# xUhEngwAng/I2V-Adapter-Unofficial

Measured on AMD Instinct MI355X. Metric: denoising steps/sec @ 16fx512x512 SD1.5+I2V-Adapter, higher is better.
Workload: dtype f16

## Files before the change

i2v-adapter-unofficial_amd/_lib.py:

```python
import ctypes as C
import os

_HERE = os.path.dirname(os.path.abspath(__file__))
LIB_PATH = os.environ.get("I2V_LIB_PATH") or os.path.join(_HERE, "libi2v_hip.so")
ABI_VERSION = 27

I2V_EPI_NONE, I2V_EPI_GELU, I2V_EPI_GEGLU = 0, 1, 2
I2V_STORE_ROWMAJOR, I2V_STORE_ROWPERM, I2V_STORE_VT, I2V_STORE_VT_T = 0, 1, 2, 3
I2V_A_PLAIN, I2V_A_CONV3X3 = 0, 1
I2V_LORA_MAX_ADAPTERS, I2V_LORA_MAX_RANK = 8, 256
I2V_ROUTE_GENERIC, I2V_ROUTE_CONV_THIN, I2V_ROUTE_BIG_TILE, I2V_ROUTE_BIG_DEEP, I2V_ROUTE_BIG_SPLITK = 0, 1, 2, 3, 4
I2V_EXTRA_NONE, I2V_EXTRA_LNF, I2V_EXTRA_HILO, I2V_EXTRA_GNS, I2V_EXTRA_UPF = 0, 1, 2, 4, 8
I2V_TATTN_LDS_FORM, I2V_TATTN_REG_FORM = 0, 1
I2V_ADD_RES_MAX = 16
I2V_TAESD_PREP_IDENTITY, I2V_TAESD_PREP_UNIT, I2V_TAESD_PREP_CLAMP = 0, 1, 2


class HipLibraryError(RuntimeError):
    pass


class GemmParams(C.Structure):
    _fields_ = [
        ("a", C.c_void_p), ("lda", C.c_int64),
        ("a2", C.c_void_p), ("lda2", C.c_int64),
        ("k_split", C.c_int32), ("a_mode", C.c_int32),
        ("w", C.c_void_p), ("ldw", C.c_int64),
        ("bias", C.c_void_p),
        ("residual", C.c_void_p), ("ldr", C.c_int64),
        ("rowvec", C.c_void_p), ("ld_rowvec", C.c_int64), ("rows_per_vec", C.c_int32), ("rowvec_period", C.c_int32),
        ("ln_wsum", C.c_void_p), ("ln_eps", C.c_float),
        ("c", C.c_void_p), ("ldc", C.c_int64),
        ("M", C.c_int32), ("N", C.c_int32), ("K", C.c_int32),
        ("epilogue", C.c_int32), ("store_mode", C.c_int32),
        ("frames", C.c_int32), ("hw", C.c_int32),
        ("vt_len", C.c_int32), ("vt_ld", C.c_int32),
        ("out_scale", C.c_float),
        ("n_img", C.c_int32), ("in_h", C.c_int32), ("in_w", C.c_int32), ("cin", C.c_int32),
        ("out_h", C.c_int32), ("out_w", C.c_int32), ("stride", C.c_int32), ("upsample", C.c_int32),
        ("asym_pad", C.c_int32), ("conv_kblock", C.c_int32),
        ("w_batch_stride", C.c_int64), ("rows_per_w", C.c_int32),
        ("a_perm_frames", C.c_int32), ("a_perm_hw", C.c_int32),
        ("workspace", C.c_void_p), ("workspace_bytes", C.c_int64),
        ("c_is_f32", C.c_int32),
        ("gn_partial", C.c_void_p), ("gn_groups", C.c_int32),
        ("residual_lo", C.c_void_p), ("c_lo", C.c_void_p),
    ]


class GemmRoute(C.Structure):
    _fields_ = [
        ("family", C.c_int32), ("a_mode", C.c_int32),
        ("rows", C.c_int32), ("cols", C.c_int32), ("stages", C.c_int32),
        ("splits", C.c_int32), ("kps", C.c_int32),
        ("extra", C.c_int32), ("persistent", C.c_int32),
        ("generic_tile", C.c_int32), ("vec4", C.c_int32),
        ("epilogue", C.c_int32), ("store_mode", C.c_int32),
    ]

    def as_dict(self):
        return {name: int(getattr(self, name)) for name, _ in self._fields_}


class AttnParams(C.Structure):
    _fields_ = [
        ("q", C.c_void_p), ("q_row_stride", C.c_int64), ("q_batch_stride", C.c_int64),
        ("k", C.c_void_p), ("k_row_stride", C.c_int64), ("k_batch_stride", C.c_int64),
        ("vt", C.c_void_p), ("vt_row_stride", C.c_int64), ("vt_batch_stride", C.c_int64),
        ("o", C.c_void_p), ("o_row_stride", C.c_int64), ("o_batch_stride", C.c_int64),
        ("batch_q", C.c_int32), ("kv_group", C.c_int32), ("heads", C.c_int32), ("head_dim", C.c_int32),
        ("lq", C.c_int32), ("lk", C.c_int32),
        ("scale", C.c_float), ("accumulate", C.c_int32), ("acc_scale", C.c_float),
        ("lse", C.c_void_p),
    ]


class AttnBwdParams(C.Structure):
    _fields_ = [
        ("q", C.c_void_p), ("q_row_stride", C.c_int64), ("q_batch_stride", C.c_int64),
        ("qt", C.c_void_p), ("qt_row_stride", C.c_int64), ("qt_batch_stride", C.c_int64),
        ("k", C.c_void_p), ("k_row_stride", C.c_int64), ("k_batch_stride", C.c_int64),
        ("kt", C.c_void_p), ("kt_row_stride", C.c_int64), ("kt_batch_stride", C.c_int64),
        ("v", C.c_void_p), ("v_row_stride", C.c_int64), ("v_batch_stride", C.c_int64),
        ("dout", C.c_void_p), ("do_row_stride", C.c_int64), ("do_batch_stride", C.c_int64),
        ("doutt", C.c_void_p), ("dot_row_stride", C.c_int64), ("dot_batch_stride", C.c_int64),
        ("lse", C.c_void_p), ("delta", C.c_void_p),
        ("dq", C.c_void_p), ("dq_row_stride", C.c_int64), ("dq_batch_stride", C.c_int64),
        ("dk", C.c_void_p), ("dk_row_stride", C.c_int64), ("dk_batch_stride", C.c_int64),
        ("dv", C.c_void_p), ("dv_row_stride", C.c_int64), ("dv_batch_stride", C.c_int64),
        ("batch_q", C.c_int32), ("kv_group", C.c_int32), ("heads", C.c_int32), ("head_dim", C.c_int32),
        ("lq", C.c_int32), ("lk", C.c_int32),
        ("scale", C.c_float), ("kv_partitions", C.c_int32), ("dkv_partial", C.c_void_p),
    ]


class TAttnParams(C.Structure):
    _fields_ = [
        ("q", C.c_void_p), ("q_row_stride", C.c_int64),
        ("k", C.c_void_p), ("k_row_stride", C.c_int64),
        ("vt", C.c_void_p), ("vt_ld", C.c_int32),
        ("o", C.c_void_p), ("o_row_stride", C.c_int64),
        ("n_pixels", C.c_int32), ("frames", C.c_int32), ("heads", C.c_int32), ("head_dim", C.c_int32),
        ("scale", C.c_float),
    ]


class TAttnRoute(C.Structure):
    _fields_ = [
        ("form", C.c_int32), ("dqk", C.c_int32), ("dpv", C.c_int32),
        ("pf", C.c_int32), ("nqt", C.c_int32), ("blocks", C.c_int32),
    ]

    def as_dict(self):
        return {name: int(getattr(self, name)) for name, _ in self._fields_}


class MotionAttnParams(C.Structure):
    _fields_ = [
        ("x", C.c_void_p), ("ldx", C.c_int64),
        ("gamma", C.c_void_p),
        ("shift", C.c_void_p), ("ld_shift", C.c_int64),
        ("w_qkv", C.c_void_p),
        ("out", C.c_void_p), ("ldo", C.c_int64),
        ("rows", C.c_int64),
        ("channels", C.c_int32), ("heads", C.c_int32), ("head_dim", C.c_int32), ("frames", C.c_int32),
        ("eps", C.c_float), ("scale", C.c_float),
        ("w_o", C.c_void_p), ("b_o", C.c_void_p),
    ]


class CrossAttnFusedParams(C.Structure):
    _fields_ = [
        ("x", C.c_void_p), ("ldx", C.c_int64),
        ("gamma", C.c_void_p), ("beta", C.c_void_p),
        ("w_q", C.c_void_p),
        ("ctx_frag", C.c_void_p),
        ("out", C.c_void_p), ("ldo", C.c_int64),
        ("rows", C.c_int64), ("rows_per_ctx", C.c_int64),
        ("channels", C.c_int32), ("heads", C.c_int32), ("head_dim", C.c_int32), ("ctx_len", C.c_int32),
        ("eps", C.c_float), ("scale", C.c_float),
        ("ip_frag", C.c_void_p), ("ip_len", C.c_int32), ("ip_scale", C.c_float),
        ("w_o", C.c_void_p), ("b_o", C.c_void_p),
    ]


class FfFusedParams(C.Structure):
    _fields_ = [
        ("x", C.c_void_p), ("ldx", C.c_int64),
        ("gamma", C.c_void_p), ("beta", C.c_void_p),
        ("w1", C.c_void_p), ("b1", C.c_void_p),
        ("w2", C.c_void_p), ("b2", C.c_void_p),
        ("out", C.c_void_p), ("ldo", C.c_int64),
        ("rows", C.c_int64),
        ("channels", C.c_int32), ("inner", C.c_int32),
        ("eps", C.c_float),
        ("w3", C.c_void_p), ("b3", C.c_void_p),
        ("res2", C.c_void_p), ("ld_res2", C.c_int64),
        ("perm_frames", C.c_int32), ("perm_hw", C.c_int32),
        ("res2_lo", C.c_void_p), ("out_lo", C.c_void_p),
    ]


class LnQkvParams(C.Structure):
    _fields_ = [
        ("x", C.c_void_p), ("ldx", C.c_int64),
        ("gamma", C.c_void_p), ("beta", C.c_void_p),
        ("w", C.c_void_p),
        ("qk", C.c_void_p), ("ld_qk", C.c_int64),
        ("vt", C.c_void_p), ("vt_batch_stride", C.c_int64), ("vt_row_stride", C.c_int64),
        ("rows", C.c_int64), ("rows_per_image", C.c_int64),
        ("channels", C.c_int32), ("n_qk", C.c_int32),
        ("eps", C.c_float),
        ("x_image_stride", C.c_int64),
    ]


class UnetConfig(C.Structure):
    _fields_ = [
        ("in_channels", C.c_int32), ("out_channels", C.c_int32),
        ("block_out_channels", C.c_int32 * 4),
        ("layers_per_block", C.c_int32), ("num_attention_heads", C.c_int32),
        ("cross_attention_dim", C.c_int32), ("norm_num_groups", C.c_int32),
        ("motion_max_seq_length", C.c_int32), ("motion_num_attention_heads", C.c_int32),
        ("use_motion_mid_block", C.c_int32), ("ip_num_tokens", C.c_int32),
    ]


class UnetPlan(C.Structure):
    _fields_ = [
        ("batch", C.c_int32), ("frames", C.c_int32), ("height", C.c_int32), ("width", C.c_int32),
        ("ctx_len", C.c_int32), ("has_ip", C.c_int32),
    ]


class GnParams(C.Structure):
    _fields_ = [
        ("x", C.c_void_p), ("c1", C.c_int32),
        ("x2", C.c_void_p), ("c2", C.c_int32),
        ("gamma", C.c_void_p), ("beta", C.c_void_p),
        ("y", C.c_void_p),
        ("n_img", C.c_int32), ("hw", C.c_int32), ("groups", C.c_int32), ("frames_per_stat", C.c_int32),
        ("eps", C.c_float), ("silu", C.c_int32),
        ("out_perm", C.c_int32), ("frames", C.c_int32),
        ("workspace", C.c_void_p),
        ("gpartial_in", C.c_void_p), ("gpartial_rows", C.c_int32),
    ]


class LoraAdapter(C.Structure):
    _fields_ = [("down", C.c_void_p), ("up", C.c_void_p), ("rank", C.c_int32), ("scale", C.c_float)]


class LnParams(C.Structure):
    _fields_ = [
        ("x", C.c_void_p), ("ldx", C.c_int64),
        ("gamma", C.c_void_p), ("beta", C.c_void_p),
        ("pe", C.c_void_p), ("ld_pe", C.c_int64), ("pe_period", C.c_int32),
        ("y", C.c_void_p), ("ldy", C.c_int64),
        ("rows", C.c_int32), ("C", C.c_int32),
        ("eps", C.c_float),
        ("x_rows_per_batch", C.c_int32), ("x_batch_stride", C.c_int64),
    ]


class AddResidualsEntry(C.Structure):
    _fields_ = [("dst", C.c_void_p), ("dst_lo", C.c_void_p), ("skip", C.c_void_p), ("skip_lo", C.c_void_p), ("res", C.c_void_p),
                ("numel", C.c_int64)]


class AddResidualsParams(C.Structure):
    _fields_ = [("t", AddResidualsEntry * I2V_ADD_RES_MAX), ("n", C.c_int32), ("scale_rows", C.c_int32), ("scale_table", C.c_void_p),
                ("step_idx", C.c_void_p)]


class ConvC64Params(C.Structure):
    _fields_ = [
        ("x", C.c_void_p), ("ldx", C.c_int64),
        ("w", C.c_void_p), ("bias", C.c_void_p),
        ("residual", C.c_void_p), ("ldr", C.c_int64),
        ("out", C.c_void_p), ("ldo", C.c_int64),
        ("n_img", C.c_int32), ("height", C.c_int32), ("width", C.c_int32),
        ("cin", C.c_int32), ("cout", C.c_int32),
        ("relu_mid", C.c_int32), ("relu_out", C.c_int32),
        ("max_workgroups", C.c_int32),
    ]


_P = C.c_void_p
SIGNATURES = {
    "i2v_abi_version": (C.c_int, []),
    "i2v_last_error": (C.c_char_p, []),
    "i2v_gemm_f16": (C.c_int, [C.POINTER(GemmParams), _P]),
    "i2v_gemm_ln_supported": (C.c_int, [C.POINTER(GemmParams)]),
    "i2v_gemm_batch_supported": (C.c_int, [C.POINTER(GemmParams)]),
    "i2v_gemm_upconv_fold_supported": (C.c_int, [C.POINTER(GemmParams)]),
    "i2v_gemm_workspace_bytes": (C.c_int64, [C.POINTER(GemmParams)]),
    "i2v_gemm_gn_partial_rows": (C.c_int32, [C.POINTER(GemmParams)]),
    "i2v_gemm_route": (C.c_int, [C.POINTER(GemmParams), C.POINTER(GemmRoute)]),
    "i2v_gemm_last_route": (C.c_int, [C.POINTER(GemmRoute)]),
    "i2v_gemm_kernel_exists": (C.c_int, [C.POINTER(GemmRoute)]),
    "i2v_attention_f16": (C.c_int, [C.POINTER(AttnParams), _P]),
    "i2v_temporal_attention_f16": (C.c_int, [C.POINTER(TAttnParams), _P]),
    "i2v_temporal_attention_route": (C.c_int, [C.POINTER(TAttnParams), C.POINTER(TAttnRoute)]),
    "i2v_temporal_attention_last_route": (C.c_int, [C.POINTER(TAttnRoute)]),
    "i2v_tattn_kernel_exists": (C.c_int, [C.POINTER(TAttnRoute)]),
    "i2v_motion_attn_supported": (C.c_int32, [C.c_int64, C.c_int32, C.c_int32, C.c_int32, C.c_int32]),
    "i2v_motion_attn_pack_rows": (C.c_int32, [C.c_int32, C.c_int32]),
    "i2v_motion_attn_f16": (C.c_int, [C.POINTER(MotionAttnParams), _P]),
    "i2v_cross_attn_fused_supported": (C.c_int32, [C.c_int64, C.c_int32, C.c_int32, C.c_int32, C.c_int32, C.c_int64]),
    "i2v_cross_attn_fused_pack_rows": (C.c_int32, [C.c_int32, C.c_int32]),
    "i2v_cross_attn_fused_ctx_elems": (C.c_int64, [C.c_int32, C.c_int32, C.c_int32]),
    "i2v_cross_attn_fused_f16": (C.c_int, [C.POINTER(CrossAttnFusedParams), _P]),
    "i2v_ln_qkv_supported": (C.c_int32, [C.c_int64, C.c_int32, C.c_int32, C.c_int64]),
    "i2v_ln_qkv_f16": (C.c_int, [C.POINTER(LnQkvParams), _P]),
    "i2v_ff_fused_supported": (C.c_int32, [C.c_int64, C.c_int32, C.c_int32]),
    "i2v_ff_fused_tail_supported": (C.c_int32, [C.c_int64, C.c_int32, C.c_int32, C.c_int32, C.c_int32]),
    "i2v_ff_fused_f16": (C.c_int, [C.POINTER(FfFusedParams), _P]),
    "i2v_groupnorm_workspace_bytes": (C.c_int64, [C.c_int32, C.c_int32, C.c_int32]),
    "i2v_groupnorm_f16": (C.c_int, [C.POINTER(GnParams), _P]),
    "i2v_groupnorm_fold_f16": (C.c_int, [C.POINTER(GnParams), _P, C.c_int64, _P, C.c_int32, _P, _P, _P]),
    "i2v_layernorm_f16": (C.c_int, [C.POINTER(LnParams), _P]),
    "i2v_softmax_rows_f16": (C.c_int, [_P, C.c_int64, _P, C.c_int64, C.c_int32, C.c_int32, C.c_float, _P]),
    "i2v_nchw_to_tokens": (C.c_int, [_P, C.c_int32, _P, C.c_int32, C.c_int32, C.c_int32, C.c_int32, _P]),
    "i2v_tokens_to_nchw": (C.c_int, [_P, C.c_int32, C.c_int64, _P, C.c_int32, C.c_int32, C.c_int32, C.c_int32, _P]),
    "i2v_timestep_embedding": (C.c_int, [_P, _P, C.c_int32, _P, C.c_int32, C.c_int32, _P]),
    "i2v_silu_f16": (C.c_int, [_P, _P, C.c_int64, _P]),
    "i2v_repeat_rows_f16": (C.c_int, [_P, _P, C.c_int64, C.c_int64, C.c_int32, _P]),
    "i2v_copy3d_f16": (C.c_int, [_P, C.c_int64, C.c_int64, _P, C.c_int64, C.c_int64, C.c_int64, C.c_int64,
                                 C.c_int64, _P]),
    "i2v_pack_ctx_fragments_elems": (C.c_int64, [C.c_int32, C.c_int32, C.c_int32]),
    "i2v_pack_ctx_fragments_f16": (C.c_int, [_P, C.c_int64, _P, C.c_int64, C.c_int64, _P, C.c_int32, C.c_int32, C.c_int32, C.c_int32, _P]),
    "i2v_ddim_prep": (C.c_int, [_P, _P, _P, C.c_int32, C.c_int32, C.c_int32, C.c_int32, C.c_int32, C.c_int32, _P]),
    "i2v_gaussian_sample_f32": (C.c_int, [_P, _P, _P, C.c_int32, C.c_int32, C.c_int32, _P]),
    "i2v_first_frame_prior_f32": (C.c_int, [_P, _P, _P, _P, C.c_int32, C.c_int32, C.c_int32, C.c_int32, C.c_int32,
                                            C.c_float, C.c_float, C.c_float, C.c_float, C.c_float, _P]),
    "i2v_attention_lse_f32": (C.c_int, [C.POINTER(AttnParams), _P, _P]),
    "i2v_attention_bwd_f16": (C.c_int, [C.POINTER(AttnBwdParams), _P]),
    "i2v_transpose_f16": (C.c_int, [_P, C.c_int64, C.c_int64, _P, C.c_int64, C.c_int64, C.c_int32, C.c_int32, C.c_int32, _P]),
    "i2v_rowdot_heads_f32": (C.c_int, [_P, C.c_int64, _P, C.c_int64, _P, C.c_int64, C.c_int32, C.c_int32, C.c_int32, _P]),
    "i2v_layernorm_bwd_f16": (C.c_int, [_P, C.c_int64, _P, C.c_int64, _P, _P, C.c_int64, _P, C.c_int64, C.c_int32, C.c_int32,
                                        C.c_float, _P]),
    "i2v_geglu_bwd_f16": (C.c_int, [_P, C.c_int64, _P, C.c_int64, _P, C.c_int64, C.c_int64, C.c_int32, _P]),
    "i2v_geglu_f16": (C.c_int, [_P, C.c_int64, _P, C.c_int64, C.c_int64, C.c_int32, _P]),
    "i2v_colsum_f32": (C.c_int, [_P, C.c_int64, _P, C.c_int64, C.c_int32, _P]),
    "i2v_colsum_prod_f32": (C.c_int, [_P, C.c_int64, _P, C.c_int64, _P, C.c_int64, C.c_int32, _P]),
    "i2v_colsum_workspace_bytes": (C.c_int64, [C.c_int64, C.c_int32]),
    "i2v_colsum_det_f32": (C.c_int, [_P, C.c_int64, _P, C.c_int64, _P, C.c_int64, C.c_int32, _P, _P]),
    "i2v_masked_mse_grad_f16": (C.c_int, [_P, _P, _P, C.c_int64, C.c_int32, C.c_int32, C.c_int32, C.c_float, _P]),
    "i2v_masked_mse_grad_f32": (C.c_int, [_P, _P, _P, _P, C.c_int64, C.c_int32, C.c_int32, C.c_int32, C.c_float, _P]),
    "i2v_groupnorm_bwd_workspace_bytes": (C.c_int64, [C.c_int32, C.c_int32, C.c_int32]),
    "i2v_groupnorm_bwd_f16": (C.c_int, [C.POINTER(GnParams), _P, _P, _P, _P]),
    "i2v_add_f16": (C.c_int, [_P, _P, _P, C.c_int64, _P]),
    "i2v_permute_rows_f16": (C.c_int, [_P, _P, C.c_int64, C.c_int32, C.c_int32, C.c_int32, C.c_int32, _P]),
    "i2v_zero_insert2x_f16": (C.c_int, [_P, _P, C.c_int64, C.c_int32, C.c_int32, C.c_int32, _P]),
    "i2v_sum_pool2x_f16": (C.c_int, [_P, _P, C.c_int64, C.c_int32, C.c_int32, C.c_int32, _P]),
    "i2v_sumsq_f32": (C.c_int, [_P, C.c_int64, _P, _P]),
    "i2v_adamw_f32": (C.c_int, [_P, _P, _P, _P, C.c_int64, C.c_float, C.c_float, C.c_float, C.c_float, C.c_float, C.c_int32,
                                C.c_float, _P, C.c_float, _P]),
    "i2v_adamw_guarded_f32": (C.c_int, [_P, _P, _P, _P, C.c_int64, C.c_float, C.c_float, C.c_float, C.c_float, C.c_float,
                                        C.c_float, C.c_float, _P, C.c_int32, _P, _P, _P, _P]),
    "i2v_axpby_f32": (C.c_int, [_P, _P, C.c_float, C.c_float, C.c_int64, _P]),
    "i2v_select_row_f16": (C.c_int, [_P, C.c_int64, C.c_int32, _P, _P, C.c_int32, _P]),
    "i2v_ddim_cfg_step": (C.c_int, [_P, _P, C.c_int32, C.c_int64, _P, C.c_int32, _P, C.c_float, C.c_int32, C.c_int32,
                                    C.c_int32, C.c_int32, C.c_int32, _P]),
    "i2v_dpm_cfg_step": (C.c_int, [_P, _P, _P, C.c_int32, C.c_int64, _P, C.c_int32, _P, C.c_float, C.c_int32, C.c_int32,
                                   C.c_int32, C.c_int32, C.c_int32, _P]),
    "i2v_lcm_cfg_step": (C.c_int, [_P, _P, C.c_int32, _P, C.c_int32, C.c_int64, _P, C.c_int32, _P, C.c_float, C.c_int32, C.c_int32,
                                   C.c_int32, C.c_int32, C.c_int32, _P]),
    "i2v_freeu_f16": (C.c_int, [_P, _P, _P, _P, _P, _P, C.c_int32, C.c_int32, C.c_int32, C.c_int32, C.c_int32, C.c_float, C.c_float, _P]),
    "i2v_vae_tile_blend": (C.c_int, [_P, _P, _P, _P, C.c_int32, C.c_int32, C.c_int32, C.c_int32, C.c_int64, C.c_int32, C.c_int32, C.c_int32,
                                     C.c_int32, C.c_int32, _P, C.c_int32, C.c_int32, C.c_int32, C.c_int32, _P]),
    "i2v_lora_merge": (C.c_int, [_P, _P, C.c_int32, C.c_int32, C.c_int32, C.POINTER(LoraAdapter), C.c_int32, _P]),
    "i2v_freeinit_workspace_bytes": (C.c_int64, [C.c_int32, C.c_int32, C.c_int32, C.c_int32, C.c_int32]),
    "i2v_freeinit_mix": (C.c_int, [_P, _P, _P, _P, _P, _P, C.c_int64, C.c_int32, C.c_int32, C.c_int32, C.c_int32, C.c_int32, C.c_float,
                                   C.c_float, _P]),
    "i2v_freenoise_gather_f16": (C.c_int, [_P, C.c_int64, _P, C.c_int64, _P, C.c_int64, C.c_int32, C.c_int32, C.c_int32, C.c_int32, _P]),
    "i2v_freenoise_blend_f16": (C.c_int, [_P, C.c_int64, _P, C.c_int64, _P, _P, C.c_int64, C.c_int32, C.c_int32, C.c_int32, C.c_int32,
                                          C.c_int32, _P]),
    "i2v_clip_embed_f16": (C.c_int, [_P, _P, _P, _P, _P, C.c_int32, C.c_int32, C.c_int32, C.c_int32, C.c_int32, _P]),
    "i2v_clip_attention_f16": (C.c_int, [_P, C.c_int64, C.c_int32, C.c_int32, C.c_int32, _P, C.c_int64, C.c_int32, C.c_int32, C.c_int32,
                                         C.c_int32, C.c_float, _P]),
    "i2v_quick_gelu_f16": (C.c_int, [_P, _P, C.c_int64, _P]),
    "i2v_clip_patchify_f16": (C.c_int, [_P, _P, C.c_int64, C.c_int32, C.c_int32, C.c_int32, C.c_int32, _P]),
    "i2v_clip_vision_embed_f16": (C.c_int, [_P, _P, C.c_int64, _P, _P, C.c_int32, C.c_int32, C.c_int32, _P]),
    "i2v_clip_vision_attention_f16": (C.c_int, [_P, C.c_int64, C.c_int32, C.c_int32, C.c_int32, _P, C.c_int64, C.c_int32, C.c_int32,
                                                C.c_int32, C.c_int32, C.c_float, _P]),
    "i2v_perceiver_attention_f16": (C.c_int, [_P, C.c_int64, C.c_int32, _P, C.c_int64, C.c_int32, C.c_int32, C.c_int32, _P, C.c_int64,
                                              C.c_int32, C.c_int32, C.c_int32, _P, C.c_int64, C.c_int32, C.c_int32, C.c_int32, C.c_int32,
                                              C.c_float, _P]),
    "i2v_add_residuals_f16": (C.c_int, [C.POINTER(AddResidualsParams), _P]),
    "i2v_conv3x3_c64_f16": (C.c_int, [C.POINTER(ConvC64Params), _P]),
    "i2v_taesd_prep_f16": (C.c_int, [_P, C.c_int32, _P, C.c_int64, C.c_int32, C.c_int32, C.c_int32, C.c_int32, _P]),
    "i2v_pixel_unshuffle8_f16": (C.c_int, [_P, C.c_int32, _P, C.c_int32, C.c_int32, C.c_int32, C.c_int32, _P]),
    "i2v_avgpool2x_f16": (C.c_int, [_P, _P, C.c_int32, C.c_int32, C.c_int32, C.c_int32, _P]),
    "i2v_relu_f16": (C.c_int, [_P, _P, C.c_int64, _P]),
    "i2v_add_broadcast_residual_f16": (C.c_int, [_P, _P, _P, _P, _P, C.c_int64, C.c_int64, _P, C.c_int32, _P, _P]),
    "i2v_interp_rows_f16": (C.c_int, [_P, C.c_int64, C.c_int32, _P, _P, _P, _P, C.c_int64, C.c_int32, C.c_int32, _P]),
    "i2v_masked_renoise_f32": (C.c_int, [_P, _P, _P, _P, _P, C.c_int32, _P, C.c_int64, C.c_int32, C.c_int32, _P]),
    "i2v_weight_embeds_f16": (C.c_int, [_P, _P, _P, _P, C.c_int32, C.c_int32, C.c_int32, C.c_int64, C.c_int64, C.c_int32, _P]),
# ... 56 lines not shown
```

i2v-adapter-unofficial_amd/blocks.py:

```python
import math
import os
from typing import Optional

import torch
from torch import nn

from . import kernels as K
from . import streams
from ._lib import (I2V_EPI_GEGLU, I2V_EPI_GELU, I2V_EPI_NONE, I2V_STORE_ROWPERM, HipLibraryError)
from .checkpoint import PretrainedMixin

f16 = torch.float16


class HipModule(nn.Module):

    def __init__(self):
        super().__init__()
        self._packed = None
        self._packed_key = None

    def _pack(self):
        return {}

# ... 81 lines not shown
                    for ky in rows[py][ty]:
                        for kx in rows[px][tx]:
                            acc = w[:, :, ky, kx] if acc is None else acc + w[:, :, ky, kx]
                    taps.append(acc)
            phases.append(torch.stack(taps, dim=1))
    f = torch.stack(phases, dim=0)
    if K.conv_k_block(ci):
        f = f.reshape(4, co, 4, ci // 64, 64).permute(0, 1, 3, 2, 4)
    return f.reshape(4, co, 4 * ci).to(dtype).contiguous()


UPCONV_FOLD = os.environ.get("I2V_UPCONV_FOLD", "1") != "0"


def pack_geglu(weight, bias):
    inner = weight.shape[0] // 2
    w = torch.stack([weight[:inner], weight[inner:]], dim=1).reshape(2 * inner, weight.shape[1])
    b = torch.stack([bias[:inner], bias[inner:]], dim=1).reshape(2 * inner)
    return w16(w), w16(b)


LN_FOLD = os.environ.get("I2V_LN_FOLD", "1") != "0"


def fold_layernorm(weight, bias, gamma, beta):
    wf = (weight.detach().float() * gamma.detach().float()[None, :]).to(f16).contiguous()
    wsum = wf.float().sum(dim=1).contiguous()
    b = weight.detach().float() @ beta.detach().float()
    if bias is not None:
        b = b + bias.detach().float()
    return wf, wsum, b.to(f16).contiguous()


def fold_layernorm_geglu(proj_weight, proj_bias, gamma, beta):
    wf, wsum, b = fold_layernorm(proj_weight, proj_bias, gamma, beta)
    inner = wf.shape[0] // 2
    il = lambda t: torch.stack([t[:inner], t[inner:]], dim=1).reshape((2 * inner,) + tuple(t.shape[1:])).contiguous()
    return il(wf), il(wsum), il(b)


class LnFoldPlan:

    def __init__(self):
        self._cache = {}

    def get(self, key, probe):
        if not LN_FOLD:
            return False
        if key not in self._cache:
            self._cache[key] = bool(probe())
        return self._cache[key]


class ProjectedContext:

    def __init__(self, text, ip):
        self.text, self.ip = text, ip
        self.kv = {}
        self.frag = {}

    @property
    def shape(self):
        return self.text.shape


class ProjectedTemb:

    def __init__(self, all_proj, slices):
        self.all_proj, self.slices = all_proj, slices

    def view_for(self, resnet):
        off, n = self.slices[resnet]
        return self.all_proj[:, off: off + n]

    def first_half(self):
        r = self.all_proj.shape[0]
        return self if r == 1 else ProjectedTemb(self.all_proj[: r // 2], self.slices)


GN_FOLD = os.environ.get("I2V_GN_FOLD", "1") != "0"
GN_FOLD_RATIO = float(os.environ.get("I2V_GN_FOLD_RATIO", "4"))


def gn_proj_in(x, gamma, beta, groups, eps, w, bias, frames=0):
    n, hh, ww, c = x.shape
    hw = hh * ww
    fps = frames if frames > 0 else 1
    s_groups, n_out = n // fps, w.shape[0]
    if GN_FOLD and GN_FOLD_RATIO * s_groups * n_out <= n * hw:
        kw = dict(rows_per_vec=fps * hw, w_rows=fps * hw, a_perm=(frames, hw) if frames > 0 else None)
        if _fold_supported(x, s_groups, n_out, kw):
            w_s, b_s = K.groupnorm_fold(x, gamma, beta, groups, eps, w, bias, frames_per_stat=fps)
            return K.gemm(x.view(-1, c), w_s, None, rowvec=b_s, **kw)
    if frames > 0:
        h = K.groupnorm(x, gamma, beta, groups, eps, frames_per_stat=frames, out_perm=True, frames=frames)
    else:
        h = K.groupnorm(x, gamma, beta, groups, eps).view(-1, c)
    return K.gemm(h, w, bias)


_FOLD_OK = {}


def _fold_supported(x, s_groups, n_out, kw):
    key = (tuple(x.shape), s_groups, n_out, kw["w_rows"], kw["a_perm"])
    ok = _FOLD_OK.get(key)
    if ok is None:
        c = x.shape[3]
        w_s = torch.empty((s_groups, n_out, c), dtype=f16, device=x.device)
        b_s = torch.empty((s_groups, n_out), dtype=f16, device=x.device)
        ok = _FOLD_OK[key] = K.gemm(x.view(-1, c), w_s, None, rowvec=b_s, query_batch_support=True, **kw)
    return ok


def to_tokens(x: torch.Tensor, c_pad: Optional[int] = None) -> torch.Tensor:
    return K.nchw_to_tokens(x, c_pad)


def from_tokens(x: torch.Tensor, dtype) -> torch.Tensor:
    return K.tokens_to_nchw(x, dtype=dtype if dtype in (torch.float32, f16) else f16)


def _as_f16_matrix(t: torch.Tensor) -> torch.Tensor:
    if not t.is_cuda:
        raise HipLibraryError(f"tensor on {t.device}: the HIP path has no CPU fallback")
    return t.to(f16).contiguous()


class Timesteps(nn.Module):

    def __init__(self, num_channels: int, flip_sin_to_cos: bool = True, downscale_freq_shift: float = 0):
        super().__init__()
        if not flip_sin_to_cos or downscale_freq_shift != 0:
            raise NotImplementedError("hot path uses Timesteps(C, flip_sin_to_cos=True, freq_shift=0)")
        self.num_channels = num_channels

    def forward(self, timesteps: torch.Tensor) -> torch.Tensor:
        return K.timestep_embedding(timesteps.to(torch.float32).contiguous(), self.num_channels)


class TimestepEmbedding(HipModule):

    def __init__(self, in_channels: int, time_embed_dim: int, act_fn: str = "silu"):
        super().__init__()
        self.linear_1 = nn.Linear(in_channels, time_embed_dim)
        self.act = nn.SiLU()
        self.linear_2 = nn.Linear(time_embed_dim, time_embed_dim)

    def _pack(self):
        return dict(w1=w16(self.linear_1.weight), b1=w16(self.linear_1.bias), w2=w16(self.linear_2.weight),
                    b2=w16(self.linear_2.bias))

    def forward(self, sample, condition=None):
        p = self.packed()
        h = K.silu(K.gemm(_as_f16_matrix(sample), p["w1"], p["b1"]))
        return K.gemm(h, p["w2"], p["b2"])


_PRECISE_STREAM = os.environ.get("I2V_STREAM_PRECISE", "0") != "0"


def precise_stream() -> bool:
    return _PRECISE_STREAM


def set_precise_stream(on: bool) -> bool:
    global _PRECISE_STREAM
    prev, _PRECISE_STREAM = _PRECISE_STREAM, bool(on)
    return prev


GN_FROM_CONV = os.environ.get("I2V_GN_FROM_CONV", "1") != "0"


class ResnetBlock2D(HipModule):
# ... 194 lines not shown
        return o

    def forward(self, hidden_states, encoder_hidden_states=None, attention_mask=None):
        if attention_mask is not None:
            raise NotImplementedError("attention masks are never passed on the hot path (SURVEY 8b)")
        p = self.packed()
        x = _as_f16_matrix(hidden_states)
        b, l, c = x.shape
        q = K.gemm(x.view(-1, c), p["wq"])
        ctx = x if encoder_hidden_states is None else _as_f16_matrix(encoder_hidden_states)
        ctx_ip = None
        if self.ip_num_tokens and encoder_hidden_states is not None:
            end = ctx.shape[1] - self.ip_num_tokens
            ctx_text = torch.empty((ctx.shape[0], end, ctx.shape[2]), dtype=f16, device=x.device)
            ctx_ip = torch.empty((ctx.shape[0], self.ip_num_tokens, ctx.shape[2]), dtype=f16, device=x.device)
            K.copy3d(ctx[:, :end], ctx_text)
            K.copy3d(ctx[:, end:], ctx_ip)
            ctx = ctx_text
        if b % ctx.shape[0] != 0:
            raise ValueError(f"context batch {ctx.shape[0]} does not divide query batch {b}")
        o = self._cross(q, ctx, ctx_ip, b, l, b // ctx.shape[0])
        out = K.gemm(o, p["wo"], p["bo"])
        return out.view(b, l, -1).to(hidden_states.dtype)


class GEGLU(nn.Module):
    def __init__(self, dim_in, dim_out, bias=True):
        super().__init__()
        self.proj = nn.Linear(dim_in, dim_out * 2, bias=bias)


class GELU(nn.Module):
    def __init__(self, dim_in, dim_out, approximate="none", bias=True):
        super().__init__()
        if approximate != "none":
            raise NotImplementedError("only erf GELU is implemented")
        self.proj = nn.Linear(dim_in, dim_out, bias=bias)


def ff_tail_operands(weight, bias, c_in, c_out):
    if c_in != c_out or not K.ff_fused_tail_supported(128, c_in, 4 * c_in):
        return None
    return K.pack_ff_tail(weight.detach().reshape(c_out, c_in), bias)


class FeedForward(HipModule):

    def __init__(self, dim, dim_out=None, mult=4, dropout=0.0, activation_fn="geglu", inner_dim=None, bias=True):
        super().__init__()
        if not bias:
            raise NotImplementedError("ff_bias=False is not on the hot path")
        inner_dim = int(dim * mult) if inner_dim is None else inner_dim
        dim_out = dim if dim_out is None else dim_out
        self.activation_fn = activation_fn
        if activation_fn == "geglu":
            act = GEGLU(dim, inner_dim, bias=bias)
        elif activation_fn == "gelu":
            act = GELU(dim, inner_dim, bias=bias)
        else:
            raise ValueError(f"unsupported activation_fn {activation_fn}")
        self.net = nn.ModuleList([act, nn.Dropout(dropout), nn.Linear(inner_dim, dim_out, bias=bias)])

    def _pack(self):
        proj = self.net[0].proj
        if self.activation_fn == "geglu":
            w1, b1 = pack_geglu(proj.weight.detach(), proj.bias.detach())
        else:
            w1, b1 = w16(proj.weight), w16(proj.bias)
        out = LazyPack(w1=w1, b1=b1, w2=w16(self.net[2].weight), b2=w16(self.net[2].bias))
        if self.activation_fn == "geglu" and K.ff_fused_supported(128, self.net[2].weight.shape[0], self.net[2].weight.shape[1]):
            out.lazy("fused", lambda proj=proj, lin=self.net[2]: K.pack_ff_fused(proj.weight, proj.bias, lin.weight, lin.bias))
        return out

    def _fwd(self, n2d, residual2d, **store):
        p = self.packed()
        epi = I2V_EPI_GEGLU if self.activation_fn == "geglu" else I2V_EPI_GELU
        h = K.gemm(n2d, p["w1"], p["b1"], epilogue=epi)
        return K.gemm(h, p["w2"], p["b2"], residual=residual2d, **store)

    def fused_supported(self, x2d):
        p = self.packed()
        return FUSED_FF and "fused" in p and K.ff_fused_supported(x2d.shape[0], x2d.shape[1], p["b1"].numel() // 2)

    def _fwd_fused(self, x2d, gamma32, beta32, eps, tail=None):
        return K.ff_fused(x2d, gamma32, beta32, self.packed()["fused"], eps=eps, tail=tail, precise=precise_stream())

    def tail_supported(self, x2d, tail):
        p = self.packed()
        return (FUSED_FF and FUSED_FF_TAIL and tail is not None and tail[0] is not None and "fused" in p and
                K.ff_fused_tail_supported(x2d.shape[0], x2d.shape[1], p["b1"].numel() // 2, tail[2], tail[3]))

    def fold_norm(self, norm):
        if self.activation_fn != "geglu":
            return None
        proj = self.net[0].proj
        return fold_layernorm_geglu(proj.weight, proj.bias, norm.weight, norm.bias)

    def _fwd_folded(self, x2d, eps, folded, **store):
        p = self.packed()
        wf, wsum, bf = folded
        h = K.gemm(x2d, wf, bf, epilogue=I2V_EPI_GEGLU, ln=(wsum, eps))
        return K.gemm(h, p["w2"], p["b2"], residual=x2d, **store)

    def folded_supported(self, x2d, eps, folded):
        wf, wsum, bf = folded
        return K.gemm(x2d, wf, bf, epilogue=I2V_EPI_GEGLU, ln=(wsum, eps), query_ln_support=True)

    def forward(self, hidden_states, scale: float = 1.0):
        x = _as_f16_matrix(hidden_states)
        shp = x.shape
        return self._fwd(x.view(-1, shp[-1]), None).view(*shp[:-1], -1).to(hidden_states.dtype)


class SinusoidalPositionalEmbedding(nn.Module):

    def __init__(self, embed_dim: int, max_seq_length: int = 32):
        super().__init__()
        self.embed_dim, self.max_seq_length = embed_dim, max_seq_length
        self.register_buffer("pe", self._table(embed_dim, max_seq_length))

    @staticmethod
    def _table(embed_dim, max_seq_length):
        position = torch.arange(max_seq_length, device="cpu").unsqueeze(1)
        div_term = torch.exp(torch.arange(0, embed_dim, 2, device="cpu") * (-math.log(10000.0) / embed_dim))
        pe = torch.zeros(1, max_seq_length, embed_dim, device="cpu")
        pe[0, :, 0::2] = torch.sin(position * div_term)
        pe[0, :, 1::2] = torch.cos(position * div_term)
        return pe

    def reset_table_(self):
        with torch.no_grad():
            self.pe.copy_(self._table(self.embed_dim, self.max_seq_length).to(self.pe.dtype))


FUSED_MOTION_ATTN = os.environ.get("I2V_MOTION_FUSED", "1") != "0"
FUSED_FF = os.environ.get("I2V_FF_FUSED", "1") != "0"
FUSED_FF_TAIL = os.environ.get("I2V_FF_TAIL", "1") != "0"
FUSED_ATTN_OUT = os.environ.get("I2V_ATTN_OUTP", "1") != "0"


class TemporalTransformerBlock(HipModule):

    def __init__(self, dim, num_attention_heads, attention_head_dim, dropout=0.0, cross_attention_dim=None,
                 activation_fn="geglu", attention_bias=False, double_self_attention=True,
                 norm_elementwise_affine=True, norm_eps=1e-5, positional_embeddings="sinusoidal",
                 num_positional_embeddings=32, **_unused):
        super().__init__()
        if cross_attention_dim is not None or not double_self_attention or positional_embeddings != "sinusoidal":
            raise NotImplementedError("motion modules use double self-attention with sinusoidal positions (A9)")
        self.dim, self.heads, self.dim_head = dim, num_attention_heads, attention_head_dim
        self.eps = norm_eps
        self.max_len = num_positional_embeddings
        self.pos_embed = SinusoidalPositionalEmbedding(dim, max_seq_length=num_positional_embeddings)
        self.norm1 = nn.LayerNorm(dim, elementwise_affine=norm_elementwise_affine, eps=norm_eps)
        self.attn1 = Attention(query_dim=dim, heads=num_attention_heads, dim_head=attention_head_dim,
                               dropout=dropout, bias=attention_bias)
        self.norm2 = nn.LayerNorm(dim, elementwise_affine=norm_elementwise_affine, eps=norm_eps)
        self.attn2 = Attention(query_dim=dim, heads=num_attention_heads, dim_head=attention_head_dim,
                               dropout=dropout, bias=attention_bias)
        self.norm3 = nn.LayerNorm(dim, elementwise_affine=norm_elementwise_affine, eps=norm_eps)
        self.ff = FeedForward(dim, dropout=dropout, activation_fn=activation_fn)
        self._plan = LnFoldPlan()
        self.free_noise = None

    def _pack(self):
        p = LazyPack(pe=w16(self.pos_embed.pe[0]))
        for i, (norm, attn) in enumerate(((self.norm1, self.attn1), (self.norm2, self.attn2)), 1):
# ... 68 lines not shown
                if FUSED_ATTN_OUT:
                    t = K.motion_attn(t, tab[0], tab[1], p[f"wqkv{i}"], heads=self.heads, head_dim=self.dim_head, frames=frames,
                                      eps=self.eps, out_proj=p[f"wo_frag{i}"])
                    continue
                o = K.motion_attn(t, tab[0], tab[1], p[f"wqkv{i}"], heads=self.heads, head_dim=self.dim_head, frames=frames,
                                  eps=self.eps)
                t = K.gemm(o, p[f"wo{i}"], p[f"bo{i}"], residual=t)
                continue
            n = None if fold_attn else K.layernorm(t, p[f"g{i}"], p[f"b{i}"], self.eps, pe=p["pe"], pe_period=frames)
            with streams.fork(overlap, t.device) as fk:
                with fk.side():
                    if fold_attn:
                        vt = K.project_vt(t, p[f"f_wv{i}"], frames, bias=p[f"f_cv{i}"], ln=(p[f"f_sv{i}"], self.eps),
                                          pe_t=p[f"f_pev{i}"], pe_period=frames)
                    else:
                        vt = K.project_vt(n, p[f"wv{i}"], frames)
                if fold_attn:
                    qk = K.gemm(t, p[f"f_wqk{i}"], p[f"f_cqk{i}"], ln=(p[f"f_sqk{i}"], self.eps),
                                rowvec=p[f"f_peqk{i}"], rowvec_period=frames)
                else:
                    qk = K.gemm(n, p[f"wqk{i}"])
            o = K.temporal_attention(qk[:, :c], qk[:, c:], vt, n_pixels=n_pixels, frames=frames, heads=self.heads,
                                     head_dim=self.dim_head, scale=self.dim_head ** -0.5)
            t = K.gemm(o, p[f"wo{i}"], p[f"bo{i}"], residual=t)
        return t

    def _fwd_ff(self, t, fold_ff, tail):
        p = self.packed()

        def ret(v, applied=False):
            return v if tail is None else (v, applied)
        if self.ff.fused_supported(t):
            if self.ff.tail_supported(t, tail):
                return ret(self.ff._fwd_fused(t, p["g3_f32"], p["b3_f32"], self.eps, tail=tail), True)
            return ret(self.ff._fwd_fused(t, p["g3_f32"], p["b3_f32"], self.eps))
        if fold_ff:
            return ret(self.ff._fwd_folded(t, self.eps, p["f_ff"]))
        n = K.layernorm(t, p["g3"], p["b3"], self.eps)
        return ret(self.ff._fwd(n, t))


class TransformerTemporalModel(HipModule):

    def __init__(self, num_attention_heads=16, attention_head_dim=88, in_channels=None, out_channels=None,
                 num_layers=1, dropout=0.0, norm_num_groups=32, cross_attention_dim=None, attention_bias=False,
                 activation_fn="geglu", norm_elementwise_affine=True, double_self_attention=True,
                 positional_embeddings=None, num_positional_embeddings=None):
        super().__init__()
        inner_dim = num_attention_heads * attention_head_dim
        self.in_channels, self.inner_dim = in_channels, inner_dim
        self.groups = norm_num_groups
        self.norm = nn.GroupNorm(norm_num_groups, in_channels, eps=1e-6, affine=True)
        self.proj_in = nn.Linear(in_channels, inner_dim)
        self.transformer_blocks = nn.ModuleList([
            TemporalTransformerBlock(inner_dim, num_attention_heads, attention_head_dim, dropout=dropout,
                                     cross_attention_dim=cross_attention_dim, activation_fn=activation_fn,
                                     attention_bias=attention_bias, double_self_attention=double_self_attention,
                                     norm_elementwise_affine=norm_elementwise_affine,
                                     positional_embeddings=positional_embeddings,
                                     num_positional_embeddings=num_positional_embeddings)
            for _ in range(num_layers)])
        self.proj_out = nn.Linear(inner_dim, in_channels)

    def _pack(self):
        p = LazyPack(g=w16(self.norm.weight), b=w16(self.norm.bias), wi=w16(self.proj_in.weight),
                     bi=w16(self.proj_in.bias), wo=w16(self.proj_out.weight), bo=w16(self.proj_out.bias))
        p.lazy("tail", lambda po=self.proj_out, ci=self.inner_dim, co=self.in_channels: ff_tail_operands(po.weight, po.bias, ci, co))
        return p

    def set_free_noise(self, settings):
        for blk in self.transformer_blocks:
            if settings is not None and settings.context_length > blk.max_len:
                raise ValueError(f"`context_length` {settings.context_length} exceeds the motion module's num_positional_embeddings "
                                 f"({blk.max_len})")
        for blk in self.transformer_blocks:
            blk.free_noise = settings

    def _fwd(self, x, num_frames):
        p = self.packed()
        n, hh, ww, c = x.shape
        if n % num_frames != 0:
            raise ValueError(f"batch {n} is not a multiple of num_frames {num_frames}")
        n_pixels = (n // num_frames) * hh * ww
        t = gn_proj_in(x, p["g"], p["b"], self.groups, 1e-6, p["wi"], p["bi"], frames=num_frames)
        applied = False
        for j, blk in enumerate(self.transformer_blocks):
            if j + 1 == len(self.transformer_blocks):
                t, applied = blk._fwd(t, n_pixels, num_frames, tail=(p["tail"], K.sview(x, -1, c), num_frames, hh * ww))
            else:
                t = blk._fwd(t, n_pixels, num_frames)
        if applied:
            return K.sview(t, n, hh, ww, c)
        out = K.gemm(t, p["wo"], p["bo"], residual=K.sview(x, -1, c), store=I2V_STORE_ROWPERM, frames=num_frames,
                     hw=hh * ww, precise=precise_stream())
        return K.sview(out, n, hh, ww, c)

    def forward(self, hidden_states, encoder_hidden_states=None, num_frames: int = 1, return_dict=False, **_unused):
        return (from_tokens(self._fwd(to_tokens(hidden_states), num_frames), hidden_states.dtype),)


class ImageProjection(HipModule):

    def __init__(self, image_embed_dim=768, cross_attention_dim=768, num_image_text_embeds=4):
        super().__init__()
        self.num_image_text_embeds = num_image_text_embeds
        self.cross_attention_dim = cross_attention_dim
        self.image_embeds = nn.Linear(image_embed_dim, num_image_text_embeds * cross_attention_dim)
        self.norm = nn.LayerNorm(cross_attention_dim)

    def _pack(self):
        return dict(w=w16(self.image_embeds.weight), b=w16(self.image_embeds.bias), g=w16(self.norm.weight),
                    be=w16(self.norm.bias))

    def forward(self, image_embeds):
        p = self.packed()
        x = _as_f16_matrix(image_embeds)
        y = K.gemm(x, p["w"], p["b"]).view(-1, self.cross_attention_dim)
        y = K.layernorm(y, p["g"], p["be"], self.norm.eps)
        return y.view(x.shape[0], self.num_image_text_embeds, self.cross_attention_dim)


class _ResamplerAttention(nn.Module):

    def __init__(self, dim, inner):
        super().__init__()
        self.to_q, self.to_k, self.to_v = (nn.Linear(dim, inner, bias=False) for _ in range(3))
        self.to_out = nn.ModuleList([nn.Linear(inner, dim, bias=False), nn.Dropout(0.0)])


class _ResamplerFeedForward(nn.Module):

    def __init__(self, dim, inner):
        super().__init__()
        self.net = nn.ModuleList([GELU(dim, inner, bias=False), nn.Dropout(0.0), nn.Linear(inner, dim, bias=False)])


class Resampler(HipModule):

    DIM_HEAD, MAX_QUERIES, MAX_KEYS = 64, 64, 288

    def __init__(self, embed_dims=768, output_dims=1024, hidden_dims=1280, depth=4, dim_head=64, heads=16, num_queries=8, ffn_ratio=4):
        super().__init__()
        if dim_head != self.DIM_HEAD:
            raise NotImplementedError(f"dim_head {dim_head}: the attention kernel (i2v_perceiver_attention_f16) implements head_dim "
                                      f"{self.DIM_HEAD} only")
        if not 1 <= num_queries <= self.MAX_QUERIES:
            raise NotImplementedError(f"num_queries {num_queries}: the attention kernel (i2v_perceiver_attention_f16) takes 1 to "
                                      f"{self.MAX_QUERIES} queries")
        inner_ff = int(hidden_dims * ffn_ratio)
        if embed_dims % 8 or output_dims % 8 or hidden_dims % 8 or inner_ff % 8 or inner_ff != hidden_dims * ffn_ratio:
            raise NotImplementedError(f"embed_dims {embed_dims}, output_dims {output_dims}, hidden_dims {hidden_dims} and hidden_dims * "
                                      f"ffn_ratio {hidden_dims * ffn_ratio} must be multiples of 8 (i2v_gemm_f16)")
        self.embed_dims, self.output_dims, self.hidden_dims = embed_dims, output_dims, hidden_dims
        self.depth, self.dim_head, self.heads, self.num_queries, self.ffn_ratio = depth, dim_head, heads, num_queries, ffn_ratio
        self.latents = nn.Parameter(torch.randn(1, num_queries, hidden_dims) / hidden_dims ** 0.5)
        self.proj_in = nn.Linear(embed_dims, hidden_dims)
        self.proj_out = nn.Linear(hidden_dims, output_dims)
        self.norm_out = nn.LayerNorm(output_dims)
        self.layers = nn.ModuleList([
            nn.ModuleList([nn.LayerNorm(hidden_dims), nn.LayerNorm(hidden_dims), _ResamplerAttention(hidden_dims, dim_head * heads),
                           nn.Sequential(nn.LayerNorm(hidden_dims), _ResamplerFeedForward(hidden_dims, inner_ff))])
            for _ in range(depth)])

    def check_tokens(self, tokens: int):
        if tokens < 1 or tokens + self.num_queries > self.MAX_KEYS:
            raise NotImplementedError(f"{tokens} image tokens + {self.num_queries} queries: the attention kernel "
                                      f"(i2v_perceiver_attention_f16) takes at most {self.MAX_KEYS} keys")
# ... 500 lines not shown
```

i2v-adapter-unofficial_amd/csrc/ff_fused.hip:

```cpp
#include <stdlib.h>

#include <type_traits>

#include "common.h"

namespace {

__device__ __forceinline__ void ff_dma16(__amdgpu_buffer_rsrc_t rsrc, f16* lds_wave_base, unsigned voff, unsigned soff = 0) {
  __builtin_amdgcn_raw_ptr_buffer_load_lds(rsrc, (__attribute__((address_space(3))) void*)lds_wave_base, 16, voff, soff, 0, 0);
}
__device__ __forceinline__ int opaque(int v) {
  asm volatile("" : "+v"(v));
  return v;
}

constexpr int FF_PIX = 8;
constexpr int FF_CH = 128;
constexpr int FF_U = 2;
constexpr int FF_PD = 3;
constexpr int FF_AD = 4;

template <int C, int INNER, int H, bool PROJ, bool HILO = false>
__global__ __launch_bounds__(64 * H) void ff_fused_kernel(const i2v_ff_fused_params p, const int ntiles, long long* __restrict__ stamps) {
  constexpr int KS = C / 32, NJ = C / 64, NCH = INNER / FF_CH, DN = C / H, DT = (DN + 15) / 16;
  static_assert(C % 64 == 0 && H == 8 && INNER % FF_CH == 0 && DT == 3 && DN == 40, "SD-1.5 64^2 level: C = 320, inner = 1280");
  static_assert(PROJ || !HILO, "the precise stream enters and leaves through the tail");
  extern __shared__ __attribute__((aligned(16))) f16 lds[];
  f16* panel = lds;
  f16* hbuf = lds + FF_PIX * 16 * C;
  f16* raw = lds + FF_PIX * 16 * C;
  static_assert(2 * FF_PIX * 16 * FF_CH <= FF_PIX * 16 * C, "the raw rows of a tile cover the chunk buffers (160 KB of LDS in all)");
  const int tid = threadIdx.x, lane = tid & 63, wave = __builtin_amdgcn_readfirstlane(tid >> 6);
  const int g = lane >> 4, l15 = lane & 15, sub = lane & 7, sw = l15 & 7;
  const int swz[2] = {(g ^ sw) * 8, ((4 + g) ^ sw) * 8};
  const f16* __restrict__ X = reinterpret_cast<const f16*>(p.x);

  auto fetch_rows = [&](const int tile) {
    const f16* base = X + ((int64_t)tile * (FF_PIX * 16) + 16 * wave) * p.ldx;
    const auto rs = __builtin_amdgcn_make_buffer_rsrc(const_cast<f16*>(base), 0, (int)((15 * p.ldx + C) * 2), 0x00020000);
    const int ln = opaque(lane);
    const unsigned voff = (unsigned)(((ln >> 3) * p.ldx + (ln & 7) * 8) * 2);
#pragma unroll
    for (int half = 0; half < 2; ++half)
#pragma unroll
      for (int j = 0; j < NJ; ++j)
        ff_dma16(rs, raw + 16 * wave * C + (half * NJ + j) * 512, voff, (unsigned)((8 * half * p.ldx + 8 * j * 8) * 2));
  };
  auto fetch_residual = [&](const int tile) {
    const f16* base = X + ((int64_t)tile * (FF_PIX * 16) + 16 * wave) * p.ldx;
    const auto rs = __builtin_amdgcn_make_buffer_rsrc(const_cast<f16*>(base), 0, (int)((15 * p.ldx + C) * 2), 0x00020000);
    constexpr int CPR = C / 8;
    static_assert((16 * CPR) % 64 == 0 && CPR % 8 == 0, "whole DMA instructions per wave, swizzle inside groups of 8 chunks");
    const int ln = opaque(lane);
#pragma unroll
    for (int i = 0; i < 16 * CPR / 64; ++i) {
      const int q = i * 64 + ln, r = q / CPR, cp = q - r * CPR;
      ff_dma16(rs, panel + 16 * wave * C + i * 512, (unsigned)((r * p.ldx + (cp ^ (r & 7)) * 8) * 2));
    }
  };
  auto normalise_rows = [&]() {
    f16x8 xv[2][NJ];
#pragma unroll
    for (int half = 0; half < 2; ++half)
#pragma unroll
      for (int j = 0; j < NJ; ++j) xv[half][j] = *reinterpret_cast<const f16x8*>(raw + 16 * wave * C + ((half * NJ + j) * 64 + lane) * 8);
    const float* gp = reinterpret_cast<const float*>(p.gamma);
    const float* bp = reinterpret_cast<const float*>(p.beta);
    asm volatile("" : "+s"(gp), "+s"(bp));
    f32x4 ga[NJ][2], be[NJ][2];
#pragma unroll
    for (int j = 0; j < NJ; ++j) {
      ga[j][0] = *reinterpret_cast<const f32x4*>(gp + (sub + 8 * j) * 8);
      ga[j][1] = *reinterpret_cast<const f32x4*>(gp + (sub + 8 * j) * 8 + 4);
      be[j][0] = *reinterpret_cast<const f32x4*>(bp + (sub + 8 * j) * 8);
      be[j][1] = *reinterpret_cast<const f32x4*>(bp + (sub + 8 * j) * 8 + 4);
    }
#pragma unroll
    for (int half = 0; half < 2; ++half) {
      const int row = 16 * wave + 8 * half + (lane >> 3);
      float v[NJ][8];
      float s = 0.f;
#pragma unroll
      for (int j = 0; j < NJ; ++j)
#pragma unroll
        for (int e = 0; e < 8; ++e) {
          v[j][e] = (float)xv[half][j][e];
          s += v[j][e];
        }
      s = sum_lanes8(s);
      const float mean = s / (float)C;
      float q = 0.f;
#pragma unroll
      for (int j = 0; j < NJ; ++j)
#pragma unroll
        for (int e = 0; e < 8; ++e) {
          v[j][e] -= mean;
          q = fmaf(v[j][e], v[j][e], q);
        }
      q = sum_lanes8(q);
      const float rstd = rsqrtf(q / (float)C + p.eps);
#pragma unroll
      for (int j = 0; j < NJ; ++j) {
        const int ch = sub + 8 * j;
        f16x8 o;
#pragma unroll
        for (int e = 0; e < 8; ++e) o[e] = (f16)fmaf(v[j][e] * rstd, ga[j][e >> 2][e & 3], be[j][e >> 2][e & 3]);
        *reinterpret_cast<f16x8*>(panel + row * C + ((ch ^ (row & 7)) * 8)) = o;
      }
    }
// ... 197 lines not shown
      auto load_res2 = [&](const int h) {
#pragma unroll
        for (int q = 0; q < HP; ++q) {
          const f16* rrow = R2 + (int64_t)orow[h * HP + q] * p.ld_res2;
          r01[h][q] = *reinterpret_cast<const u32x4*>(rrow + c01);
          r2[h][q] = (eg == 0) ? *reinterpret_cast<const u32x4*>(rrow + 32) : u32x4{0u, 0u, 0u, 0u};
        }
      };
      const f16* __restrict__ R2L = reinterpret_cast<const f16*>(HILO ? p.res2_lo : p.res2) + wave * DN;
      f16* __restrict__ OL = reinterpret_cast<f16*>(HILO ? p.out_lo : p.out) + wave * DN;
      u32x4 l01[HP], l2[HP];
      auto load_res2_lo = [&](const int h) {
        if constexpr (HILO) {
#pragma unroll
          for (int q = 0; q < HP; ++q) {
            const f16* rrow = R2L + (int64_t)orow[h * HP + q] * p.ld_res2;
            l01[q] = *reinterpret_cast<const u32x4*>(rrow + c01);
            l2[q] = (eg == 0) ? *reinterpret_cast<const u32x4*>(rrow + 32) : u32x4{0u, 0u, 0u, 0u};
          }
        }
      };
      out_rows(tile, el15, orow);
#pragma unroll
      for (int pix = 0; pix < FF_PIX; ++pix)
#pragma unroll
        for (int t = 0; t < DT; ++t) {
          if (16 * t + 4 * eg < DN) {
            f16x4* slot = reinterpret_cast<f16x4*>(panel + 16 * pix * C + res_off[t]);
            const f16x4 xres = *slot;
            f32x4 o = acc2[pix][t];
#pragma unroll
            for (int r = 0; r < 4; ++r) o[r] += (float)xres[r];
            *slot = to_half(o);
          }
        }
      lds_barrier();
      f32x4 acc3[FF_PIX][DT];
      {
        const float* b3 = reinterpret_cast<const float*>(p.b3) + wave * DN;
#pragma unroll
        for (int t = 0; t < DT; ++t) {
          const f32x4 bias3 = (16 * t + 4 * eg < DN) ? *reinterpret_cast<const f32x4*>(b3 + 16 * t + 4 * eg) : f32x4{0.f, 0.f, 0.f, 0.f};
#pragma unroll
          for (int pix = 0; pix < FF_PIX; ++pix) acc3[pix][t] = bias3;
        }
      }
      {
        const int w3o = wave * (KS * DT * 1024);
        auto ldw3 = [&](const int s, const int t) {
          return __builtin_bit_cast(f16x8, __builtin_amdgcn_raw_buffer_load_b128(rs_w3, w_lane, w3o + (s * DT + t) * 1024, 0));
        };
        f16x8 wf[FF_PD][DT];
#pragma unroll
        for (int s = 0; s < FF_PD - 1; ++s)
#pragma unroll
          for (int t = 0; t < DT; ++t) wf[s][t] = ldw3(s, t);
        constexpr int NI = KS * FF_PIX;
        auto lda = [&](const int i) {
          return *reinterpret_cast<const f16x8*>(alane + 16 * (i % FF_PIX) * C + 64 * ((i / FF_PIX) >> 1) + swz[(i / FF_PIX) & 1]);
        };
        f16x8 af[FF_AD + 1];
#pragma unroll
        for (int i = 0; i < FF_AD; ++i) af[i] = lda(i);
#pragma unroll
        for (int i = 0; i < NI; ++i) {
          const int s = i / FF_PIX, pix = i % FF_PIX;
          if (pix == 0 && s + FF_PD - 1 < KS) {
#pragma unroll
            for (int t = 0; t < DT; ++t) wf[(s + FF_PD - 1) % FF_PD][t] = ldw3(s + FF_PD - 1, t);
          }
          if (pix == 0 && s + FF_PD - 1 == KS - 1) {
            if (next < ntiles) fetch_rows(next);
            load_res2(0);
          }
          if (i + FF_AD < NI) af[(i + FF_AD) % (FF_AD + 1)] = lda(i + FF_AD);
#pragma unroll
          for (int t = 0; t < DT; ++t) acc3[pix][t] = mfma16x16x32(wf[s % FF_PD][t], af[i % (FF_AD + 1)], acc3[pix][t]);
          __builtin_amdgcn_sched_barrier(0);
        }
      }
      FF_T(t_p);
      load_res2(1);
      load_res2_lo(0);
#pragma unroll
      for (int pix = 0; pix < FF_PIX; ++pix) {
        if (pix == HP) {
          __builtin_amdgcn_sched_barrier(0);
          load_res2_lo(1);
        }
        const u32x4 q01 = r01[pix / HP][pix % HP], q2 = r2[pix / HP][pix % HP];
        u32x2 xa = {q01[0], q01[1]}, xb = {q01[2], q01[3]}, xc = {q2[0], q2[1]}, xd = {q2[2], q2[3]};
        asm volatile("s_nop 1\n\tv_permlane16_swap_b32 %0, %1\n\tv_permlane16_swap_b32 %2, %3\n\t"
                     "v_permlane16_swap_b32 %4, %5\n\tv_permlane16_swap_b32 %6, %7"
                     : "+v"(xa[0]), "+v"(xb[0]), "+v"(xa[1]), "+v"(xb[1]), "+v"(xc[0]), "+v"(xd[0]), "+v"(xc[1]), "+v"(xd[1]));
        const f16x4 xres[DT] = {__builtin_bit_cast(f16x4, xa), __builtin_bit_cast(f16x4, xb), __builtin_bit_cast(f16x4, xc)};
        f16x4 xlo[DT] = {};
        if constexpr (HILO) {
          const u32x4 p01 = l01[pix % HP], p2 = l2[pix % HP];
          u32x2 la = {p01[0], p01[1]}, lb = {p01[2], p01[3]}, lc = {p2[0], p2[1]}, ld = {p2[2], p2[3]};
          asm volatile("s_nop 1\n\tv_permlane16_swap_b32 %0, %1\n\tv_permlane16_swap_b32 %2, %3\n\t"
                       "v_permlane16_swap_b32 %4, %5\n\tv_permlane16_swap_b32 %6, %7"
                       : "+v"(la[0]), "+v"(lb[0]), "+v"(la[1]), "+v"(lb[1]), "+v"(lc[0]), "+v"(ld[0]), "+v"(lc[1]), "+v"(ld[1]));
          xlo[0] = __builtin_bit_cast(f16x4, la);
          xlo[1] = __builtin_bit_cast(f16x4, lb);
          xlo[2] = __builtin_bit_cast(f16x4, lc);
        }
        u32x2 oh[DT], ol[DT];
#pragma unroll
        for (int t = 0; t < DT; ++t) {
          f32x4 o = acc3[pix][t];
#pragma unroll
          for (int r = 0; r < 4; ++r) o[r] += (float)xres[t][r];
          if constexpr (HILO) {
#pragma unroll
            for (int r = 0; r < 4; ++r) o[r] += (float)xlo[t][r];
          }
          const f16x4 o16 = to_half(o);
          oh[t] = __builtin_bit_cast(u32x2, o16);
          if constexpr (HILO) {
            f32x4 d;
#pragma unroll
            for (int r = 0; r < 4; ++r) d[r] = o[r] - (float)o16[r];
            ol[t] = __builtin_bit_cast(u32x2, to_half(d));
          }
        }
        store_row(O + (int64_t)orow[pix] * p.ldo, oh);
        if constexpr (HILO) store_row(OL + (int64_t)orow[pix] * p.ldo, ol);
      }
    }
    lds_barrier();
    FF_T(t_epi);
  }
#ifdef I2V_FF_STAMPS
  if (stamps != nullptr && lane == 0) {
    long long* st = stamps + ((int64_t)blockIdx.x * H + wave) * 8;
    st[0] = t_ln; st[1] = t_ff1; st[2] = t_glu; st[3] = t_bar; st[4] = t_ff2; st[5] = t_epi; st[6] = t_w; st[7] = t_p;
  }
#endif
}

constexpr size_t FF_LDS = 2 * (size_t)FF_PIX * 16 * 320 * sizeof(f16);

template <bool PROJ, bool HILO = false>
int ff_cus() { return i2v_big_lds_kernel_cus(reinterpret_cast<const void*>(ff_fused_kernel<320, 1280, 8, PROJ, HILO>), FF_LDS); }

}

extern "C" int32_t i2v_ff_fused_supported(int64_t rows, int32_t channels, int32_t inner) {
  return rows > 0 && rows % (FF_PIX * 16) == 0 && rows / (FF_PIX * 16) < (1 << 24) && channels == 320 && inner == 1280 &&
         ff_cus<false>() > 0;
}

extern "C" int32_t i2v_ff_fused_tail_supported(int64_t rows, int32_t channels, int32_t inner, int32_t perm_frames, int32_t perm_hw) {
  if (!(rows > 0 && rows % (FF_PIX * 16) == 0 && rows / (FF_PIX * 16) < (1 << 24) && channels == 320 && inner == 1280)) return 0;
  if (perm_frames != 0 || perm_hw != 0) {
    if (perm_frames <= 0 || (perm_frames & (perm_frames - 1)) || perm_hw <= 0 || rows % ((int64_t)perm_frames * perm_hw) != 0) return 0;
  }
  return ff_cus<true>() > 0;
}

extern "C" int i2v_ff_fused_f16(const i2v_ff_fused_params* pp, i2v_stream_t stream) {
  I2V_CHECK_ARG(pp != nullptr, "i2v_ff_fused_f16: null params");
  const i2v_ff_fused_params& p = *pp;
  I2V_CHECK_ARG(p.x && p.gamma && p.beta && p.w1 && p.b1 && p.w2 && p.b2 && p.out, "i2v_ff_fused_f16: null pointer");
  const bool tail = p.w3 != nullptr;
  I2V_CHECK_ARG(p.rows > 0 && p.rows % (FF_PIX * 16) == 0 && p.rows / (FF_PIX * 16) < (1 << 24) && p.channels == 320 && p.inner == 1280,
                "i2v_ff_fused_f16: rows %lld channels %d inner %d is not a fused shape (i2v_ff_fused_supported)", (long long)p.rows,
                p.channels, p.inner);
  I2V_CHECK_ARG(p.ldx >= p.channels && p.ldx % 8 == 0 && p.ldo >= p.channels && p.ldo % 8 == 0, "i2v_ff_fused_f16: row strides");
  I2V_CHECK_ARG(i2v_al16(p.x) && i2v_al16(p.gamma) && i2v_al16(p.beta) && i2v_al16(p.w1) && i2v_al16(p.b1) && i2v_al16(p.w2) && i2v_al16(p.b2) && i2v_al16(p.out),
                "i2v_ff_fused_f16: pointers must be 16-byte aligned");
  I2V_CHECK_ARG(p.ldx < (1 << 24), "i2v_ff_fused_f16: ldx");
  if (tail) {
    I2V_CHECK_ARG(p.b3 && p.res2, "i2v_ff_fused_f16: the tail needs w3, b3 and res2");
    I2V_CHECK_ARG(i2v_al16(p.w3) && i2v_al16(p.b3) && i2v_al16(p.res2) && p.ld_res2 >= p.channels && p.ld_res2 % 8 == 0,
                  "i2v_ff_fused_f16: tail operands must be 16-byte aligned, ld_res2 a multiple of 8");
    I2V_CHECK_ARG(i2v_ff_fused_tail_supported(p.rows, p.channels, p.inner, p.perm_frames, p.perm_hw) ||
                      ff_cus<true>() == 0,
                  "i2v_ff_fused_f16: perm_frames %d / perm_hw %d do not describe rows %lld (i2v_ff_fused_tail_supported)", p.perm_frames,
                  p.perm_hw, (long long)p.rows);
    I2V_CHECK_ARG(!(p.perm_frames > 0 && p.out == p.x), "i2v_ff_fused_f16: out must not alias x when the tail permutes the rows");
    I2V_CHECK_ARG((p.res2_lo == nullptr) == (p.out_lo == nullptr) && i2v_al16(p.res2_lo) && i2v_al16(p.out_lo) && (p.out_lo == nullptr || p.out_lo != p.out),
                  "i2v_ff_fused_f16: res2_lo and out_lo come together, 16-byte aligned");
  } else {
    I2V_CHECK_ARG(p.b3 == nullptr && p.res2 == nullptr && p.perm_frames == 0 && p.perm_hw == 0 && p.res2_lo == nullptr && p.out_lo == nullptr,
                  "i2v_ff_fused_f16: tail fields set without w3");
  }
  const bool hilo = tail && p.out_lo != nullptr;
  const int cus = hilo ? ff_cus<true, true>() : tail ? ff_cus<true>() : ff_cus<false>();
  if (cus <= 0) I2V_FAIL(I2V_ERR_UNSUPPORTED, "i2v_ff_fused_f16: %zu bytes of LDS refused by this device", FF_LDS);
  const int ntiles = (int)(p.rows / (FF_PIX * 16));
  const int grid = i2v_persistent_grid(ntiles, cus);
  long long* stamps = nullptr;
#ifdef I2V_FF_STAMPS
  stamps = getenv("I2V_FF_STAMP_PTR") ? reinterpret_cast<long long*>(strtoull(getenv("I2V_FF_STAMP_PTR"), nullptr, 0)) : nullptr;
#endif
  hipStream_t s = reinterpret_cast<hipStream_t>(stream);
  if (hilo)
    hipLaunchKernelGGL((ff_fused_kernel<320, 1280, 8, true, true>), dim3((unsigned)grid), dim3(512), FF_LDS, s, p, ntiles, stamps);
  else if (tail)
    hipLaunchKernelGGL((ff_fused_kernel<320, 1280, 8, true>), dim3((unsigned)grid), dim3(512), FF_LDS, s, p, ntiles, stamps);
  else
    hipLaunchKernelGGL((ff_fused_kernel<320, 1280, 8, false>), dim3((unsigned)grid), dim3(512), FF_LDS, s, p, ntiles, stamps);
  return i2v_check_launch("i2v_ff_fused_f16");
}
```

i2v-adapter-unofficial_amd/csrc/norm.hip:

```cpp
#include <cstdlib>

#include "common.h"

namespace {

static inline int gn_rows_per_chunk(int n_img, int hw) {
  const int want_chunks = (int)i2v_cdiv(1024, n_img);
  int rpc = (int)i2v_cdiv(hw, want_chunks);
  rpc = (rpc + 7) / 8 * 8;
  if (rpc < 16) rpc = 16;
  if (rpc > 256) rpc = 256;
  return rpc;
}

__device__ __forceinline__ float wave_sum(float v) {
#pragma unroll
  for (int o = 32; o >= 1; o >>= 1) v += __shfl_xor(v, o, 64);
  return v;
}

constexpr int GN_MAXC = 2560, GN_MAXG = 64;
__global__ __launch_bounds__(256) void gn_stats_kernel(const f16* __restrict__ x1, int c1, const f16* __restrict__ x2,
                                                       int c2, int hw, int rpc, float* __restrict__ partial,
                                                       float* __restrict__ gpartial = nullptr, int groups = 0) {
// ... 645 lines not shown
        if (row < p.rows) {
          f16x8 pv = zero8();
          if (p.pe) pv = ld_global_16B(reinterpret_cast<const f16*>(p.pe) + (int64_t)(row % p.pe_period) * p.ld_pe + vi * 8);
          f16x8 o;
#pragma unroll
          for (int e = 0; e < 8; ++e) {
            float t = (v[r][i][e] - mean[r]) * rstd[r] * (float)ga[e] + (float)be[e];
            if (p.pe) t += (float)pv[e];
            o[e] = (f16)t;
          }
          *reinterpret_cast<f16x8*>(reinterpret_cast<f16*>(p.y) + (int64_t)row * p.ldy + vi * 8) = o;
        }
      }
    }
  }
}

__global__ __launch_bounds__(256) void softmax_rows_kernel(const f16* __restrict__ x, int64_t ldx, f16* __restrict__ y,
                                                           int64_t ldy, int rows, int cols, float scale_log2) {
  const int lane = threadIdx.x & 63;
  const int row = blockIdx.x * 4 + (threadIdx.x >> 6);
  if (row >= rows) return;
  const f16* xr = x + (int64_t)row * ldx;
  f16* yr = y + (int64_t)row * ldy;
  const int nvec = cols / 8;
  float mx = -INFINITY;
  for (int v = lane; v < nvec; v += 64) {
    const f16x8 t = ld_global_16B(xr + v * 8);
#pragma unroll
    for (int e = 0; e < 8; ++e) mx = fmaxf(mx, (float)t[e]);
  }
  for (int c = nvec * 8 + lane; c < cols; c += 64) mx = fmaxf(mx, (float)xr[c]);
#pragma unroll
  for (int o = 32; o >= 1; o >>= 1) mx = fmaxf(mx, __shfl_xor(mx, o, 64));
  const float mb = mx * scale_log2;
  float sum = 0.f;
  for (int v = lane; v < nvec; v += 64) {
    const f16x8 t = ld_global_16B(xr + v * 8);
#pragma unroll
    for (int e = 0; e < 8; ++e) sum += __builtin_amdgcn_exp2f((float)t[e] * scale_log2 - mb);
  }
  for (int c = nvec * 8 + lane; c < cols; c += 64) sum += __builtin_amdgcn_exp2f((float)xr[c] * scale_log2 - mb);
  sum = wave_sum(sum);
  const float inv = 1.0f / sum;
  for (int v = lane; v < nvec; v += 64) {
    const f16x8 t = ld_global_16B(xr + v * 8);
    f16x8 o;
#pragma unroll
    for (int e = 0; e < 8; ++e) o[e] = (f16)(__builtin_amdgcn_exp2f((float)t[e] * scale_log2 - mb) * inv);
    *reinterpret_cast<f16x8*>(yr + v * 8) = o;
  }
  for (int c = nvec * 8 + lane; c < cols; c += 64) yr[c] = (f16)(__builtin_amdgcn_exp2f((float)xr[c] * scale_log2 - mb) * inv);
}

}

extern "C" int64_t i2v_groupnorm_workspace_bytes(int32_t n_img, int32_t hw, int32_t channels) {
  const int64_t nchunk = i2v_cdiv(hw, gn_rows_per_chunk(n_img, hw));
  return ((int64_t)n_img * nchunk * channels * 2 + (int64_t)n_img * channels * 2 + (int64_t)n_img * nchunk * GN_MAXG * 2) *
         (int64_t)sizeof(float);
}

extern "C" int i2v_groupnorm_fold_f16(const i2v_gn_params* pp, const void* w, int64_t ldw, const void* bias, int32_t n_out,
                                      void* w_out, void* bias_out, i2v_stream_t stream) {
  I2V_CHECK_ARG(pp != nullptr, "i2v_groupnorm_fold_f16: null params");
  const i2v_gn_params& p = *pp;
  const int C = p.c1 + p.c2;
  I2V_CHECK_ARG(p.x && p.gamma && p.beta && p.workspace && w && w_out && bias_out, "i2v_groupnorm_fold_f16: null pointer");
  I2V_CHECK_ARG(p.n_img > 0 && p.hw > 0 && p.c1 > 0 && p.c2 >= 0 && n_out > 0 && ldw >= C,
                "i2v_groupnorm_fold_f16: bad sizes");
  I2V_CHECK_ARG((p.c2 == 0) == (p.x2 == nullptr), "i2v_groupnorm_fold_f16: x2 / c2 mismatch");
  I2V_CHECK_ARG(p.c1 % 8 == 0 && p.c2 % 8 == 0, "i2v_groupnorm_fold_f16: channel counts must be multiples of 8");
  I2V_CHECK_ARG(p.groups > 0 && C % p.groups == 0, "i2v_groupnorm_fold_f16: channels %d not divisible by groups %d", C,
                p.groups);
  I2V_CHECK_ARG(p.frames_per_stat > 0 && p.n_img % p.frames_per_stat == 0,
                "i2v_groupnorm_fold_f16: n_img %d not divisible by frames_per_stat %d", p.n_img, p.frames_per_stat);
  I2V_CHECK_ARG(i2v_al16(p.x) && (!p.x2 || i2v_al16(p.x2)) && i2v_al16(p.workspace) && i2v_al16(p.gamma) && i2v_al16(p.beta),
                "i2v_groupnorm_fold_f16: pointers must be 16-byte aligned");
  hipStream_t s = reinterpret_cast<hipStream_t>(stream);
  const int rpc = gn_rows_per_chunk(p.n_img, p.hw);
  const int nchunk = (int)i2v_cdiv(p.hw, rpc);
  float* partial = reinterpret_cast<float*>(p.workspace);
  float* coef = partial + (int64_t)p.n_img * nchunk * C * 2;
  if (p.groups <= GN_MAXG && C <= GN_MAXC) {
    float* gpartial = coef + (int64_t)p.n_img * C * 2;
    hipLaunchKernelGGL(gn_stats_kernel, dim3(nchunk, p.n_img), dim3(256), (size_t)C * 2 * sizeof(float), s,
                       reinterpret_cast<const f16*>(p.x), p.c1, reinterpret_cast<const f16*>(p.x2), p.c2, p.hw, rpc, partial, gpartial,
                       p.groups);
    hipLaunchKernelGGL(gn_finalize_g_kernel, dim3(p.n_img / p.frames_per_stat, p.groups), dim3(256), 0, s, gpartial, nchunk, C,
                       p.groups, p.frames_per_stat, p.hw, rpc, p.eps, reinterpret_cast<const f16*>(p.gamma),
                       reinterpret_cast<const f16*>(p.beta), coef);
  } else {
    hipLaunchKernelGGL(gn_stats_kernel, dim3(nchunk, p.n_img), dim3(256), 0, s, reinterpret_cast<const f16*>(p.x), p.c1,
                       reinterpret_cast<const f16*>(p.x2), p.c2, p.hw, rpc, partial);
    hipLaunchKernelGGL(gn_finalize_kernel, dim3(p.n_img / p.frames_per_stat, p.groups), dim3(256), 0, s, partial, nchunk, C,
                       p.groups, p.frames_per_stat, p.hw, rpc, p.eps, reinterpret_cast<const f16*>(p.gamma),
                       reinterpret_cast<const f16*>(p.beta), coef);
  }
  hipLaunchKernelGGL(gn_fold_kernel, dim3(n_out, p.n_img / p.frames_per_stat), dim3(256), 0, s, coef, p.frames_per_stat, C,
                     reinterpret_cast<const f16*>(w), ldw, reinterpret_cast<const f16*>(bias), n_out,
                     reinterpret_cast<f16*>(w_out), reinterpret_cast<f16*>(bias_out));
  return i2v_check_launch("i2v_groupnorm_fold_f16");
}

extern "C" int i2v_groupnorm_f16(const i2v_gn_params* pp, i2v_stream_t stream) {
  I2V_CHECK_ARG(pp != nullptr, "i2v_groupnorm_f16: null params");
  const i2v_gn_params& p = *pp;
  const int C = p.c1 + p.c2;
  I2V_CHECK_ARG(p.x && p.gamma && p.beta && p.y && p.workspace, "i2v_groupnorm_f16: null pointer");
  I2V_CHECK_ARG(p.n_img > 0 && p.hw > 0 && p.c1 > 0 && p.c2 >= 0, "i2v_groupnorm_f16: bad sizes");
  I2V_CHECK_ARG((p.c2 == 0) == (p.x2 == nullptr), "i2v_groupnorm_f16: x2 / c2 mismatch");
  I2V_CHECK_ARG(p.c1 % 8 == 0 && p.c2 % 8 == 0, "i2v_groupnorm_f16: channel counts must be multiples of 8 (%d, %d)",
                p.c1, p.c2);
  I2V_CHECK_ARG(p.groups > 0 && C % p.groups == 0, "i2v_groupnorm_f16: channels %d not divisible by groups %d", C,
                p.groups);
  I2V_CHECK_ARG(p.frames_per_stat > 0 && p.n_img % p.frames_per_stat == 0,
                "i2v_groupnorm_f16: n_img %d not divisible by frames_per_stat %d", p.n_img, p.frames_per_stat);
  if (p.out_perm) I2V_CHECK_ARG(p.frames > 0 && p.n_img % p.frames == 0, "i2v_groupnorm_f16: bad frames for out_perm");
  I2V_CHECK_ARG(i2v_al16(p.x) && i2v_al16(p.y) && (!p.x2 || i2v_al16(p.x2)) && i2v_al16(p.workspace) && i2v_al16(p.gamma) && i2v_al16(p.beta),
                "i2v_groupnorm_f16: pointers must be 16-byte aligned");
  hipStream_t s = reinterpret_cast<hipStream_t>(stream);
  if (p.gpartial_in != nullptr) {
    I2V_CHECK_ARG(p.frames_per_stat == 1 && !p.out_perm && p.x2 == nullptr && p.groups <= GN_MAXG && C <= GN_MAXC,
                  "i2v_groupnorm_f16: gpartial_in is for per-image statistics of one source without a row permutation");
    I2V_CHECK_ARG(p.gpartial_rows > 0 && p.hw % p.gpartial_rows == 0 && (reinterpret_cast<uintptr_t>(p.gpartial_in) & 7) == 0,
                  "i2v_groupnorm_f16: gpartial_rows (%d) must divide hw (%d)", p.gpartial_rows, p.hw);
    const int pchunks = p.hw / p.gpartial_rows;
    const size_t lds = ((size_t)pchunks * p.groups * 2 + (size_t)p.groups * 2) * sizeof(float);
    I2V_CHECK_ARG(lds <= 48 * 1024, "i2v_groupnorm_f16: %d partial blocks per image do not fit the finalise step", pchunks);
    const int rpc = gn_rows_per_chunk(p.n_img, p.hw);
    hipLaunchKernelGGL(gn_apply_fused_kernel, dim3((unsigned)i2v_cdiv(p.hw, rpc), p.n_img), dim3(256), lds, s,
                       reinterpret_cast<const f16*>(p.x), p.c1, static_cast<const f16*>(nullptr), 0,
                       reinterpret_cast<const float*>(p.gpartial_in), p.groups, reinterpret_cast<const f16*>(p.gamma),
                       reinterpret_cast<const f16*>(p.beta), p.eps, reinterpret_cast<f16*>(p.y), p.hw, rpc, p.silu, pchunks,
                       p.gpartial_rows);
    return i2v_check_launch("i2v_groupnorm_f16(partials from the producer)");
  }
  {
    size_t lds = 0;
    const int gb = gn_slab_plan(p.n_img, p.hw, C, p.groups, p.frames_per_stat, &lds);
    if (gb > 0) {
      static const bool attr_ok = hipFuncSetAttribute(reinterpret_cast<const void*>(gn_slab_kernel),
                                                      hipFuncAttributeMaxDynamicSharedMemorySize, 97 * 1024) == hipSuccess;
      if (attr_ok) {
        hipLaunchKernelGGL(gn_slab_kernel, dim3(p.groups / gb, p.n_img / p.frames_per_stat), dim3(256), lds, s,
                           reinterpret_cast<const f16*>(p.x), p.c1, reinterpret_cast<const f16*>(p.x2), p.c2,
                           reinterpret_cast<const f16*>(p.gamma), reinterpret_cast<const f16*>(p.beta),
                           reinterpret_cast<f16*>(p.y), p.hw, p.frames_per_stat, p.groups, gb, p.eps, p.silu, p.out_perm,
                           p.frames);
        return i2v_check_launch("i2v_groupnorm_f16(slab)");
      }
    }
  }
  const int rpc = gn_rows_per_chunk(p.n_img, p.hw);
  const int nchunk = (int)i2v_cdiv(p.hw, rpc);
  float* partial = reinterpret_cast<float*>(p.workspace);
  float* coef = partial + (int64_t)p.n_img * nchunk * C * 2;
  const f16* x1 = reinterpret_cast<const f16*>(p.x);
  const f16* x2 = reinterpret_cast<const f16*>(p.x2);
  static const int fused_off = getenv("I2V_GN_FUSED") ? (atoi(getenv("I2V_GN_FUSED")) == 0) : 0;
  const size_t fused_lds = ((size_t)nchunk * p.groups * 2 + (size_t)p.groups * 2) * sizeof(float);
  if (!fused_off && p.frames_per_stat == 1 && !p.out_perm && p.groups <= GN_MAXG && C <= GN_MAXC && fused_lds <= 48 * 1024) {
    float* gpartial = coef + (int64_t)p.n_img * C * 2;
    hipLaunchKernelGGL(gn_stats_kernel, dim3(nchunk, p.n_img), dim3(256), (size_t)C * 2 * sizeof(float), s, x1, p.c1, x2, p.c2, p.hw,
                       rpc, partial, gpartial, p.groups);
    hipLaunchKernelGGL(gn_apply_fused_kernel, dim3(nchunk, p.n_img), dim3(256), fused_lds, s, x1, p.c1, x2, p.c2, gpartial, p.groups,
                       reinterpret_cast<const f16*>(p.gamma), reinterpret_cast<const f16*>(p.beta), p.eps,
                       reinterpret_cast<f16*>(p.y), p.hw, rpc, p.silu, nchunk, rpc);
    return i2v_check_launch("i2v_groupnorm_f16(fused finalize)");
  }
  if (!fused_off && p.groups <= GN_MAXG && C <= GN_MAXC) {
    float* gpartial = coef + (int64_t)p.n_img * C * 2;
    hipLaunchKernelGGL(gn_stats_kernel, dim3(nchunk, p.n_img), dim3(256), (size_t)C * 2 * sizeof(float), s, x1, p.c1, x2, p.c2, p.hw,
                       rpc, partial, gpartial, p.groups);
    hipLaunchKernelGGL(gn_finalize_g_kernel, dim3(p.n_img / p.frames_per_stat, p.groups), dim3(256), 0, s, gpartial, nchunk, C,
                       p.groups, p.frames_per_stat, p.hw, rpc, p.eps, reinterpret_cast<const f16*>(p.gamma),
                       reinterpret_cast<const f16*>(p.beta), coef);
  } else {
    hipLaunchKernelGGL(gn_stats_kernel, dim3(nchunk, p.n_img), dim3(256), 0, s, x1, p.c1, x2, p.c2, p.hw, rpc, partial);
    hipLaunchKernelGGL(gn_finalize_kernel, dim3(p.n_img / p.frames_per_stat, p.groups), dim3(256), 0, s, partial, nchunk, C,
                       p.groups, p.frames_per_stat, p.hw, rpc, p.eps, reinterpret_cast<const f16*>(p.gamma),
                       reinterpret_cast<const f16*>(p.beta), coef);
  }
  const int64_t total = (int64_t)p.n_img * p.hw * (C / 8);
  const int blocks = (int)(i2v_cdiv(total, 256) < 4096 ? i2v_cdiv(total, 256) : 4096);
  hipLaunchKernelGGL(gn_apply_kernel, dim3(blocks), dim3(256), 0, s, x1, p.c1, x2, p.c2, coef,
                     reinterpret_cast<f16*>(p.y), p.n_img, p.hw, p.silu, p.out_perm, p.frames);
  return i2v_check_launch("i2v_groupnorm_f16");
}


extern "C" int64_t i2v_groupnorm_bwd_workspace_bytes(int32_t n_img, int32_t hw, int32_t channels) {
  const int64_t nchunk = i2v_cdiv(hw, gn_rows_per_chunk(n_img, hw));
  return ((int64_t)n_img * nchunk * channels * 5 + (int64_t)n_img * channels * 5) * (int64_t)sizeof(float);
}

extern "C" int i2v_groupnorm_bwd_f16(const i2v_gn_params* pp, const void* dy, void* dx, void* dx2, i2v_stream_t stream) {
  I2V_CHECK_ARG(pp != nullptr, "i2v_groupnorm_bwd_f16: null params");
  const i2v_gn_params& p = *pp;
  const int C = p.c1 + p.c2;
  I2V_CHECK_ARG(p.x && p.gamma && p.beta && p.workspace && dy && dx, "i2v_groupnorm_bwd_f16: null pointer");
  I2V_CHECK_ARG(p.n_img > 0 && p.hw > 0 && p.c1 > 0 && p.c2 >= 0, "i2v_groupnorm_bwd_f16: bad sizes");
  I2V_CHECK_ARG((p.c2 == 0) == (p.x2 == nullptr) && (p.c2 == 0) == (dx2 == nullptr), "i2v_groupnorm_bwd_f16: x2 / dx2 / c2 mismatch");
  I2V_CHECK_ARG(p.c1 % 8 == 0 && p.c2 % 8 == 0 && p.groups > 0 && C % p.groups == 0, "i2v_groupnorm_bwd_f16: channel counts");
  I2V_CHECK_ARG(p.frames_per_stat > 0 && p.n_img % p.frames_per_stat == 0 && !p.out_perm,
                "i2v_groupnorm_bwd_f16: frames_per_stat must divide n_img; out_perm is not supported");
  I2V_CHECK_ARG(i2v_al16(p.x) && (!p.x2 || i2v_al16(p.x2)) && i2v_al16(dy) && i2v_al16(dx) && (!dx2 || i2v_al16(dx2)) && i2v_al16(p.workspace) &&
                    i2v_al16(p.gamma) && i2v_al16(p.beta), "i2v_groupnorm_bwd_f16: pointers must be 16-byte aligned");
  hipStream_t s = reinterpret_cast<hipStream_t>(stream);
// ... 61 lines not shown
```

i2v-adapter-unofficial_amd/i2v_adapter.py:

```python
import os
from typing import Optional

import torch
from torch import nn

from . import kernels as K
from . import streams
from .blocks import (gn_proj_in, ff_tail_operands, precise_stream, Attention, FeedForward, HipModule, LazyPack, LnFoldPlan, _as_f16_matrix,
                     fold_layernorm, from_tokens, to_tokens, w16)
from ._lib import HipLibraryError
from .checkpoint import PretrainedMixin

f16 = torch.float16


def get_block(out_channel, block_depth, num_attention_heads, transformer_layers_per_block):
    block = nn.Module()
    attn_blocks = []
    for _ in range(block_depth):
        attn_block = nn.Module()
        tbs = []
        for _ in range(transformer_layers_per_block):
            tb = nn.Module()
            tb.i2v_adapter = Attention(query_dim=out_channel, heads=num_attention_heads,
# ... 47 lines not shown
                 ff_bias: bool = True, attention_out_bias: bool = True, with_adapter: bool = True, **_unused):
        super().__init__()
        if norm_type != "layer_norm" or only_cross_attention or double_self_attention or positional_embeddings:
            raise NotImplementedError("only the layer-norm spatial block of the hot path is implemented "
                                      "(SURVEY 8b: ada-norm / GLIGEN / only_cross_attention branches are dropped)")
        self.dim, self.heads, self.dim_head = dim, num_attention_heads, attention_head_dim
        self.eps = norm_eps
        self.only_cross_attention = only_cross_attention
        self.norm1 = nn.LayerNorm(dim, elementwise_affine=norm_elementwise_affine, eps=norm_eps)
        self.attn1 = Attention(query_dim=dim, heads=num_attention_heads, dim_head=attention_head_dim,
                               dropout=dropout, bias=attention_bias, out_bias=attention_out_bias)
        if cross_attention_dim is not None:
            self.norm2 = nn.LayerNorm(dim, elementwise_affine=norm_elementwise_affine, eps=norm_eps)
            self.attn2 = Attention(query_dim=dim, cross_attention_dim=cross_attention_dim,
                                   heads=num_attention_heads, dim_head=attention_head_dim, dropout=dropout,
                                   bias=attention_bias, out_bias=attention_out_bias)
        else:
            self.norm2 = None
            self.attn2 = None
        self.norm3 = nn.LayerNorm(dim, elementwise_affine=norm_elementwise_affine, eps=norm_eps)
        self.ff = FeedForward(dim, dropout=dropout, activation_fn=activation_fn, inner_dim=ff_inner_dim,
                              bias=ff_bias)
        self.i2v_adapter = Attention(query_dim=dim, heads=num_attention_heads, dim_head=attention_head_dim,
                                     dropout=dropout, bias=attention_bias, cross_attention_dim=dim,
                                     out_bias=attention_out_bias) if with_adapter else None
        self._plan = LnFoldPlan()

    def _pack(self):
        a1, ad = self.attn1, self.i2v_adapter
        p = LazyPack(g1=w16(self.norm1.weight), b1=w16(self.norm1.bias), g3=w16(self.norm3.weight),
                     b3=w16(self.norm3.bias))
        qkq = [a1.to_q.weight, a1.to_k.weight] + ([ad.to_q.weight] if ad is not None else [])
        p["w_qkq"] = w16(torch.cat(qkq, dim=0))
        p["w_v1"] = w16(a1.to_v.weight)
        p["w_o1"], p["b_o1"] = w16(a1.to_out[0].weight), w16(a1.to_out[0].bias)
        if ad is not None:
            p["w_k_ad"], p["w_v_ad"] = w16(ad.to_k.weight), w16(ad.to_v.weight)
            p["w_o_dual"] = w16(torch.cat([a1.to_out[0].weight, ad.to_out[0].weight], dim=1))
            p["b_o_dual"] = w16(a1.to_out[0].bias.float() + ad.to_out[0].bias.float())
        if self.attn2 is not None:
            p["g2"], p["b2"] = w16(self.norm2.weight), w16(self.norm2.bias)
            p["w_q2"] = w16(self.attn2.to_q.weight)
            p["w_o2"], p["b_o2"] = w16(self.attn2.to_out[0].weight), w16(self.attn2.to_out[0].bias)
            p["f_q2"] = fold_layernorm(self.attn2.to_q.weight, None, self.norm2.weight, self.norm2.bias)
            p.lazy("wq2_frag", lambda a2=self.attn2, heads=self.heads: K.pack_cross_q(a2.to_q.weight, heads))
            p.lazy("wo2_frag", lambda a2=self.attn2, heads=self.heads: K.pack_attn_out(a2.to_out[0].weight, a2.to_out[0].bias, heads))
            p.lazy("g2_f32", lambda n2=self.norm2: n2.weight.detach().float().contiguous())
            p.lazy("b2_f32", lambda n2=self.norm2: n2.bias.detach().float().contiguous())
        p["f_qkq"] = fold_layernorm(torch.cat(qkq, dim=0), None, self.norm1.weight, self.norm1.bias)
        p["f_v1"] = fold_layernorm(a1.to_v.weight, None, self.norm1.weight, self.norm1.bias)
        p["f_ff"] = self.ff.fold_norm(self.norm3)
        p.lazy("g3_f32", lambda n3=self.norm3: n3.weight.detach().float().contiguous())
        p.lazy("b3_f32", lambda n3=self.norm3: n3.bias.detach().float().contiguous())
        if K.ln_qkv_supported(128, self.dim, 3 * self.dim, 128):
            p.lazy("g1_f32", lambda n1=self.norm1: n1.weight.detach().float().contiguous())
            p.lazy("b1_f32", lambda n1=self.norm1: n1.bias.detach().float().contiguous())
            p.lazy("w_lnqkv2", lambda a1=a1: K.pack_ln_qkv(torch.cat([a1.to_q.weight, a1.to_k.weight], dim=0), a1.to_v.weight))
            if ad is not None:
                p.lazy("w_lnqkv3", lambda a1=a1, ad=ad: K.pack_ln_qkv(torch.cat([a1.to_q.weight, a1.to_k.weight, ad.to_q.weight], dim=0), a1.to_v.weight))
                p.lazy("w_lnkv_ad", lambda ad=ad: K.pack_ln_qkv(ad.to_k.weight, ad.to_v.weight))
        return p

    def _fold_ok(self, x, L, rows_qkq):
        M = x.shape[0]

        def probe1():
            p = self.packed()
            wf, ws, cb = p["f_qkq"]
            wv, sv, cv = p["f_v1"]
            return (K.gemm(x, wf[:rows_qkq], cb[:rows_qkq], ln=(ws[:rows_qkq], self.eps), query_ln_support=True) and
                    K.project_vt(x, wv, L, bias=cv, ln=(sv, self.eps), query_ln_support=True))

        def probe2():
            wf, ws, cb = self.packed()["f_q2"]
            return K.gemm(x, wf, cb, ln=(ws, self.eps), query_ln_support=True)

        def probe3():
            p = self.packed()
            return p["f_ff"] is not None and self.ff.folded_supported(x, self.eps, p["f_ff"])

        return (self._plan.get((1, M, L, rows_qkq), probe1),
                self.attn2 is not None and self._plan.get((2, M), probe2), self._plan.get((3, M), probe3))

    def _fwd(self, x, n_img, L, enable_cross_frame_attn, num_frames, ctx_text, ctx_ip, cfg_expand=False, tail=None):
        p = self.packed()
        c = self.dim
        if self.i2v_adapter is None:
            enable_cross_frame_attn = False
        if enable_cross_frame_attn:
            if num_frames is None:
                raise ValueError('`num_frames` must be provided when `enable_cross_frame_attn` is True.')
            if n_img % num_frames != 0:
                raise ValueError(f'Batch size {n_img} must be divisible by the number of frames {num_frames}.')
        rows_qkq = 3 * c if enable_cross_frame_attn else 2 * c
        fold1, fold2, fold3 = self._fold_ok(x, L, rows_qkq)
        overlap = x.shape[0] <= streams.MAX_ROWS
        fused_qkv = FUSED_LN_QKV and "w_lnqkv2" in p and K.ln_qkv_supported(x.shape[0], c, rows_qkq, L)
        n = None if (fold1 or fused_qkv) else K.layernorm(x, p["g1"], p["b1"], self.eps)
        k0 = v0t = None
        if fused_qkv:
            proj, vt1 = K.ln_qkv(x, p["g1_f32"], p["b1_f32"], p["w_lnqkv3" if enable_cross_frame_attn else "w_lnqkv2"],
                                 n_qk=rows_qkq, rows_per_image=L, eps=self.eps)
        with streams.fork(overlap, x.device) as fk:
            with fk.side():
                if fused_qkv:
                    pass
                elif fold1:
                    wv, sv, cv = p["f_v1"]
                    vt1 = K.project_vt(x, wv, L, bias=cv, ln=(sv, self.eps))
                else:
                    vt1 = K.project_vt(n, p["w_v1"], L)
                if enable_cross_frame_attn and fused_qkv and K.ln_qkv_supported(n_img // num_frames * L, c, c, L):
                    clips = n_img // num_frames
                    k0, v0t = K.ln_qkv(x, p["g1_f32"], p["b1_f32"], p["w_lnkv_ad"], n_qk=c, rows_per_image=L, eps=self.eps,
                                       images=clips, x_image_stride=num_frames * L * x.stride(0))
                elif enable_cross_frame_attn:
                    clips = n_img // num_frames
                    if n is None:
                        first = K.layernorm(x.view(clips, num_frames * L, c)[:, :L], p["g1"], p["b1"], self.eps)
                    elif clips == 1:
                        first = n[:L]
                    else:
                        first = torch.empty((clips, L, c), dtype=f16, device=x.device)
                        K.copy3d(n.view(clips, num_frames * L, c)[:, :L], first)
                    f2d = first.reshape(-1, c)
                    k0 = K.gemm(f2d, p["w_k_ad"])
                    v0t = K.project_vt(f2d, p["w_v_ad"], L)
            if fused_qkv:
                pass
            elif fold1:
                wf, ws, cb = p["f_qkq"]
                proj = K.gemm(x, wf[:rows_qkq], cb[:rows_qkq], ln=(ws[:rows_qkq], self.eps))
            else:
                proj = K.gemm(n, p["w_qkq"][:rows_qkq])
        with streams.fork(overlap and enable_cross_frame_attn, x.device) as fk:
            if enable_cross_frame_attn:
                with fk.side():
                    o2 = K.attention(proj[:, 2 * c:], k0, v0t, batch_q=n_img, lq=L, lk=L, heads=self.heads,
                                     head_dim=self.dim_head, kv_group=num_frames, scale=self.dim_head ** -0.5)
            o1 = K.attention(proj[:, :c], proj[:, c:2 * c], vt1, batch_q=n_img, lq=L, lk=L, heads=self.heads,
                             head_dim=self.dim_head, scale=self.dim_head ** -0.5)
        if enable_cross_frame_attn:
            x = K.gemm(o1, p["w_o_dual"], p["b_o_dual"], a2=o2, residual=x)
        else:
            x = K.gemm(o1, p["w_o1"], p["b_o1"], residual=x)
        if cfg_expand:
            x, n_img = K.duplicate_batch(x), 2 * n_img
        if self.attn2 is not None:
            if ctx_text is None:
                raise ValueError("encoder_hidden_states is required by the cross-attention layer")
            if n_img % ctx_text.shape[0] != 0:
                raise ValueError(f"context batch {ctx_text.shape[0]} does not divide batch {n_img}")
            kv_group = n_img // ctx_text.shape[0]
            kv = self.attn2.context_kv(ctx_text, ctx_ip)
            _k, _vt, kip, _vtip, lt, li = kv
            use_ip = kip is not None and bool(self.attn2.ip_num_tokens)
            fused_out2 = False
            if FUSED_TEXT_ATTN and (not use_ip or li <= 16) and \
                    K.cross_attn_fused_supported(x.shape[0], c, self.heads, self.dim_head, lt, kv_group * L):
                frag, frag_ip = self.attn2.context_fragments(ctx_text, kv)
                o = K.cross_attn_fused(x, p["g2_f32"], p["b2_f32"], p["wq2_frag"], frag, heads=self.heads, head_dim=self.dim_head,
                                       ctx_len=lt, rows_per_ctx=kv_group * L, eps=self.eps, scale=self.attn2.scale,
                                       ip_frag=frag_ip, ip_len=li if use_ip else 0, ip_scale=float(self.attn2.ip_scale),
                                       out_proj=p["wo2_frag"] if FUSED_ATTN_OUT else None)
                fused_out2 = FUSED_ATTN_OUT
            else:
                if fold2:
                    wf, ws, cb = p["f_q2"]
                    q = K.gemm(x, wf, cb, ln=(ws, self.eps))
                else:
                    n = K.layernorm(x, p["g2"], p["b2"], self.eps)
                    q = K.gemm(n, p["w_q2"])
                o = self.attn2._cross(q, ctx_text, ctx_ip, n_img, L, kv_group, kv=kv)
            if fused_out2:
                x = o
            else:
                x = K.gemm(o, p["w_o2"], p["b_o2"], residual=x)
        def ret(v, applied=False):
            return v if tail is None else (v, applied)
        if self.ff.fused_supported(x):
            if self.ff.tail_supported(x, tail):
                return ret(self.ff._fwd_fused(x, p["g3_f32"], p["b3_f32"], self.eps, tail=tail), True)
            return ret(self.ff._fwd_fused(x, p["g3_f32"], p["b3_f32"], self.eps))
        if fold3:
            return ret(self.ff._fwd_folded(x, self.eps, p["f_ff"]))
        n = K.layernorm(x, p["g3"], p["b3"], self.eps)
        return ret(self.ff._fwd(n, x))

    def _split_ctx(self, encoder_hidden_states):
        if encoder_hidden_states is None:
            return None, None
        ctx = _as_f16_matrix(encoder_hidden_states)
        nip = self.attn2.ip_num_tokens if self.attn2 is not None else 0
        if not nip:
            return ctx, None
        end = ctx.shape[1] - nip
        ct = torch.empty((ctx.shape[0], end, ctx.shape[2]), dtype=f16, device=ctx.device)
        ci = torch.empty((ctx.shape[0], nip, ctx.shape[2]), dtype=f16, device=ctx.device)
        K.copy3d(ctx[:, :end], ct)
        K.copy3d(ctx[:, end:], ci)
        return ct, ci

    def forward(self, hidden_states, enable_cross_frame_attn: bool = False, num_frames: Optional[int] = None,
                attention_mask=None, encoder_hidden_states=None, encoder_attention_mask=None, timestep=None,
                cross_attention_kwargs=None, class_labels=None, added_cond_kwargs=None):
        if attention_mask is not None or encoder_attention_mask is not None:
            raise NotImplementedError("attention masks are never passed on the hot path (SURVEY 8b)")
        x = _as_f16_matrix(hidden_states)
        b, l, c = x.shape
        ct, ci = self._split_ctx(encoder_hidden_states)
        out = self._fwd(x.view(-1, c), b, l, enable_cross_frame_attn, num_frames, ct, ci)
        return out.view(b, l, c).to(hidden_states.dtype)


class _Out:
    def __init__(self, sample):
        self.sample = sample

    def __getitem__(self, i):
        return (self.sample,)[i]


class I2VAdapterTransformer2DModel(HipModule):

    def __init__(self, num_attention_heads: int = 16, attention_head_dim: int = 88,
                 in_channels: Optional[int] = None, out_channels: Optional[int] = None, num_layers: int = 1,
                 dropout: float = 0.0, norm_num_groups: int = 32, cross_attention_dim: Optional[int] = None,
                 attention_bias: bool = False, sample_size: Optional[int] = None,
                 num_vector_embeds: Optional[int] = None, patch_size: Optional[int] = None,
                 activation_fn: str = "geglu", num_embeds_ada_norm: Optional[int] = None,
                 use_linear_projection: bool = False, only_cross_attention: bool = False,
                 double_self_attention: bool = False, upcast_attention: bool = False,
                 norm_type: str = "layer_norm", norm_elementwise_affine: bool = True, norm_eps: float = 1e-5,
                 attention_type: str = "default", caption_channels: int = None, with_adapter: bool = True):
        super().__init__()
        if in_channels is None or num_vector_embeds is not None or patch_size is not None:
            raise NotImplementedError("only the continuous-input branch is on the hot path (SURVEY 8b)")
        inner_dim = num_attention_heads * attention_head_dim
        self.in_channels, self.inner_dim = in_channels, inner_dim
        self.groups = norm_num_groups
        self.use_linear_projection = use_linear_projection
        self.norm = nn.GroupNorm(norm_num_groups, in_channels, eps=1e-6, affine=True)
        if use_linear_projection:
            self.proj_in = nn.Linear(in_channels, inner_dim)
        else:
            self.proj_in = nn.Conv2d(in_channels, inner_dim, kernel_size=1, stride=1, padding=0)
        self.transformer_blocks = nn.ModuleList([
            I2VAdapterTransformerBlock(inner_dim, num_attention_heads, attention_head_dim, dropout=dropout,
                                       cross_attention_dim=cross_attention_dim, activation_fn=activation_fn,
                                       attention_bias=attention_bias, only_cross_attention=only_cross_attention,
                                       double_self_attention=double_self_attention, norm_type=norm_type,
                                       norm_elementwise_affine=norm_elementwise_affine, norm_eps=norm_eps,
                                       with_adapter=with_adapter)
            for _ in range(num_layers)])
        if use_linear_projection:
            self.proj_out = nn.Linear(inner_dim, in_channels)
        else:
            self.proj_out = nn.Conv2d(inner_dim, in_channels, kernel_size=1, stride=1, padding=0)

    def from_transformer2d_model(self, transformer2d_model):
        self.load_state_dict(transformer2d_model.state_dict(), strict=False)
        for mine, theirs in zip(self.transformer_blocks, transformer2d_model.transformer_blocks):
            mine.i2v_adapter.load_state_dict(theirs.attn1.state_dict())
            mine.i2v_adapter.to_out[0].weight.data.zero_()
            mine.i2v_adapter.to_out[0].bias.data.zero_()

    def _pack(self):
        p = LazyPack(g=w16(self.norm.weight), b=w16(self.norm.bias),
                     wi=w16(self.proj_in.weight.reshape(self.inner_dim, self.in_channels)), bi=w16(self.proj_in.bias),
                     wo=w16(self.proj_out.weight.reshape(self.in_channels, self.inner_dim)), bo=w16(self.proj_out.bias))
        p.lazy("tail", lambda po=self.proj_out, ci=self.inner_dim, co=self.in_channels: ff_tail_operands(po.weight, po.bias, ci, co))
        return p

    def packed(self):
        leaves = [self.norm.weight, self.norm.bias, self.proj_in.weight, self.proj_in.bias, self.proj_out.weight,
                  self.proj_out.bias]
        key = tuple((p.data_ptr(), p._version, p.dtype) for p in leaves)
        if self._packed is None or key != self._packed_key:
            for p in leaves:
                if not p.is_cuda:
                    raise HipLibraryError(
                        f"{type(self).__name__} has parameters on {p.device}: the HIP path has no CPU fallback")
            with torch.no_grad():
                self._packed = self._pack()
            self._packed_key = key
        return self._packed

    def _fwd(self, x, enable_cross_frame_attn, num_frames, ctx_text, ctx_ip, cfg_expand=False):
        p = self.packed()
        n_img, hh, ww, c = x.shape
        t = gn_proj_in(x, p["g"], p["b"], self.groups, 1e-6, p["wi"], p["bi"])
        applied = False
        for j, blk in enumerate(self.transformer_blocks):
            expand = cfg_expand and j == 0
            n_in = n_img
            if expand:
                n_img, x = 2 * n_img, K.duplicate_batch(x)
            if j + 1 == len(self.transformer_blocks):
                t, applied = blk._fwd(t, n_in, hh * ww, enable_cross_frame_attn, num_frames, ctx_text, ctx_ip,
                                      cfg_expand=expand, tail=(p["tail"], K.sview(x, -1, c), 0, 0))
            else:
                t = blk._fwd(t, n_in, hh * ww, enable_cross_frame_attn, num_frames, ctx_text, ctx_ip, cfg_expand=expand)
        if applied:
            return K.sview(t, n_img, hh, ww, c)
        out = K.gemm(t, p["wo"], p["bo"], residual=K.sview(x, -1, c), precise=precise_stream())
        return K.sview(out, n_img, hh, ww, c)

    def forward(self, hidden_states, enable_cross_frame_attn: bool = False, encoder_hidden_states=None,
                num_frames: Optional[int] = None, timestep=None, added_cond_kwargs=None, class_labels=None,
                cross_attention_kwargs=None, attention_mask=None, encoder_attention_mask=None,
                return_dict: bool = True):
        if attention_mask is not None or encoder_attention_mask is not None:
            raise NotImplementedError("attention masks are never passed on the hot path (SURVEY 8b)")
        ct, ci = self.transformer_blocks[0]._split_ctx(encoder_hidden_states)
        out = from_tokens(self._fwd(to_tokens(hidden_states), enable_cross_frame_attn, num_frames, ct, ci),
                          hidden_states.dtype)
        if not return_dict:
            return (out,)
        return _Out(out)
```

i2v-adapter-unofficial_amd/kernels.py:

```python
import ctypes as C
import functools
import os
from typing import Optional

import torch

from . import _lib
from ._lib import (I2V_A_CONV3X3, I2V_A_PLAIN, I2V_EPI_GEGLU, I2V_EPI_GELU, I2V_EPI_NONE, I2V_STORE_ROWMAJOR,
                   I2V_STORE_ROWPERM, I2V_STORE_VT, I2V_STORE_VT_T, AttnBwdParams, AttnParams, GemmParams, GnParams,
                   HipLibraryError, LnParams, TAttnParams)

f16 = torch.float16


def _stream():
    return C.c_void_p(torch.cuda.current_stream().cuda_stream)


def _req(t: torch.Tensor, name: str, dtype=f16):
    if not isinstance(t, torch.Tensor):
        raise TypeError(f"{name} must be a tensor")
    if not t.is_cuda:
        raise HipLibraryError(f"{name} is on {t.device}: the I2V-Adapter HIP path has no CPU fallback "
                              "(move tensors to a ROCm device)")
    if dtype is not None and t.dtype != dtype:
        raise TypeError(f"{name} must be {dtype}, got {t.dtype}")
    return t


def _mat(t: torch.Tensor, name: str):
    _req(t, name)
    if t.dim() != 2:
        raise ValueError(f"{name} must be 2-D, got {tuple(t.shape)}")
    if t.shape[1] > 1 and t.stride(1) != 1:
        raise ValueError(f"{name} must have unit stride along its last dim")
    ld = t.stride(0) if t.shape[0] > 1 else max(t.stride(0), t.shape[1])
    return t, ld


def _p(t: Optional[torch.Tensor]):
    return None if t is None else C.c_void_p(t.data_ptr())


def pad8(n: int) -> int:
    return (n + 7) // 8 * 8


def lo_of(t):
    return None if t is None else getattr(t, "_i2v_lo", None)


def sview(t, *shape):
    v, lo = t.view(*shape), lo_of(t)
    if lo is not None:
        v._i2v_lo = lo.view(*shape)
    return v


def _attach_lo(p_res_lo_setter, residual, out):
    rl = lo_of(residual)
    if rl is not None and (rl.shape != residual.shape or rl.stride() != residual.stride() or rl.dtype != f16):
        raise ValueError("the low half of a stream tensor must be laid out like the tensor")
    cl = torch.empty_like(out)
    if cl.stride() != out.stride():
        raise ValueError("precise stream: `out` must be dense")
    p_res_lo_setter(rl, cl)
    out._i2v_lo = cl
    return rl, cl


def gemm(a, w, bias=None, *, a2=None, residual=None, rowvec=None, rows_per_vec=0, epilogue=I2V_EPI_NONE,
         out=None, store=I2V_STORE_ROWMAJOR, frames=0, hw=0, vt_len=0, vt_ld=0, out_scale=1.0, ln=None,
         rowvec_period=0, query_ln_support=False, w_rows=0, a_perm=None, query_batch_support=False, precise=False):
    lib = _lib.load()
    a, lda = _mat(a, "a")
    w_stack = None
    if w.dim() == 3:
        _req(w, "w")
        if w_rows <= 0 or not w.is_contiguous() or a.shape[0] != w.shape[0] * w_rows:
            raise ValueError(f"stacked w {tuple(w.shape)} needs contiguous storage and w_rows with S * w_rows == M")
        w_stack, w = w, w[0]
    w, ldw = _mat(w, "w")
    M, K1 = a.shape
    N, K = w.shape
    p = GemmParams()
    if w_stack is not None:
        p.w_batch_stride, p.rows_per_w = w_stack.stride(0), w_rows
    if a_perm is not None:
        p.a_perm_frames, p.a_perm_hw = int(a_perm[0]), int(a_perm[1])
    p.a, p.lda = _p(a), lda
    if a2 is not None:
        a2, lda2 = _mat(a2, "a2")
        if a2.shape[0] != M or K1 + a2.shape[1] != K:
            raise ValueError(f"dual-source A shapes {tuple(a.shape)} + {tuple(a2.shape)} do not match W {tuple(w.shape)}")
        p.a2, p.lda2, p.k_split = _p(a2), lda2, K1
    elif K1 != K:
        raise ValueError(f"A is {tuple(a.shape)} but W is {tuple(w.shape)}")
    p.a_mode = I2V_A_PLAIN
    p.w, p.ldw = _p(w), ldw
    if bias is not None:
        _req(bias, "bias")
        if bias.numel() != N or not bias.is_contiguous():
            raise ValueError("bias must be a contiguous vector of N elements")
        p.bias = _p(bias)
    n_out = N // 2 if epilogue == I2V_EPI_GEGLU else N
    if store in (I2V_STORE_VT, I2V_STORE_VT_T):
        tokens, chans = (N, M) if store == I2V_STORE_VT else (M, N)
        if out is None or vt_len <= 0 or vt_ld < vt_len or tokens % vt_len != 0:
            raise ValueError("VT store needs an `out` buffer, vt_len > 0, vt_ld >= vt_len and tokens % vt_len == 0")
        _req(out, "out")
        if not out.is_contiguous() or out.numel() < (tokens // vt_len) * chans * vt_ld:
            raise ValueError("VT `out` must be contiguous with at least (tokens / vt_len) * channels * vt_ld elements")
        p.c, p.ldc = _p(out), vt_ld
        p.vt_len, p.vt_ld = vt_len, vt_ld
    else:
        if out is None:
            out = torch.empty((M, n_out), dtype=f16, device=a.device)
        out, ldc = _mat(out, "out")
        if out.shape != (M, n_out):
            raise ValueError(f"out must be {(M, n_out)}, got {tuple(out.shape)}")
        p.c, p.ldc = _p(out), ldc
    if residual is not None:
        residual, ldr = _mat(residual, "residual")
        if residual.shape != (M, n_out) or epilogue == I2V_EPI_GEGLU:
            raise ValueError(f"residual must be {(M, n_out)} (and is not supported with GEGLU)")
        p.residual, p.ldr = _p(residual), ldr
    if rowvec is not None:
        rowvec, ldv = _mat(rowvec, "rowvec")
        if rowvec_period > 0:
            want = (N, rowvec_period) if store == I2V_STORE_VT_T else (rowvec_period, N)
            if rowvec.shape[0] < want[0] or rowvec.shape[1] < want[1] or (store != I2V_STORE_VT_T and rowvec.shape[1] != N):
                raise ValueError(f"periodic rowvec must cover {want}, got {tuple(rowvec.shape)}")
            p.rowvec, p.ld_rowvec, p.rowvec_period = _p(rowvec), ldv, rowvec_period
        else:
            if rows_per_vec <= 0 or M % rows_per_vec != 0 or rowvec.shape != (M // rows_per_vec, N):
                raise ValueError(f"rowvec must be [M / rows_per_vec, N], got {tuple(rowvec.shape)}")
            p.rowvec, p.ld_rowvec, p.rows_per_vec = _p(rowvec), ldv, rows_per_vec
    if ln is not None:
        wsum, eps = ln
# ... 451 lines not shown
            raise ValueError(f"cross_attn_fused: ip_frag is {tuple(ip_frag.shape)} (pack_ctx_fragments of the image tokens)")
        p.ip_frag, p.ip_len, p.ip_scale = _p(ip_frag), int(ip_len), float(ip_scale)
    if out_proj is not None:
        p.w_o, p.b_o = _attn_out_operands(out_proj, c, heads, head_dim, "cross_attn_fused")
    _lib.check(lib.i2v_cross_attn_fused_f16(C.byref(p), _stream()), "i2v_cross_attn_fused_f16")
    return out


def ln_qkv_supported(rows, channels, n_qk, rows_per_image):
    return bool(_lib.load().i2v_ln_qkv_supported(rows, channels, n_qk, rows_per_image))


def pack_ln_qkv(w_qk, w_v):
    w = torch.cat([w_qk.detach().to(f16), w_v.detach().to(f16)], dim=0)
    n, c = w.shape
    if n % 160 or c % 32:
        raise ValueError(f"pack_ln_qkv: {n} rows x {c} columns is not whole waves of 160 rows / K steps of 32")
    return w.view(n // 16, 16, c // 32, 4, 8).permute(0, 2, 3, 1, 4).contiguous().view(n, c)


def ln_qkv(x, gamma32, beta32, w_packed, *, n_qk, rows_per_image, eps, qk=None, vt=None, images=None, x_image_stride=0):
    lib = _lib.load()
    x, ldx = _mat(x, "x")
    rows, c = x.shape
    if images is not None:
        if x_image_stride % ldx or (images - 1) * (x_image_stride // ldx) + rows_per_image > rows:
            raise ValueError(f"ln_qkv: {images} images of {rows_per_image} rows at stride {x_image_stride} do not fit x {tuple(x.shape)}")
        rows = images * rows_per_image
    _req(w_packed, "w")
    for name, t in (("gamma32", gamma32), ("beta32", beta32)):
        _req(t, name, dtype=torch.float32)
    if tuple(gamma32.shape) != (c,) or tuple(beta32.shape) != (c,) or tuple(w_packed.shape) != (n_qk + c, c) or \
            not w_packed.is_contiguous():
        raise ValueError(f"ln_qkv: gamma {tuple(gamma32.shape)}, beta {tuple(beta32.shape)}, w {tuple(w_packed.shape)} for C {c}, "
                         f"n_qk {n_qk} (pack_ln_qkv)")
    if rows % rows_per_image:
        raise ValueError(f"ln_qkv: {rows} rows are not whole images of {rows_per_image}")
    n_img, ld = rows // rows_per_image, pad8(rows_per_image)
    if qk is None:
        qk = torch.empty((rows, n_qk), dtype=f16, device=x.device)
    if vt is None:
        vt = torch.empty((n_img, c, ld), dtype=f16, device=x.device)
    qk, ld_qk = _mat(qk, "qk")
    _req(vt, "vt")
    if tuple(qk.shape) != (rows, n_qk) or tuple(vt.shape) != (n_img, c, ld) or not vt.is_contiguous():
        raise ValueError(f"ln_qkv: qk {tuple(qk.shape)}, vt {tuple(vt.shape)}")
    p = _lib.LnQkvParams()
    p.x, p.ldx = _p(x), ldx
    p.gamma, p.beta, p.w = _p(gamma32), _p(beta32), _p(w_packed)
    p.qk, p.ld_qk = _p(qk), ld_qk
    p.vt, p.vt_batch_stride, p.vt_row_stride = _p(vt), c * ld, ld
    p.rows, p.rows_per_image, p.channels, p.n_qk, p.eps = rows, rows_per_image, c, n_qk, float(eps)
    p.x_image_stride = int(x_image_stride) if images is not None else 0
    _lib.check(lib.i2v_ln_qkv_f16(C.byref(p), _stream()), "i2v_ln_qkv_f16")
    return qk, vt


def ff_fused_supported(rows, channels, inner):
    return bool(_lib.load().i2v_ff_fused_supported(rows, channels, inner))


def pack_ff_fused(w1, b1, w2, b2):
    inner, c = w2.shape[1], w2.shape[0]
    nch, heads, dn = inner // 128, 8, c // 8
    dt = (dn + 15) // 16
    dev = w1.device
    m = torch.arange(16, device=dev)
    idx = ((m & 1) * inner + (m >> 1))[None, None, None, :] + (128 * torch.arange(nch, device=dev))[:, None, None, None] + \
        (16 * torch.arange(8, device=dev))[None, :, None, None] + (8 * torch.arange(2, device=dev))[None, None, :, None]
    t1 = w1.detach().to(f16)[idx.reshape(-1)].view(nch, 8, 2, 16, c // 32, 4, 8)
    w1f = t1.permute(0, 1, 2, 4, 5, 3, 6).contiguous().view(-1, 8)
    b1f = b1.detach().float()[idx.reshape(-1)].view(nch, 8, 2, 16).contiguous()
    w2p = torch.zeros((heads, 16 * dt, inner), dtype=f16, device=dev)
    w2p[:, :dn] = w2.detach().to(f16).view(heads, dn, inner)
    t2 = w2p.view(heads, dt, 16, nch, 4, 4, 8)
    w2f = t2.permute(0, 3, 4, 1, 5, 2, 6).contiguous().view(-1, 8)
    return w1f, b1f, w2f, b2.detach().float().contiguous()


def ff_fused_tail_supported(rows, channels, inner, perm_frames=0, perm_hw=0):
    return bool(_lib.load().i2v_ff_fused_tail_supported(rows, channels, inner, perm_frames, perm_hw))


def pack_ff_tail(w3, b3):
    return pack_cross_q(w3, 8), b3.detach().float().contiguous()


def ff_fused(x, gamma32, beta32, packed, *, eps, out=None, tail=None, precise=False):
    lib = _lib.load()
    x, ldx = _mat(x, "x")
    rows, c = x.shape
    w1f, b1f, w2f, b2f = packed
    inner = b1f.numel() // 2
    for name, t, dt_ in (("gamma32", gamma32, torch.float32), ("beta32", beta32, torch.float32), ("w1", w1f, f16),
                         ("b1", b1f, torch.float32), ("w2", w2f, f16), ("b2", b2f, torch.float32)):
        _req(t, name, dtype=dt_)
    if tuple(gamma32.shape) != (c,) or tuple(beta32.shape) != (c,) or b2f.numel() != c or w1f.numel() != 2 * inner * c or \
            w2f.numel() != 8 * ((c // 8 + 15) // 16 * 16) * inner:
        raise ValueError(f"ff_fused: operand sizes do not match C {c}, inner {inner} (pack_ff_fused)")
    if out is None:
        out = torch.empty((rows, c), dtype=f16, device=x.device)
    out, ldo = _mat(out, "out")
    if tuple(out.shape) != (rows, c):
        raise ValueError(f"ff_fused: out is {tuple(out.shape)}")
    p = _lib.FfFusedParams()
    p.x, p.ldx = _p(x), ldx
    p.gamma, p.beta = _p(gamma32), _p(beta32)
    p.w1, p.b1, p.w2, p.b2 = _p(w1f), _p(b1f), _p(w2f), _p(b2f)
    p.out, p.ldo = _p(out), ldo
    p.rows, p.channels, p.inner, p.eps = rows, c, inner, float(eps)
    keep = None
    if tail is not None:
        (w3f, b3f), res2, perm_frames, perm_hw = tail
        _req(w3f, "w3")
        _req(b3f, "b3", dtype=torch.float32)
        res2, ld2 = _mat(res2, "res2")
        if tuple(w3f.shape) != (8 * ((c // 8 + 15) // 16 * 16), c) or not w3f.is_contiguous() or b3f.numel() != c or \
                tuple(res2.shape) != (rows, c):
            raise ValueError(f"ff_fused: tail operands w3 {tuple(w3f.shape)}, b3 {tuple(b3f.shape)}, res2 {tuple(res2.shape)} "
                             f"do not match rows {rows}, C {c} (pack_ff_tail)")
        if perm_frames and out.data_ptr() == x.data_ptr():
            raise ValueError("ff_fused: out must not alias x when the tail permutes the rows")
        p.w3, p.b3, p.res2, p.ld_res2 = _p(w3f), _p(b3f), _p(res2), ld2
        p.perm_frames, p.perm_hw = int(perm_frames), int(perm_hw)
        if precise and lo_of(res2) is not None:
            def set_lo(rl, cl):
                p.res2_lo, p.out_lo = _p(rl), _p(cl)
            keep = _attach_lo(set_lo, res2, out)
    _lib.check(lib.i2v_ff_fused_f16(C.byref(p), _stream()), "i2v_ff_fused_f16")
    del keep
    return out


def motion_attn_tables(gamma, beta, pe, frames):
    return (gamma.detach().float().contiguous(),
            (beta.detach().float()[None, :] + pe.detach().float()[:frames]).contiguous())


def motion_attn(x, gamma32, shift32, w_qkv, *, heads, head_dim, frames, eps, scale=None, out=None, out_proj=None):
    lib = _lib.load()
    x, ldx = _mat(x, "x")
    rows, c = x.shape
    _req(w_qkv, "w_qkv")
    for name, t in (("gamma32", gamma32), ("shift32", shift32)):
        _req(t, name, dtype=torch.float32)
    if c != heads * head_dim or tuple(gamma32.shape) != (c,) or tuple(shift32.shape) != (frames, c) or not shift32.is_contiguous():
        raise ValueError(f"motion_attn: C {c} vs heads {heads} x head_dim {head_dim}, gamma {tuple(gamma32.shape)}, "
                         f"shift {tuple(shift32.shape)} (expected [{frames}, {c}])")
    if tuple(w_qkv.shape) != (lib.i2v_motion_attn_pack_rows(heads, head_dim), c) or not w_qkv.is_contiguous():
        raise ValueError(f"motion_attn: w_qkv is {tuple(w_qkv.shape)} (pack_motion_qkv)")
    if out is None:
        out = torch.empty((rows, c), dtype=f16, device=x.device)
    out, ldo = _mat(out, "out")
    if tuple(out.shape) != (rows, c):
        raise ValueError(f"motion_attn: out is {tuple(out.shape)}")
    p = _lib.MotionAttnParams()
    p.x, p.ldx = _p(x), ldx
    p.gamma = _p(gamma32)
    p.shift, p.ld_shift = _p(shift32), c
    p.w_qkv = _p(w_qkv)
    p.out, p.ldo = _p(out), ldo
    p.rows, p.channels, p.heads, p.head_dim, p.frames = rows, c, heads, head_dim, frames
    p.eps, p.scale = float(eps), float(head_dim) ** -0.5 if scale is None else float(scale)
    if out_proj is not None:
        p.w_o, p.b_o = _attn_out_operands(out_proj, c, heads, head_dim, "motion_attn")
    _lib.check(lib.i2v_motion_attn_f16(C.byref(p), _stream()), "i2v_motion_attn_f16")
    return out


def groupnorm(x, gamma, beta, groups, eps, *, x2=None, silu=False, frames_per_stat=1, out_perm=False, frames=0, stats=None):
    lib = _lib.load()
    _req(x, "x")
    if x.dim() != 4 or not x.is_contiguous():
        raise ValueError(f"x must be contiguous [N, H, W, C], got {tuple(x.shape)}")
    n, h, w, c1 = x.shape
    c2 = 0
    if x2 is not None:
        _req(x2, "x2")
        if x2.dim() != 4 or not x2.is_contiguous() or x2.shape[:3] != x.shape[:3]:
            raise ValueError("x2 must be contiguous [N, H, W, C2] with the same N, H, W as x")
        c2 = x2.shape[3]
    Cc = c1 + c2
    _req(gamma, "gamma")
    _req(beta, "beta")
    if gamma.numel() != Cc or beta.numel() != Cc:
        raise ValueError(f"gamma / beta must have {Cc} elements")
    ws = torch.empty((lib.i2v_groupnorm_workspace_bytes(n, h * w, Cc) + 3) // 4, dtype=torch.float32, device=x.device)
    y = torch.empty((n * h * w, Cc) if out_perm else (n, h, w, Cc), dtype=f16, device=x.device)
    p = GnParams()
    p.x, p.c1, p.x2, p.c2 = _p(x), c1, _p(x2), c2
    p.gamma, p.beta, p.y = _p(gamma.contiguous()), _p(beta.contiguous()), _p(y)
    p.n_img, p.hw, p.groups, p.frames_per_stat = n, h * w, groups, frames_per_stat
    p.eps, p.silu = eps, 1 if silu else 0
    p.out_perm, p.frames = (1 if out_perm else 0), frames
    p.workspace = _p(ws)
    if stats is not None:
        part, rows = stats
        _req(part, "stats", dtype=torch.float32)
        if x2 is not None or frames_per_stat != 1 or out_perm or tuple(part.shape) != (n, (h * w) // rows, groups, 2) or \
                not part.is_contiguous():
            raise ValueError(f"groupnorm: stats {tuple(part.shape)} / rows {rows} do not describe x {tuple(x.shape)} in {groups} groups")
        p.gpartial_in, p.gpartial_rows = _p(part), int(rows)
    _lib.check(lib.i2v_groupnorm_f16(C.byref(p), _stream()), "i2v_groupnorm_f16")
    return y


def groupnorm_fold(x, gamma, beta, groups, eps, w, bias, *, x2=None, frames_per_stat=1):
    lib = _lib.load()
    _req(x, "x")
    if x.dim() != 4 or not x.is_contiguous():
        raise ValueError(f"x must be contiguous [N, H, W, C], got {tuple(x.shape)}")
    n, h, wd, c1 = x.shape
    c2 = 0
    if x2 is not None:
        _req(x2, "x2")
        if x2.dim() != 4 or not x2.is_contiguous() or x2.shape[:3] != x.shape[:3]:
            raise ValueError("x2 must be contiguous [N, H, W, C2] with the same N, H, W as x")
        c2 = x2.shape[3]
    Cc = c1 + c2
    _req(gamma, "gamma")
    _req(beta, "beta")
    w2, ldw = _mat(w, "w")
    if gamma.numel() != Cc or beta.numel() != Cc or w2.shape[1] != Cc:
        raise ValueError(f"gamma / beta / w columns must have {Cc} elements")
    n_out = w2.shape[0]
    if bias is not None:
        _req(bias, "bias")
        if bias.numel() != n_out or not bias.is_contiguous():
            raise ValueError("bias must be a contiguous vector of n_out elements")
    if frames_per_stat <= 0 or n % frames_per_stat != 0:
        raise ValueError(f"batch {n} is not a multiple of frames_per_stat {frames_per_stat}")
    S = n // frames_per_stat
    ws = torch.empty((lib.i2v_groupnorm_workspace_bytes(n, h * wd, Cc) + 3) // 4, dtype=torch.float32, device=x.device)
    w_s = torch.empty((S, n_out, Cc), dtype=f16, device=x.device)
    b_s = torch.empty((S, n_out), dtype=f16, device=x.device)
    p = GnParams()
    p.x, p.c1, p.x2, p.c2 = _p(x), c1, _p(x2), c2
    p.gamma, p.beta = _p(gamma.contiguous()), _p(beta.contiguous())
    p.n_img, p.hw, p.groups, p.frames_per_stat = n, h * wd, groups, frames_per_stat
    p.eps = eps
    p.workspace = _p(ws)
    _lib.check(lib.i2v_groupnorm_fold_f16(C.byref(p), _p(w2), ldw, _p(bias), n_out, _p(w_s), _p(b_s), _stream()),
               "i2v_groupnorm_fold_f16")
    return w_s, b_s


def layernorm(x, gamma, beta, eps, *, pe=None, pe_period=0):
    lib = _lib.load()
    batched = None
    if x.dim() == 3:
        _req(x, "x")
        if x.stride(2) != 1 or x.stride(1) % 8 != 0 or x.stride(0) % 8 != 0 or x.stride(0) <= 0:
            raise ValueError("batched layernorm input needs unit last stride and row / batch strides that are multiples of 8")
        batched = (x.shape[1], x.stride(0))
        ldx = x.stride(1)
        rows, Cc = x.shape[0] * x.shape[1], x.shape[2]
    else:
        x, ldx = _mat(x, "x")
        rows, Cc = x.shape
    _req(gamma, "gamma")
    _req(beta, "beta")
    y = torch.empty((rows, Cc), dtype=f16, device=x.device)
    p = LnParams()
    p.x, p.ldx = _p(x), ldx
    p.gamma, p.beta = _p(gamma), _p(beta)
    if pe is not None:
        pe, ldpe = _mat(pe, "pe")
        if pe.shape[1] != Cc or pe.shape[0] < pe_period or pe_period <= 0:
            raise ValueError("pe must be [>= pe_period, C]")
        p.pe, p.ld_pe, p.pe_period = _p(pe), ldpe, pe_period
    p.y, p.ldy = _p(y), Cc
    p.rows, p.C, p.eps = rows, Cc, eps
    if batched is not None:
        p.x_rows_per_batch, p.x_batch_stride = batched
    _lib.check(lib.i2v_layernorm_f16(C.byref(p), _stream()), "i2v_layernorm_f16")
    return y


def softmax_rows(x, scale=1.0, out=None):
    lib = _lib.load()
    x, ldx = _mat(x, "x")
    if out is None:
        out = torch.empty((x.shape[0], pad8(x.shape[1])), dtype=f16, device=x.device)[:, : x.shape[1]]
    out, ldy = _mat(out, "out")
    if out.shape != x.shape:
        raise ValueError("softmax_rows: out must have x's shape")
    _lib.check(lib.i2v_softmax_rows_f16(_p(x), ldx, _p(out), ldy, x.shape[0], x.shape[1], float(scale), _stream()),
               "i2v_softmax_rows_f16")
    return out


def nchw_to_tokens(src, c_pad=None):
    lib = _lib.load()
    _req(src, "src", dtype=None)
    if src.dtype not in (torch.float32, f16) or src.dim() != 4:
        raise TypeError("src must be a 4-D fp32 / fp16 tensor")
    src = src.contiguous()
    n, c, h, w = src.shape
    c_pad = c if c_pad is None else c_pad
    dst = torch.empty((n, h, w, c_pad), dtype=f16, device=src.device)
    _lib.check(lib.i2v_nchw_to_tokens(_p(src), 1 if src.dtype == torch.float32 else 0, _p(dst), n, c, h * w, c_pad,
                                      _stream()), "i2v_nchw_to_tokens")
    return dst


def tokens_to_nchw(src, c=None, dtype=f16):
    lib = _lib.load()
    _req(src, "src", dtype=None)
    if src.dtype not in (torch.float32, f16):
        raise TypeError("src must be fp16 or fp32")
    if src.dim() != 4 or not src.is_contiguous():
        raise ValueError("src must be contiguous [N, H, W, C]")
    n, h, w, ld = src.shape
    c = ld if c is None else c
    if dtype not in (torch.float32, f16):
        raise TypeError("dtype must be fp32 or fp16")
    dst = torch.empty((n, c, h, w), dtype=dtype, device=src.device)
    _lib.check(lib.i2v_tokens_to_nchw(_p(src), 1 if src.dtype == torch.float32 else 0, ld, _p(dst),
                                      1 if dtype == torch.float32 else 0, n, c, h * w, _stream()), "i2v_tokens_to_nchw")
    return dst


def timestep_embedding(t, dim, t_index=None):
    lib = _lib.load()
# ... 1031 lines not shown
```

i2v-adapter-unofficial_amd/profiling.py:

```python
import torch

from . import kernels as K


def _numel_bytes(*ts):
    return sum(t.numel() * t.element_size() for t in ts if isinstance(t, torch.Tensor))


def _work_gemm(args, kw, out):
    a, w = args[0], args[1]
    M, N, Kd = a.shape[0], w.shape[-2], w.shape[-1]
    tag = "".join(t for t, on in ((" geglu", kw.get("epilogue") == K.I2V_EPI_GEGLU), (" gelu", kw.get("epilogue") == K.I2V_EPI_GELU),
                                  (" +res", kw.get("residual") is not None), (" +ln", kw.get("ln") is not None),
                                  (" st%d" % kw.get("store", 0), bool(kw.get("store")))) if on)
    if w.dim() == 3:
        tag += " wstack%d" % w.shape[0] + (" perm" if kw.get("a_perm") is not None else "")
    return ("gemm", 2.0 * M * N * Kd, _numel_bytes(a, kw.get("a2"), w, kw.get("residual"), out),
            f"{M}x{N}x{Kd}{tag}")


def _work_conv(args, kw, out):
    x, w = args[0], args[1]
    stats = None
    if isinstance(out, tuple):
        out, stats = out
    M = out.shape[0] * out.shape[1] * out.shape[2]
    wf = kw.get("w_folded")
    if wf is not None:
        return ("conv3x3", 2.0 * M * wf.shape[1] * wf.shape[2], _numel_bytes(x, wf, out), f"{M}x{wf.shape[1]}x{wf.shape[2]} up4")
    return ("conv3x3", 2.0 * M * w.shape[0] * w.shape[1], _numel_bytes(x, w, kw.get("residual"), out),
            f"{M}x{w.shape[0]}x{w.shape[1]}" + (" s2" if kw.get("stride", 1) == 2 else "")
            + (" up" if kw.get("upsample") else "") + (" +res" if kw.get("residual") is not None else "")
            + (" +gn stats" if stats is not None else ""))


def _work_attn(args, kw, out):
    c = kw["heads"] * kw["head_dim"]
    return ("attention", 4.0 * kw["batch_q"] * kw["lq"] * kw["lk"] * c, _numel_bytes(args[0], args[1], args[2], out),
            f"B{kw['batch_q']} Lq{kw['lq']} Lk{kw['lk']} h{kw['heads']} d{kw['head_dim']}")


def _work_tattn(args, kw, out):
    c = kw["heads"] * kw["head_dim"]
    return ("temporal_attention", 4.0 * kw["n_pixels"] * kw["frames"] * kw["frames"] * c,
            _numel_bytes(args[0], args[1], out) + kw["n_pixels"] * c * kw["frames"] * 2,
            f"px{kw['n_pixels']} F{kw['frames']} h{kw['heads']} d{kw['head_dim']}")


def _work_mattn(args, kw, out):
    x, w = args[0], args[3]
    rows, c = x.shape
    op = kw.get("out_proj")
    return ("motion_attn", 2.0 * rows * c * (4 if op else 3) * c + 4.0 * rows * kw["frames"] * c,
            _numel_bytes(x, w, out) + (_numel_bytes(x, op[0]) if op else 0),
            f"{rows}x{c} F{kw['frames']} h{kw['heads']} d{kw['head_dim']} (LN + q,k,v + attention" + (" + to_out + residual)" if op else ")"))


def _work_cattn(args, kw, out):
    x, w = args[0], args[3]
    rows, c = x.shape
    op = kw.get("out_proj")
    return ("cross_attn_fused", 2.0 * rows * c * (2 if op else 1) * c + 4.0 * rows * kw["ctx_len"] * c,
            _numel_bytes(x, w, args[4], out) + (_numel_bytes(x, op[0]) if op else 0),
            f"{rows}x{c} Lk{kw['ctx_len']} h{kw['heads']} d{kw['head_dim']} (LN + q + text attention" + (" + to_out + residual)" if op else ")"))


def _work_ff(args, kw, out):
    x = args[0]
    rows, c = x.shape
    inner = args[3][1].numel() // 2
    tail = kw.get("tail")
    if tail is not None:
        return ("ff_fused", 2.0 * rows * c * 2 * inner + 2.0 * rows * inner * c + 2.0 * rows * c * c,
                _numel_bytes(x, args[3][0], args[3][2], tail[0][0], tail[1], out),
                f"{rows}x{c} inner {inner} (LN + GEGLU FF + residual + proj_out + residual{', rows permuted' if tail[2] else ''})")
    return ("ff_fused", 2.0 * rows * c * 2 * inner + 2.0 * rows * inner * c, _numel_bytes(x, args[3][0], args[3][2], out),
            f"{rows}x{c} inner {inner} (LN + GEGLU FF + residual)")


def _work_lnqkv(args, kw, out):
    x, w = args[0], args[3]
    rows, c = x.shape
    return ("ln_qkv", 2.0 * rows * c * (kw["n_qk"] + c), _numel_bytes(x, w, out[0], out[1]),
            f"{rows}x{kw['n_qk']}+{c}x{c} (LN + q,k[,q_adapter] + V^T)")


def _work_gn(args, kw, out):
    if kw.get("stats") is not None:
        return "groupnorm", 0.0, 2 * _numel_bytes(out), "x".join(map(str, out.shape)) + " (stats given)"
    return "groupnorm", 0.0, 3 * _numel_bytes(out), "x".join(map(str, out.shape))


def _work_gn_fold(args, kw, out):
    x = args[0]
    return "groupnorm", 0.0, _numel_bytes(x, kw.get("x2")), "fold " + "x".join(map(str, x.shape))


def _work_ln(args, kw, out):
    return "layernorm", 0.0, 2 * _numel_bytes(out), "x".join(map(str, out.shape))


def _work_clip_attn(args, kw, out):
    b, l, h, d = kw["batch"], kw["length"], kw["heads"], kw["head_dim"]
    return "clip_text", 2.0 * 2 * b * h * d * l * (l + 1) / 2, 4 * _numel_bytes(out), f"causal b{b} h{h} L{l} d{d}"


def _work_clip_vision_attn(args, kw, out):
    b, l, h, d = kw["batch"], kw["length"], kw["heads"], kw["head_dim"]
    return "clip_vision", 2.0 * 2 * b * h * d * l * l, 4 * _numel_bytes(out), f"bidirectional b{b} h{h} L{l} d{d}"


def _work_misc(name):
    def f(args, kw, out):
        return name, 0.0, 2 * _numel_bytes(out), ""
    return f


def _work_perceiver_attn(args, kw, out):
    b, nq, h, d, l = kw["batch"], kw["n_q"], kw["heads"], kw.get("head_dim", 64), kw["len_a"] + kw.get("len_b", 0)
    return "perceiver", 2.0 * 2 * b * h * d * nq * l, 2 * _numel_bytes(out) + 4 * b * h * d * l, f"b{b} h{h} q{nq} keys{l} d{d}"


_WRAPPED = {
    "gemm": _work_gemm, "conv3x3": _work_conv, "attention": _work_attn, "temporal_attention": _work_tattn,
    "motion_attn": _work_mattn, "cross_attn_fused": _work_cattn, "ff_fused": _work_ff, "ln_qkv": _work_lnqkv,
    "groupnorm": _work_gn, "groupnorm_fold": _work_gn_fold, "layernorm": _work_ln, "silu": _work_misc("elementwise"),
    "copy3d": _work_misc("elementwise"), "timestep_embedding": _work_misc("elementwise"),
    "ddim_prep": _work_misc("elementwise"), "ddim_cfg_step": _work_misc("elementwise"),
    "nchw_to_tokens": _work_misc("elementwise"), "tokens_to_nchw": _work_misc("elementwise"),
    "lcm_cfg_step": _work_misc("elementwise"), "freenoise_gather": _work_misc("elementwise"),
    "freenoise_blend": _work_misc("elementwise"),
    "clip_embed": _work_misc("clip_text"), "clip_attention": _work_clip_attn, "quick_gelu": _work_misc("clip_text"),
    "clip_patchify": _work_misc("clip_vision"), "clip_vision_embed": _work_misc("clip_vision"),
    "clip_vision_attention": _work_clip_vision_attn, "perceiver_attention": _work_perceiver_attn,
}


class KernelProfile:
    def __init__(self):
        self.records = []
        self._saved = {}
        self._depth = 0

    def _wrap(self, name, fn, work):
        def wrapped(*args, **kw):
            if self._depth or kw.get("query_ln_support"):
                return fn(*args, **kw)
            s, e = torch.cuda.Event(enable_timing=True), torch.cuda.Event(enable_timing=True)
            self._depth += 1
            s.record()
            try:
                out = fn(*args, **kw)
            finally:
                self._depth -= 1
            e.record()
            cls, flops, nbytes, detail = work(args, kw, out)
            self.records.append((cls, flops, nbytes, s, e, f"{name} {detail}".strip()))
            return out
        return wrapped

    def __enter__(self):
        for name, work in _WRAPPED.items():
            self._saved[name] = getattr(K, name)
            setattr(K, name, self._wrap(name, self._saved[name], work))
        return self

    def __exit__(self, *exc):
        for name, fn in self._saved.items():
            setattr(K, name, fn)
        self._saved = {}

    def summary(self):
        return self._aggregate(lambda rec: rec[0])

    def by_shape(self):
        return self._aggregate(lambda rec: rec[5])

# ... 16 lines not shown
```

i2v-adapter-unofficial_amd/unet_motion_cross_frame_attn.py:

```python
import inspect
from typing import Any, Dict, Optional, Tuple, Union

import torch
from torch import nn

from . import kernels as K
from ._lib import HipLibraryError
from .blocks import (Attention, DownBlockMotion, Downsample2D, HipModule, ImageProjection, MotionAdapter, Resampler,
                     ProjectedContext, ProjectedTemb, ResnetBlock2D, TimestepEmbedding, Timesteps, UpBlockMotion, freeu_scales,
                     Upsample2D, _as_f16_matrix, _motion, from_tokens, pack_conv3x3, precise_stream, to_tokens, w16)
from .checkpoint import PretrainedMixin
from .i2v_adapter import I2VAdapterModule, I2VAdapterTransformer2DModel
from .lora import UNetLoraMixin

f16 = torch.float16


def _split_ctx(block, encoder_hidden_states):
    t2d = block.attentions[0]
    return t2d.transformer_blocks[0]._split_ctx(encoder_hidden_states)


class CrossFrameAttnDownBlockMotion(nn.Module):

    def __init__(self, in_channels: int, out_channels: int, temb_channels: int, dropout: float = 0.0,
                 num_layers: int = 1, transformer_layers_per_block: int = 1, resnet_eps: float = 1e-6,
                 resnet_time_scale_shift: str = "default", resnet_act_fn: str = "swish", resnet_groups: int = 32,
                 resnet_pre_norm: bool = True, num_attention_heads: int = 1, cross_attention_dim: int = 1280,
                 output_scale_factor: float = 1.0, downsample_padding: int = 1, add_downsample: bool = True,
                 dual_cross_attention: bool = False, use_linear_projection: bool = False,
                 only_cross_attention: bool = False, upcast_attention: bool = False,
                 attention_type: str = "default", temporal_cross_attention_dim: Optional[int] = None,
                 temporal_num_attention_heads: int = 8, temporal_max_seq_length: int = 32):
        super().__init__()
        self.has_cross_attention = True
        self.num_attention_heads = num_attention_heads
        resnets, attentions, motion_modules = [], [], []
        for i in range(num_layers):
            cin = in_channels if i == 0 else out_channels
            resnets.append(ResnetBlock2D(cin, out_channels, temb_channels=temb_channels, eps=resnet_eps,
                                         groups=resnet_groups, output_scale_factor=output_scale_factor))
            attentions.append(I2VAdapterTransformer2DModel(
                num_attention_heads, out_channels // num_attention_heads, in_channels=out_channels,
                num_layers=transformer_layers_per_block, cross_attention_dim=cross_attention_dim,
                norm_num_groups=resnet_groups, use_linear_projection=use_linear_projection,
                only_cross_attention=only_cross_attention))
            motion_modules.append(_motion(out_channels, temporal_num_attention_heads, resnet_groups,
                                          temporal_cross_attention_dim, temporal_max_seq_length))
        self.attentions = nn.ModuleList(attentions)
        self.resnets = nn.ModuleList(resnets)
        self.motion_modules = nn.ModuleList(motion_modules)
        self.downsamplers = (nn.ModuleList([Downsample2D(out_channels, use_conv=True, out_channels=out_channels,
                                                         padding=downsample_padding, name="op")])
                             if add_downsample else None)

    def _fwd(self, x, temb_act, enable, ctx_text, ctx_ip, num_frames, additional_residuals=None, cfg_shared=False,
             residual_scale=None):
        states = ()
        n_layers = len(self.resnets)
        for i, (resnet, attn, motion) in enumerate(zip(self.resnets, self.attentions, self.motion_modules)):
            shared = cfg_shared and i == 0
            x = resnet._fwd(x, temb_act.first_half() if shared else temb_act)
            x = attn._fwd(x, enable, num_frames, ctx_text, ctx_ip, cfg_expand=shared)
            x = motion._fwd(x, num_frames)
            if i == n_layers - 1 and additional_residuals is not None:
                x = K.add_broadcast_residual(x, additional_residuals, scale=residual_scale)
            states += (x,)
        if self.downsamplers is not None:
            for d in self.downsamplers:
                x = d._fwd(x)
            states += (x,)
        return x, states

    def forward(self, hidden_states, temb=None, enable_cross_frame_attn: bool = False,
                encoder_hidden_states=None, attention_mask=None, num_frames: int = 1,
                encoder_attention_mask=None, cross_attention_kwargs=None, additional_residuals=None):
        if attention_mask is not None or encoder_attention_mask is not None:
            raise NotImplementedError("attention masks are never passed on the hot path (SURVEY 8b)")
        ta = K.silu(_as_f16_matrix(temb)) if temb is not None else None
        ct, ci = _split_ctx(self, encoder_hidden_states)
        x, states = self._fwd(to_tokens(hidden_states), ta, enable_cross_frame_attn, ct, ci, num_frames,
                              None if additional_residuals is None else to_tokens(additional_residuals))
        dt = hidden_states.dtype
        return from_tokens(x, dt), tuple(from_tokens(s, dt) for s in states)


class CrossFrameAttnUpBlockMotion(nn.Module):

    def __init__(self, in_channels: int, out_channels: int, prev_output_channel: int, temb_channels: int,
                 resolution_idx: Optional[int] = None, dropout: float = 0.0, num_layers: int = 1,
                 transformer_layers_per_block: int = 1, resnet_eps: float = 1e-6,
                 resnet_time_scale_shift: str = "default", resnet_act_fn: str = "swish", resnet_groups: int = 32,
                 resnet_pre_norm: bool = True, num_attention_heads: int = 1, cross_attention_dim: int = 1280,
                 output_scale_factor: float = 1.0, add_upsample: bool = True, dual_cross_attention: bool = False,
                 use_linear_projection: bool = False, only_cross_attention: bool = False,
                 upcast_attention: bool = False, attention_type: str = "default",
                 temporal_cross_attention_dim: Optional[int] = None, temporal_num_attention_heads: int = 8,
                 temporal_max_seq_length: int = 32):
        super().__init__()
        self.has_cross_attention = True
        self.num_attention_heads = num_attention_heads
        resnets, attentions, motion_modules = [], [], []
        for i in range(num_layers):
            res_skip_channels = in_channels if (i == num_layers - 1) else out_channels
            resnet_in_channels = prev_output_channel if i == 0 else out_channels
            resnets.append(ResnetBlock2D(resnet_in_channels + res_skip_channels, out_channels,
                                         temb_channels=temb_channels, eps=resnet_eps, groups=resnet_groups,
                                         output_scale_factor=output_scale_factor))
            attentions.append(I2VAdapterTransformer2DModel(
                num_attention_heads, out_channels // num_attention_heads, in_channels=out_channels,
                num_layers=transformer_layers_per_block, cross_attention_dim=cross_attention_dim,
                norm_num_groups=resnet_groups, use_linear_projection=use_linear_projection,
                only_cross_attention=only_cross_attention))
            motion_modules.append(_motion(out_channels, temporal_num_attention_heads, resnet_groups,
                                          temporal_cross_attention_dim, temporal_max_seq_length))
        self.attentions = nn.ModuleList(attentions)
        self.resnets = nn.ModuleList(resnets)
        self.motion_modules = nn.ModuleList(motion_modules)
        self.upsamplers = (nn.ModuleList([Upsample2D(out_channels, use_conv=True, out_channels=out_channels)])
                           if add_upsample else None)
        self.resolution_idx = resolution_idx

    def _fwd(self, x, res_tuple, temb_act, enable, ctx_text, ctx_ip, num_frames, upsample_size=None):
        fu = freeu_scales(self)
        for resnet, attn, motion in zip(self.resnets, self.attentions, self.motion_modules):
            skip = res_tuple[-1]
            res_tuple = res_tuple[:-1]
            if fu is not None:
                x, skip = K.freeu(x, skip, *fu)
            x = resnet._fwd(x, temb_act, x2=skip)
            x = attn._fwd(x, enable, num_frames, ctx_text, ctx_ip)
            x = motion._fwd(x, num_frames)
        if self.upsamplers is not None:
            for u in self.upsamplers:
                x = u._fwd(x, upsample_size)
        return x

    def forward(self, hidden_states, res_hidden_states_tuple, temb=None, enable_cross_frame_attn: bool = False,
                encoder_hidden_states=None, cross_attention_kwargs=None, upsample_size=None,
                attention_mask=None, encoder_attention_mask=None, num_frames: int = 1):
        if attention_mask is not None or encoder_attention_mask is not None:
            raise NotImplementedError("attention masks are never passed on the hot path (SURVEY 8b)")
        ta = K.silu(_as_f16_matrix(temb)) if temb is not None else None
        ct, ci = _split_ctx(self, encoder_hidden_states)
        res = tuple(to_tokens(r) for r in res_hidden_states_tuple)
        x = self._fwd(to_tokens(hidden_states), res, ta, enable_cross_frame_attn, ct, ci, num_frames, upsample_size)
        return from_tokens(x, hidden_states.dtype)


class UNetMidBlockCrossFrameAttnMotion(nn.Module):

    def __init__(self, in_channels: int, temb_channels: int, dropout: float = 0.0, num_layers: int = 1,
                 transformer_layers_per_block: int = 1, resnet_eps: float = 1e-6,
                 resnet_time_scale_shift: str = "default", resnet_act_fn: str = "swish", resnet_groups: int = 32,
                 resnet_pre_norm: bool = True, num_attention_heads: int = 1, output_scale_factor: float = 1.0,
                 cross_attention_dim: int = 1280, dual_cross_attention=False, use_linear_projection=False,
                 upcast_attention=False, attention_type: str = "default", temporal_num_attention_heads: int = 1,
                 temporal_cross_attention_dim: Optional[int] = None, temporal_max_seq_length: int = 32):
        super().__init__()
        self.has_cross_attention = True
        self.num_attention_heads = num_attention_heads
        resnet_groups = resnet_groups if resnet_groups is not None else min(in_channels // 4, 32)

        def res():
            return ResnetBlock2D(in_channels, in_channels, temb_channels=temb_channels, eps=resnet_eps,
                                 groups=resnet_groups, output_scale_factor=output_scale_factor)

        resnets, attentions, motion_modules = [res()], [], []
        for _ in range(num_layers):
            attentions.append(I2VAdapterTransformer2DModel(
                num_attention_heads, in_channels // num_attention_heads, in_channels=in_channels,
                num_layers=transformer_layers_per_block, cross_attention_dim=cross_attention_dim,
                norm_num_groups=resnet_groups, use_linear_projection=use_linear_projection))
            resnets.append(res())
            motion_modules.append(_motion(in_channels, temporal_num_attention_heads, resnet_groups,
                                          temporal_cross_attention_dim, temporal_max_seq_length))
        self.attentions = nn.ModuleList(attentions)
        self.resnets = nn.ModuleList(resnets)
        self.motion_modules = nn.ModuleList(motion_modules)

    def _fwd(self, x, temb_act, enable, ctx_text, ctx_ip, num_frames):
        x = self.resnets[0]._fwd(x, temb_act)
        for attn, resnet, motion in zip(self.attentions, self.resnets[1:], self.motion_modules):
            x = attn._fwd(x, enable, num_frames, ctx_text, ctx_ip)
            x = motion._fwd(x, num_frames)
            x = resnet._fwd(x, temb_act)
        return x

    def forward(self, hidden_states, temb=None, enable_cross_frame_attn: bool = False,
                encoder_hidden_states=None, attention_mask=None, cross_attention_kwargs=None,
                encoder_attention_mask=None, num_frames: int = 1):
        if attention_mask is not None or encoder_attention_mask is not None:
            raise NotImplementedError("attention masks are never passed on the hot path (SURVEY 8b)")
        ta = K.silu(_as_f16_matrix(temb)) if temb is not None else None
        ct, ci = _split_ctx(self, encoder_hidden_states)
        return from_tokens(self._fwd(to_tokens(hidden_states), ta, enable_cross_frame_attn, ct, ci, num_frames),
                           hidden_states.dtype)


def get_down_block(down_block_type, num_layers, in_channels, out_channels, temb_channels, add_downsample,
                   resnet_eps, resnet_act_fn, num_attention_heads, resnet_groups=None, cross_attention_dim=None,
                   downsample_padding=None, dual_cross_attention=False, use_linear_projection=True,
                   only_cross_attention=False, upcast_attention=False, resnet_time_scale_shift="default",
                   temporal_num_attention_heads=8, temporal_max_seq_length=32, transformer_layers_per_block=1):
    if down_block_type == "DownBlockMotion":
        return DownBlockMotion(num_layers=num_layers, in_channels=in_channels, out_channels=out_channels,
                               temb_channels=temb_channels, add_downsample=add_downsample, resnet_eps=resnet_eps,
                               resnet_groups=resnet_groups, downsample_padding=downsample_padding,
                               temporal_num_attention_heads=temporal_num_attention_heads,
                               temporal_max_seq_length=temporal_max_seq_length)
    if down_block_type == "CrossFrameAttnDownBlockMotion":
        if cross_attention_dim is None:
            raise ValueError("cross_attention_dim must be specified for CrossFrameAttnDownBlockMotion")
        return CrossFrameAttnDownBlockMotion(
            num_layers=num_layers, in_channels=in_channels, out_channels=out_channels,
            temb_channels=temb_channels, add_downsample=add_downsample, resnet_eps=resnet_eps,
            resnet_groups=resnet_groups, downsample_padding=downsample_padding,
            cross_attention_dim=cross_attention_dim, num_attention_heads=num_attention_heads,
            use_linear_projection=use_linear_projection, only_cross_attention=only_cross_attention,
            temporal_num_attention_heads=temporal_num_attention_heads,
            temporal_max_seq_length=temporal_max_seq_length)
    raise ValueError(f"{down_block_type} does not exist.")


def get_up_block(up_block_type, num_layers, in_channels, out_channels, prev_output_channel, temb_channels,
                 add_upsample, resnet_eps, resnet_act_fn, num_attention_heads, resolution_idx=None,
                 resnet_groups=None, cross_attention_dim=None, dual_cross_attention=False,
                 use_linear_projection=True, only_cross_attention=False, upcast_attention=False,
                 resnet_time_scale_shift="default", temporal_num_attention_heads=8,
                 temporal_cross_attention_dim=None, temporal_max_seq_length=32, transformer_layers_per_block=1,
                 dropout=0.0):
    if up_block_type == "UpBlockMotion":
        return UpBlockMotion(num_layers=num_layers, in_channels=in_channels, out_channels=out_channels,
                             prev_output_channel=prev_output_channel, temb_channels=temb_channels,
                             add_upsample=add_upsample, resnet_eps=resnet_eps, resnet_groups=resnet_groups,
                             resolution_idx=resolution_idx,
                             temporal_num_attention_heads=temporal_num_attention_heads,
                             temporal_max_seq_length=temporal_max_seq_length)
    if up_block_type == "CrossFrameAttnUpBlockMotion":
        if cross_attention_dim is None:
            raise ValueError("cross_attention_dim must be specified for CrossFrameAttnUpBlockMotion")
        return CrossFrameAttnUpBlockMotion(
            num_layers=num_layers, in_channels=in_channels, out_channels=out_channels,
            prev_output_channel=prev_output_channel, temb_channels=temb_channels, add_upsample=add_upsample,
            resnet_eps=resnet_eps, resnet_groups=resnet_groups, cross_attention_dim=cross_attention_dim,
            num_attention_heads=num_attention_heads, use_linear_projection=use_linear_projection,
            only_cross_attention=only_cross_attention, resolution_idx=resolution_idx,
            temporal_num_attention_heads=temporal_num_attention_heads,
            temporal_max_seq_length=temporal_max_seq_length)
    raise ValueError(f"{up_block_type} does not exist.")


class _Config(dict):
    __getattr__ = dict.get

    def __setattr__(self, k, v):
        self[k] = v


class UNet3DConditionOutput:
    def __init__(self, sample):
        self.sample = sample


class AttnProcessorHIP:

    def __init__(self, num_tokens: int = 0, scale: float = 1.0):
# ... 682 lines not shown
```

include/i2v_hip.h:

```cpp
#ifndef I2V_HIP_H
#define I2V_HIP_H

#include <stdint.h>

#ifdef __cplusplus
extern "C" {
#endif

#define I2V_ABI_VERSION 27

#define I2V_OK 0
#define I2V_ERR_INVALID_ARG (-1)
#define I2V_ERR_UNSUPPORTED (-2)
#define I2V_ERR_LAUNCH (-3)

typedef void* i2v_stream_t;

int i2v_abi_version(void);
const char* i2v_last_error(void);

enum {
  I2V_EPI_NONE = 0,
  I2V_EPI_GELU = 1,
  I2V_EPI_GEGLU = 2
};

enum {
  I2V_STORE_ROWMAJOR = 0,
  I2V_STORE_ROWPERM = 1,
  I2V_STORE_VT = 2,
  I2V_STORE_VT_T = 3
};

enum {
  I2V_A_PLAIN = 0,
  I2V_A_CONV3X3 = 1
};

typedef struct i2v_gemm_params {
  const void* a;
  int64_t lda;
  const void* a2;
  int64_t lda2;
  int32_t k_split;
  int32_t a_mode;
  const void* w;
  int64_t ldw;
  const void* bias;
  const void* residual;
  int64_t ldr;
  const void* rowvec;
  int64_t ld_rowvec;
  int32_t rows_per_vec;
  int32_t rowvec_period;
  const void* ln_wsum;
  float ln_eps;
  void* c;
  int64_t ldc;
  int32_t M, N, K;
  int32_t epilogue;
  int32_t store_mode;
  int32_t frames, hw;
  int32_t vt_len, vt_ld;
  float out_scale;
  int32_t n_img, in_h, in_w, cin, out_h, out_w, stride, upsample, asym_pad;
  int32_t conv_kblock;
  int64_t w_batch_stride;
  int32_t rows_per_w;
  int32_t a_perm_frames, a_perm_hw;
  void* workspace;
  int64_t workspace_bytes;
  int32_t c_is_f32;
  void* gn_partial;
  int32_t gn_groups;
  const void* residual_lo;
  void* c_lo;
} i2v_gemm_params;

int i2v_gemm_f16(const i2v_gemm_params* p, i2v_stream_t stream);
int i2v_gemm_ln_supported(const i2v_gemm_params* p);
int i2v_gemm_batch_supported(const i2v_gemm_params* p);
int i2v_gemm_upconv_fold_supported(const i2v_gemm_params* p);
int64_t i2v_gemm_workspace_bytes(const i2v_gemm_params* p);
int32_t i2v_gemm_gn_partial_rows(const i2v_gemm_params* p);

enum {
  I2V_ROUTE_GENERIC = 0,
  I2V_ROUTE_CONV_THIN = 1,
  I2V_ROUTE_BIG_TILE = 2,
  I2V_ROUTE_BIG_DEEP = 3,
  I2V_ROUTE_BIG_SPLITK = 4
};
// ... 40 lines not shown
  float scale;
} i2v_tattn_params;

int i2v_temporal_attention_f16(const i2v_tattn_params* p, i2v_stream_t stream);

enum { I2V_TATTN_LDS_FORM = 0, I2V_TATTN_REG_FORM = 1 };

struct i2v_tattn_route {
  int32_t form;
  int32_t dqk, dpv;
  int32_t pf;
  int32_t nqt;
  int32_t blocks;
};

int i2v_temporal_attention_route(const i2v_tattn_params* p, struct i2v_tattn_route* route);
int i2v_temporal_attention_last_route(struct i2v_tattn_route* route);
int i2v_tattn_kernel_exists(const struct i2v_tattn_route* route);

typedef struct i2v_motion_attn_params {
  const void* x; int64_t ldx;
  const void* gamma;
  const void* shift; int64_t ld_shift;
  const void* w_qkv;
  void* out; int64_t ldo;
  int64_t rows;
  int32_t channels, heads, head_dim, frames;
  float eps, scale;
  const void* w_o; const void* b_o;
} i2v_motion_attn_params;

int32_t i2v_motion_attn_supported(int64_t rows, int32_t channels, int32_t heads, int32_t head_dim, int32_t frames);
int32_t i2v_motion_attn_pack_rows(int32_t heads, int32_t head_dim);
int i2v_motion_attn_f16(const i2v_motion_attn_params* p, i2v_stream_t stream);

typedef struct i2v_cross_attn_fused_params {
  const void* x; int64_t ldx;
  const void* gamma; const void* beta;
  const void* w_q;
  const void* ctx_frag;
  void* out; int64_t ldo;
  int64_t rows, rows_per_ctx;
  int32_t channels, heads, head_dim, ctx_len;
  float eps, scale;
  const void* ip_frag; int32_t ip_len; float ip_scale;
  const void* w_o; const void* b_o;
} i2v_cross_attn_fused_params;

int32_t i2v_cross_attn_fused_supported(int64_t rows, int32_t channels, int32_t heads, int32_t head_dim, int32_t ctx_len,
                                       int64_t rows_per_ctx);
int32_t i2v_cross_attn_fused_pack_rows(int32_t heads, int32_t head_dim);
int64_t i2v_cross_attn_fused_ctx_elems(int32_t n_ctx, int32_t heads, int32_t head_dim);
int i2v_cross_attn_fused_f16(const i2v_cross_attn_fused_params* p, i2v_stream_t stream);

typedef struct i2v_ln_qkv_params {
  const void* x; int64_t ldx;
  const void* gamma; const void* beta;
  const void* w;
  void* qk; int64_t ld_qk;
  void* vt; int64_t vt_batch_stride, vt_row_stride;
  int64_t rows, rows_per_image;
  int32_t channels, n_qk;
  float eps;
  int64_t x_image_stride;
} i2v_ln_qkv_params;

int32_t i2v_ln_qkv_supported(int64_t rows, int32_t channels, int32_t n_qk, int64_t rows_per_image);
int i2v_ln_qkv_f16(const i2v_ln_qkv_params* p, i2v_stream_t stream);

typedef struct i2v_ff_fused_params {
  const void* x; int64_t ldx;
  const void* gamma; const void* beta;
  const void* w1; const void* b1;
  const void* w2; const void* b2;
  void* out; int64_t ldo;
  int64_t rows;
  int32_t channels, inner;
  float eps;
  const void* w3; const void* b3;
  const void* res2; int64_t ld_res2;
  int32_t perm_frames, perm_hw;
  const void* res2_lo;
  void* out_lo;
} i2v_ff_fused_params;

int32_t i2v_ff_fused_supported(int64_t rows, int32_t channels, int32_t inner);
int32_t i2v_ff_fused_tail_supported(int64_t rows, int32_t channels, int32_t inner, int32_t perm_frames, int32_t perm_hw);
int i2v_ff_fused_f16(const i2v_ff_fused_params* p, i2v_stream_t stream);

typedef struct i2v_gn_params {
  const void* x;  int32_t c1;
  const void* x2; int32_t c2;
  const void* gamma; const void* beta;
  void* y;
  int32_t n_img, hw, groups, frames_per_stat;
  float eps;
  int32_t silu;
  int32_t out_perm; int32_t frames;
  void* workspace;
  const void* gpartial_in; int32_t gpartial_rows;
} i2v_gn_params;

int64_t i2v_groupnorm_workspace_bytes(int32_t n_img, int32_t hw, int32_t channels);
int i2v_groupnorm_f16(const i2v_gn_params* p, i2v_stream_t stream);
int i2v_groupnorm_fold_f16(const i2v_gn_params* p, const void* w, int64_t ldw, const void* bias, int32_t n_out,
                           void* w_out, void* bias_out, i2v_stream_t stream);

typedef struct i2v_ln_params {
  const void* x; int64_t ldx;
  const void* gamma; const void* beta;
  const void* pe; int64_t ld_pe; int32_t pe_period;
  void* y; int64_t ldy;
  int32_t rows, C;
  float eps;
  int32_t x_rows_per_batch; int64_t x_batch_stride;
} i2v_ln_params;

int i2v_layernorm_f16(const i2v_ln_params* p, i2v_stream_t stream);

int i2v_softmax_rows_f16(const void* x, int64_t ldx, void* y, int64_t ldy, int32_t rows, int32_t cols, float scale,
                         i2v_stream_t stream);

int i2v_nchw_to_tokens(const void* src, int32_t src_is_f32, void* dst, int32_t n, int32_t c, int32_t hw,
                       int32_t c_pad, i2v_stream_t stream);
int i2v_tokens_to_nchw(const void* src, int32_t src_is_f32, int64_t ld, void* dst, int32_t dst_is_f32, int32_t n,
                       int32_t c, int32_t hw, i2v_stream_t stream);
int i2v_timestep_embedding(const float* t, const int32_t* t_index, int32_t t_rows, void* out, int32_t n,
                           int32_t dim, i2v_stream_t stream);
int i2v_select_row_f16(const void* table, int64_t ld, int32_t rows, const int32_t* row_index, void* out, int32_t cols,
                       i2v_stream_t stream);
int i2v_silu_f16(const void* x, void* y, int64_t n, i2v_stream_t stream);
int i2v_repeat_rows_f16(const void* x, void* y, int64_t rows_in, int64_t cols, int32_t repeat,
                        i2v_stream_t stream);
int i2v_copy3d_f16(const void* src, int64_t src_batch_stride, int64_t ld_src, void* dst, int64_t dst_batch_stride,
                   int64_t ld_dst, int64_t batches, int64_t rows, int64_t cols, i2v_stream_t stream);

int64_t i2v_pack_ctx_fragments_elems(int32_t n_ctx, int32_t heads, int32_t head_dim);
int i2v_pack_ctx_fragments_f16(const void* k, int64_t ldk, const void* vt, int64_t vt_row_stride, int64_t vt_batch_stride, void* out,
                               int32_t n_ctx, int32_t heads, int32_t head_dim, int32_t ctx_len, i2v_stream_t stream);

int i2v_ddim_prep(float* latents, const float* cond, void* model_in, int32_t b, int32_t f, int32_t c,
                  int32_t hw, int32_t c_pad, int32_t cfg_copies, i2v_stream_t stream);
int i2v_ddim_cfg_step(float* latents, const void* noise_pred, int32_t np_is_f32, int64_t ld_np, const float* coef, int32_t n_steps,
                      int32_t* step_index, float guidance_scale, int32_t b, int32_t f, int32_t c, int32_t hw,
                      int32_t cfg_copies, i2v_stream_t stream);

int i2v_dpm_cfg_step(float* latents, float* x0_prev, const void* noise_pred, int32_t np_is_f32, int64_t ld_np, const float* coef,
                     int32_t n_steps, int32_t* step_index, float guidance_scale, int32_t b, int32_t f, int32_t c, int32_t hw,
                     int32_t cfg_copies, i2v_stream_t stream);

int i2v_lcm_cfg_step(float* latents, const float* noise, int32_t n_noise, const void* noise_pred, int32_t np_is_f32, int64_t ld_np,
                     const float* coef, int32_t n_steps, int32_t* step_index, float guidance_scale, int32_t b, int32_t f, int32_t c,
                     int32_t hw, int32_t cfg_copies, i2v_stream_t stream);

int i2v_freeu_f16(const void* hidden, const void* hidden_lo, void* hidden_out, void* hidden_out_lo, const void* skip, void* skip_out,
                  int32_t n, int32_t h, int32_t w, int32_t c1, int32_t c2, float b, float s, i2v_stream_t stream);

int i2v_vae_tile_blend(const void* tile, const void* up, const void* left, const void* upleft, int32_t src_is_f32, int32_t n, int32_t th,
                       int32_t tw, int64_t ld, int32_t c, int32_t up_h, int32_t left_w, int32_t blend_extent, int32_t limit, void* out,
                       int32_t out_h, int32_t out_w, int32_t oy, int32_t ox, i2v_stream_t stream);

#define I2V_LORA_MAX_ADAPTERS 8
#define I2V_LORA_MAX_RANK 256
typedef struct i2v_lora_adapter {
  const void* down;
  const void* up;
  int32_t rank;
  float scale;
} i2v_lora_adapter;
int i2v_lora_merge(void* dst, const void* base, int32_t is_f32, int32_t out, int32_t in, const i2v_lora_adapter* adapters,
                   int32_t n_adapters, i2v_stream_t stream);

int64_t i2v_freeinit_workspace_bytes(int32_t b, int32_t f, int32_t c, int32_t h, int32_t w);
int i2v_freeinit_mix(const float* latents, const float* init_noise, const float* z_rand, const float* lpf, float* out, void* workspace,
                     int64_t workspace_bytes, int32_t b, int32_t f, int32_t c, int32_t h, int32_t w, float sqrt_alpha,
                     float sqrt_one_minus_alpha, i2v_stream_t stream);

int i2v_freenoise_gather_f16(const void* src, int64_t ld_src, void* dst, int64_t ld_dst, const int32_t* starts, int64_t n_pixels,
                             int32_t frames, int32_t windows, int32_t length, int32_t c, i2v_stream_t stream);
int i2v_freenoise_blend_f16(const void* src, int64_t ld_src, void* dst, int64_t ld_dst, const int32_t* idx, const float* coef,
                            int64_t n_pixels, int32_t frames, int32_t windows, int32_t length, int32_t pairs, int32_t c,
                            i2v_stream_t stream);

// ... 182 lines not shown
```

Before: 20.99.

## Emit GroupNorm partial statistics from fused FF tail for the motion module's norm

The fused feed-forward + proj_out tail kernel now optionally computes per-tile, per-group mean and M2 partials of its output and writes them to a small buffer attached to the output tensor. The following motion module's GroupNorm-fold path consumes these partials through a finalize kernel instead of running a separate statistics pass that rereads the activation. This saves one full read of the 64x64-level activation per transformer-to-motion transition, at the cost of extra register pressure and wave reductions in the FF epilogue and a new kernel variant.

Result: no change. 20.97 (-0.1%).

```diff
diff --git a/i2v-adapter-unofficial_amd/_lib.py b/i2v-adapter-unofficial_amd/_lib.py
--- a/i2v-adapter-unofficial_amd/_lib.py
+++ b/i2v-adapter-unofficial_amd/_lib.py
@@ -3,7 +3,7 @@
 
 _HERE = os.path.dirname(os.path.abspath(__file__))
 LIB_PATH = os.environ.get("I2V_LIB_PATH") or os.path.join(_HERE, "libi2v_hip.so")
-ABI_VERSION = 27
+ABI_VERSION = 28
 
 I2V_EPI_NONE, I2V_EPI_GELU, I2V_EPI_GEGLU = 0, 1, 2
 I2V_STORE_ROWMAJOR, I2V_STORE_ROWPERM, I2V_STORE_VT, I2V_STORE_VT_T = 0, 1, 2, 3
@@ -158,6 +158,7 @@
         ("res2", C.c_void_p), ("ld_res2", C.c_int64),
         ("perm_frames", C.c_int32), ("perm_hw", C.c_int32),
         ("res2_lo", C.c_void_p), ("out_lo", C.c_void_p),
+        ("gn_partial", C.c_void_p), ("gn_groups", C.c_int32),
     ]
 
 
@@ -203,7 +204,7 @@
         ("eps", C.c_float), ("silu", C.c_int32),
         ("out_perm", C.c_int32), ("frames", C.c_int32),
         ("workspace", C.c_void_p),
-        ("gpartial_in", C.c_void_p), ("gpartial_rows", C.c_int32),
+        ("gpartial_in", C.c_void_p), ("gpartial_rows", C.c_int32), ("gpartial_groups", C.c_int32),
     ]
 
 
@@ -275,6 +276,7 @@
     "i2v_ln_qkv_f16": (C.c_int, [C.POINTER(LnQkvParams), _P]),
     "i2v_ff_fused_supported": (C.c_int32, [C.c_int64, C.c_int32, C.c_int32]),
     "i2v_ff_fused_tail_supported": (C.c_int32, [C.c_int64, C.c_int32, C.c_int32, C.c_int32, C.c_int32]),
+    "i2v_ff_fused_gn_partial_rows": (C.c_int32, [C.c_int64, C.c_int32, C.c_int32, C.c_int32, C.c_int32, C.c_int32]),
     "i2v_ff_fused_f16": (C.c_int, [C.POINTER(FfFusedParams), _P]),
     "i2v_groupnorm_workspace_bytes": (C.c_int64, [C.c_int32, C.c_int32, C.c_int32]),
     "i2v_groupnorm_f16": (C.c_int, [C.POINTER(GnParams), _P]),
diff --git a/i2v-adapter-unofficial_amd/blocks.py b/i2v-adapter-unofficial_amd/blocks.py
--- a/i2v-adapter-unofficial_amd/blocks.py
+++ b/i2v-adapter-unofficial_amd/blocks.py
@@ -187,7 +187,7 @@
 GN_FOLD_RATIO = float(os.environ.get("I2V_GN_FOLD_RATIO", "4"))
 
 
-def gn_proj_in(x, gamma, beta, groups, eps, w, bias, frames=0):
+def gn_proj_in(x, gamma, beta, groups, eps, w, bias, frames=0, stats=None):
     n, hh, ww, c = x.shape
     hw = hh * ww
     fps = frames if frames > 0 else 1
@@ -195,7 +195,9 @@
     if GN_FOLD and GN_FOLD_RATIO * s_groups * n_out <= n * hw:
         kw = dict(rows_per_vec=fps * hw, w_rows=fps * hw, a_perm=(frames, hw) if frames > 0 else None)
         if _fold_supported(x, s_groups, n_out, kw):
-            w_s, b_s = K.groupnorm_fold(x, gamma, beta, groups, eps, w, bias, frames_per_stat=fps)
+            if stats is not None and (stats[0].shape[1] != groups or hw % stats[1] != 0):
+                stats = None
+            w_s, b_s = K.groupnorm_fold(x, gamma, beta, groups, eps, w, bias, frames_per_stat=fps, stats=stats)
             return K.gemm(x.view(-1, c), w_s, None, rowvec=b_s, **kw)
     if frames > 0:
         h = K.groupnorm(x, gamma, beta, groups, eps, frames_per_stat=frames, out_perm=True, frames=frames)
@@ -556,7 +558,11 @@
         p = self.packed()
         return FUSED_FF and "fused" in p and K.ff_fused_supported(x2d.shape[0], x2d.shape[1], p["b1"].numel() // 2)
 
-    def _fwd_fused(self, x2d, gamma32, beta32, eps, tail=None):
+    def _fwd_fused(self, x2d, gamma32, beta32, eps, tail=None, gn_stats_groups=0):
+        if gn_stats_groups and tail is not None:
+            out, stats = K.ff_fused(x2d, gamma32, beta32, self.packed()["fused"], eps=eps, tail=tail, precise=precise_stream(),
+                                    gn_stats_groups=gn_stats_groups)
+            return K.attach_gn_stats(out, stats)
         return K.ff_fused(x2d, gamma32, beta32, self.packed()["fused"], eps=eps, tail=tail, precise=precise_stream())
 
     def tail_supported(self, x2d, tail):
@@ -791,7 +797,8 @@
         if n % num_frames != 0:
             raise ValueError(f"batch {n} is not a multiple of num_frames {num_frames}")
         n_pixels = (n // num_frames) * hh * ww
-        t = gn_proj_in(x, p["g"], p["b"], self.groups, 1e-6, p["wi"], p["bi"], frames=num_frames)
+        t = gn_proj_in(x, p["g"], p["b"], self.groups, 1e-6, p["wi"], p["bi"], frames=num_frames,
+                       stats=K.gn_stats_of(x))
         applied = False
         for j, blk in enumerate(self.transformer_blocks):
             if j + 1 == len(self.transformer_blocks):
diff --git a/i2v-adapter-unofficial_amd/csrc/ff_fused.hip b/i2v-adapter-unofficial_amd/csrc/ff_fused.hip
--- a/i2v-adapter-unofficial_amd/csrc/ff_fused.hip
+++ b/i2v-adapter-unofficial_amd/csrc/ff_fused.hip
@@ -20,11 +20,13 @@
 constexpr int FF_PD = 3;
 constexpr int FF_AD = 4;
 
-template <int C, int INNER, int H, bool PROJ, bool HILO = false>
+constexpr int FF_CPG = 10;
+template <int C, int INNER, int H, bool PROJ, bool HILO = false, bool GNS = false>
 __global__ __launch_bounds__(64 * H) void ff_fused_kernel(const i2v_ff_fused_params p, const int ntiles, long long* __restrict__ stamps) {
   constexpr int KS = C / 32, NJ = C / 64, NCH = INNER / FF_CH, DN = C / H, DT = (DN + 15) / 16;
   static_assert(C % 64 == 0 && H == 8 && INNER % FF_CH == 0 && DT == 3 && DN == 40, "SD-1.5 64^2 level: C = 320, inner = 1280");
   static_assert(PROJ || !HILO, "the precise stream enters and leaves through the tail");
+  static_assert((PROJ || !GNS) && DN % FF_CPG == 0, "statistics of the tail's output; a wave's channels are whole groups");
   extern __shared__ __attribute__((aligned(16))) f16 lds[];
   f16* panel = lds;
   f16* hbuf = lds + FF_PIX * 16 * C;
@@ -388,6 +390,8 @@
       FF_T(t_p);
       load_res2(1);
       load_res2_lo(0);
+      constexpr int GB = 5;
+      float gk[GB], gs[GB], gq[GB];
 #pragma unroll
       for (int pix = 0; pix < FF_PIX; ++pix) {
         if (pix == HP) {
@@ -421,6 +425,20 @@
 #pragma unroll
             for (int r = 0; r < 4; ++r) o[r] += (float)xlo[t][r];
           }
+          if constexpr (GNS) {
+#pragma unroll
+            for (int r = 0; r < 4; ++r) {
+              const int b = t < 2 ? 2 * t + (r >> 1) : 4;
+              if (pix == 0 && (r == 0 || (t < 2 && r == 2))) {
+                gk[b] = o[r];
+                gs[b] = gq[b] = 0.f;
+              } else {
+                const float d = o[r] - gk[b];
+                gs[b] += d;
+                gq[b] = fmaf(d, d, gq[b]);
+              }
+            }
+          }
           const f16x4 o16 = to_half(o);
           oh[t] = __builtin_bit_cast(u32x2, o16);
           if constexpr (HILO) {
@@ -432,6 +450,45 @@
         }
         store_row(O + (int64_t)orow[pix] * p.ldo, oh);
         if constexpr (HILO) store_row(OL + (int64_t)orow[pix] * p.ldo, ol);
+      }
+      if constexpr (GNS) {
+        constexpr int NG = DN / FF_CPG;
+        auto wave_total = [](float v) {
+          v = sum_lanes8(v);
+          v += __builtin_bit_cast(float, __builtin_amdgcn_mov_dpp(__builtin_bit_cast(int, v), 0x140, 0xF, 0xF, true));
+          return lane_xor32_sum(lane_xor16_sum(v));
+        };
+        float im[GB], i2[GB], bn[GB];
+        int ig[GB];
+#pragma unroll
+        for (int b = 0; b < GB; ++b) {
+          bn[b] = (float)(FF_PIX * (b < 4 ? 2 : 4));
+          im[b] = gk[b] + gs[b] / bn[b];
+          i2[b] = fmaxf(gq[b] - gs[b] * gs[b] / bn[b], 0.f);
+          const int ch = b < 4 ? 16 * (b >> 1) + 4 * eg + 2 * (b & 1) : 32 + 4 * eg;
+          ig[b] = ch < DN ? ch / FF_CPG : -1;
+        }
+        float gmean[NG], gm2[NG];
+#pragma unroll
+        for (int q = 0; q < NG; ++q) {
+          float a = 0.f;
+#pragma unroll
+          for (int b = 0; b < GB; ++b) a += (ig[b] == q) ? bn[b] * im[b] : 0.f;
+          gmean[q] = wave_total(a) * (1.0f / (FF_PIX * 16 * FF_CPG));
+          float m = 0.f;
+#pragma unroll
+          for (int b = 0; b < GB; ++b) {
+            const float dm = im[b] - gmean[q];
+            m += (ig[b] == q) ? fmaf(bn[b] * dm, dm, i2[b]) : 0.f;
+          }
+          gm2[q] = wave_total(m);
+        }
+        static_assert(NG == 4, "two 16-byte stores per wave");
+        if (eln == 0) {
+          float* dst = reinterpret_cast<float*>(p.gn_partial) + ((int64_t)tile * (C / FF_CPG) + NG * wave) * 2;
+          *reinterpret_cast<f32x4*>(dst) = f32x4{gmean[0], gm2[0], gmean[1], gm2[1]};
+          *reinterpret_cast<f32x4*>(dst + 4) = f32x4{gmean[2], gm2[2], gmean[3], gm2[3]};
+        }
       }
     }
     lds_barrier();
@@ -447,8 +504,8 @@
 
 constexpr size_t FF_LDS = 2 * (size_t)FF_PIX * 16 * 320 * sizeof(f16);
 
-template <bool PROJ, bool HILO = false>
-int ff_cus() { return i2v_big_lds_kernel_cus(reinterpret_cast<const void*>(ff_fused_kernel<320, 1280, 8, PROJ, HILO>), FF_LDS); }
+template <bool PROJ, bool HILO = false, bool GNS = false>
+int ff_cus() { return i2v_big_lds_kernel_cus(reinterpret_cast<const void*>(ff_fused_kernel<320, 1280, 8, PROJ, HILO, GNS>), FF_LDS); }
 
 }
 
@@ -463,6 +520,13 @@
     if (perm_frames <= 0 || (perm_frames & (perm_frames - 1)) || perm_hw <= 0 || rows % ((int64_t)perm_frames * perm_hw) != 0) return 0;
   }
   return ff_cus<true>() > 0;
+}
+
+extern "C" int32_t i2v_ff_fused_gn_partial_rows(int64_t rows, int32_t channels, int32_t inner, int32_t perm_frames, int32_t perm_hw,
+                                                int32_t groups) {
+  if (perm_frames != 0 || perm_hw != 0 || groups <= 0 || channels != groups * FF_CPG) return 0;
+  if (!i2v_ff_fused_tail_supported(rows, channels, inner, 0, 0)) return 0;
+  return ff_cus<true, false, true>() > 0 ? FF_PIX * 16 : 0;
 }
 
 extern "C" int i2v_ff_fused_f16(const i2v_ff_fused_params* pp, i2v_stream_t stream) {
@@ -492,8 +556,19 @@
     I2V_CHECK_ARG(p.b3 == nullptr && p.res2 == nullptr && p.perm_frames == 0 && p.perm_hw == 0 && p.res2_lo == nullptr && p.out_lo == nullptr,
                   "i2v_ff_fused_f16: tail fields set without w3");
   }
+  const bool gns = p.gn_partial != nullptr;
+  if (gns) {
+    I2V_CHECK_ARG(tail && p.perm_frames == 0, "i2v_ff_fused_f16: gn_partial is written by the tail without a row permutation");
+    I2V_CHECK_ARG(p.gn_groups > 0 && p.channels == p.gn_groups * FF_CPG,
+                  "i2v_ff_fused_f16: gn_partial in %d groups of %d channels: groups of %d only (i2v_ff_fused_gn_partial_rows)", p.gn_groups,
+                  p.channels, FF_CPG);
+    I2V_CHECK_ARG(i2v_al16(p.gn_partial), "i2v_ff_fused_f16: gn_partial must be 16-byte aligned");
+  } else {
+    I2V_CHECK_ARG(p.gn_groups == 0, "i2v_ff_fused_f16: gn_groups set without gn_partial");
+  }
   const bool hilo = tail && p.out_lo != nullptr;
-  const int cus = hilo ? ff_cus<true, true>() : tail ? ff_cus<true>() : ff_cus<false>();
+  const int cus = gns ? (hilo ? ff_cus<true, true, true>() : ff_cus<true, false, true>())
+                      : hilo ? ff_cus<true, true>() : tail ? ff_cus<true>() : ff_cus<false>();
   if (cus <= 0) I2V_FAIL(I2V_ERR_UNSUPPORTED, "i2v_ff_fused_f16: %zu bytes of LDS refused by this device", FF_LDS);
   const int ntiles = (int)(p.rows / (FF_PIX * 16));
   const int grid = i2v_persistent_grid(ntiles, cus);
@@ -502,7 +577,11 @@
   stamps = getenv("I2V_FF_STAMP_PTR") ? reinterpret_cast<long long*>(strtoull(getenv("I2V_FF_STAMP_PTR"), nullptr, 0)) : nullptr;
 #endif
   hipStream_t s = reinterpret_cast<hipStream_t>(stream);
-  if (hilo)
+  if (gns && hilo)
+    hipLaunchKernelGGL((ff_fused_kernel<320, 1280, 8, true, true, true>), dim3((unsigned)grid), dim3(512), FF_LDS, s, p, ntiles, stamps);
+  else if (gns)
+    hipLaunchKernelGGL((ff_fused_kernel<320, 1280, 8, true, false, true>), dim3((unsigned)grid), dim3(512), FF_LDS, s, p, ntiles, stamps);
+  else if (hilo)
     hipLaunchKernelGGL((ff_fused_kernel<320, 1280, 8, true, true>), dim3((unsigned)grid), dim3(512), FF_LDS, s, p, ntiles, stamps);
   else if (tail)
     hipLaunchKernelGGL((ff_fused_kernel<320, 1280, 8, true>), dim3((unsigned)grid), dim3(512), FF_LDS, s, p, ntiles, stamps);
diff --git a/i2v-adapter-unofficial_amd/csrc/norm.hip b/i2v-adapter-unofficial_amd/csrc/norm.hip
--- a/i2v-adapter-unofficial_amd/csrc/norm.hip
+++ b/i2v-adapter-unofficial_amd/csrc/norm.hip
@@ -751,7 +751,17 @@
   const int nchunk = (int)i2v_cdiv(p.hw, rpc);
   float* partial = reinterpret_cast<float*>(p.workspace);
   float* coef = partial + (int64_t)p.n_img * nchunk * C * 2;
-  if (p.groups <= GN_MAXG && C <= GN_MAXC) {
+  if (p.gpartial_in != nullptr) {
+    I2V_CHECK_ARG(p.x2 == nullptr && p.groups <= GN_MAXG && C <= GN_MAXC,
+                  "i2v_groupnorm_fold_f16: gpartial_in is for one source of at most %d channels in at most %d groups", GN_MAXC, GN_MAXG);
+    I2V_CHECK_ARG(p.gpartial_groups == p.groups,
+                  "i2v_groupnorm_fold_f16: the partials were written for %d groups, the norm has %d", p.gpartial_groups, p.groups);
+    I2V_CHECK_ARG(p.gpartial_rows > 0 && p.hw % p.gpartial_rows == 0 && (reinterpret_cast<uintptr_t>(p.gpartial_in) & 7) == 0,
+                  "i2v_groupnorm_fold_f16: gpartial_rows (%d) must divide hw (%d), gpartial_in be 8-byte aligned", p.gpartial_rows, p.hw);
+    hipLaunchKernelGGL(gn_finalize_g_kernel, dim3(p.n_img / p.frames_per_stat, p.groups), dim3(256), 0, s,
+                       reinterpret_cast<const float*>(p.gpartial_in), p.hw / p.gpartial_rows, C, p.groups, p.frames_per_stat, p.hw,
+                       p.gpartial_rows, p.eps, reinterpret_cast<const f16*>(p.gamma), reinterpret_cast<const f16*>(p.beta), coef);
+  } else if (p.groups <= GN_MAXG && C <= GN_MAXC) {
     float* gpartial = coef + (int64_t)p.n_img * C * 2;
     hipLaunchKernelGGL(gn_stats_kernel, dim3(nchunk, p.n_img), dim3(256), (size_t)C * 2 * sizeof(float), s,
                        reinterpret_cast<const f16*>(p.x), p.c1, reinterpret_cast<const f16*>(p.x2), p.c2, p.hw, rpc, partial, gpartial,
@@ -794,6 +804,8 @@
                   "i2v_groupnorm_f16: gpartial_in is for per-image statistics of one source without a row permutation");
     I2V_CHECK_ARG(p.gpartial_rows > 0 && p.hw % p.gpartial_rows == 0 && (reinterpret_cast<uintptr_t>(p.gpartial_in) & 7) == 0,
                   "i2v_groupnorm_f16: gpartial_rows (%d) must divide hw (%d)", p.gpartial_rows, p.hw);
+    I2V_CHECK_ARG(p.gpartial_groups == 0 || p.gpartial_groups == p.groups,
+                  "i2v_groupnorm_f16: the partials were written for %d groups, the norm has %d", p.gpartial_groups, p.groups);
     const int pchunks = p.hw / p.gpartial_rows;
     const size_t lds = ((size_t)pchunks * p.groups * 2 + (size_t)p.groups * 2) * sizeof(float);
     I2V_CHECK_ARG(lds <= 48 * 1024, "i2v_groupnorm_f16: %d partial blocks per image do not fit the finalise step", pchunks);
diff --git a/i2v-adapter-unofficial_amd/i2v_adapter.py b/i2v-adapter-unofficial_amd/i2v_adapter.py
--- a/i2v-adapter-unofficial_amd/i2v_adapter.py
+++ b/i2v-adapter-unofficial_amd/i2v_adapter.py
@@ -153,7 +153,7 @@
         return (self._plan.get((1, M, L, rows_qkq), probe1),
                 self.attn2 is not None and self._plan.get((2, M), probe2), self._plan.get((3, M), probe3))
 
-    def _fwd(self, x, n_img, L, enable_cross_frame_attn, num_frames, ctx_text, ctx_ip, cfg_expand=False, tail=None):
+    def _fwd(self, x, n_img, L, enable_cross_frame_attn, num_frames, ctx_text, ctx_ip, cfg_expand=False, tail=None, gn_stats_groups=0):
         p = self.packed()
         c = self.dim
         if self.i2v_adapter is None:
@@ -251,7 +251,7 @@
             return v if tail is None else (v, applied)
         if self.ff.fused_supported(x):
             if self.ff.tail_supported(x, tail):
-                return ret(self.ff._fwd_fused(x, p["g3_f32"], p["b3_f32"], self.eps, tail=tail), True)
+                return ret(self.ff._fwd_fused(x, p["g3_f32"], p["b3_f32"], self.eps, tail=tail, gn_stats_groups=gn_stats_groups), True)
             return ret(self.ff._fwd_fused(x, p["g3_f32"], p["b3_f32"], self.eps))
         if fold3:
             return ret(self.ff._fwd_folded(x, self.eps, p["f_ff"]))
@@ -357,7 +357,7 @@
             self._packed_key = key
         return self._packed
 
-    def _fwd(self, x, enable_cross_frame_attn, num_frames, ctx_text, ctx_ip, cfg_expand=False):
+    def _fwd(self, x, enable_cross_frame_attn, num_frames, ctx_text, ctx_ip, cfg_expand=False, gn_stats_groups=0):
         p = self.packed()
         n_img, hh, ww, c = x.shape
         t = gn_proj_in(x, p["g"], p["b"], self.groups, 1e-6, p["wi"], p["bi"])
@@ -369,7 +369,7 @@
                 n_img, x = 2 * n_img, K.duplicate_batch(x)
             if j + 1 == len(self.transformer_blocks):
                 t, applied = blk._fwd(t, n_in, hh * ww, enable_cross_frame_attn, num_frames, ctx_text, ctx_ip,
-                                      cfg_expand=expand, tail=(p["tail"], K.sview(x, -1, c), 0, 0))
+                                      cfg_expand=expand, tail=(p["tail"], K.sview(x, -1, c), 0, 0), gn_stats_groups=gn_stats_groups)
             else:
                 t = blk._fwd(t, n_in, hh * ww, enable_cross_frame_attn, num_frames, ctx_text, ctx_ip, cfg_expand=expand)
         if applied:
diff --git a/i2v-adapter-unofficial_amd/kernels.py b/i2v-adapter-unofficial_amd/kernels.py
--- a/i2v-adapter-unofficial_amd/kernels.py
+++ b/i2v-adapter-unofficial_amd/kernels.py
@@ -54,7 +54,23 @@
     v, lo = t.view(*shape), lo_of(t)
     if lo is not None:
         v._i2v_lo = lo.view(*shape)
+    st = gn_stats_of(t)
+    if st is not None:
+        v._i2v_gn = st
     return v
+
+
+def gn_stats_of(t):
+    return None if t is None else getattr(t, "_i2v_gn", None)
+
+
+def attach_gn_stats(t, stats):
+    if stats is None:
+        if hasattr(t, "_i2v_gn"):
+            del t._i2v_gn
+    else:
+        t._i2v_gn = stats
+    return t
 
 
 def _attach_lo(p_res_lo_setter, residual, out):
@@ -672,11 +688,15 @@
     return bool(_lib.load().i2v_ff_fused_tail_supported(rows, channels, inner, perm_frames, perm_hw))
 
 
+def ff_fused_gn_partial_rows(rows, channels, inner, perm_frames=0, perm_hw=0, groups=32):
+    return int(_lib.load().i2v_ff_fused_gn_partial_rows(rows, channels, inner, perm_frames, perm_hw, groups))
+
+
 def pack_ff_tail(w3, b3):
     return pack_cross_q(w3, 8), b3.detach().float().contiguous()
 
 
-def ff_fused(x, gamma32, beta32, packed, *, eps, out=None, tail=None, precise=False):
+def ff_fused(x, gamma32, beta32, packed, *, eps, out=None, tail=None, precise=False, gn_stats_groups=0):
     lib = _lib.load()
     x, ldx = _mat(x, "x")
     rows, c = x.shape
@@ -717,9 +737,18 @@
             def set_lo(rl, cl):
                 p.res2_lo, p.out_lo = _p(rl), _p(cl)
             keep = _attach_lo(set_lo, res2, out)
+    stats = None
+    if gn_stats_groups:
+        if tail is None:
+            raise ValueError("ff_fused: gn_stats_groups needs a tail (the statistics are those of the tail's output)")
+        prow = lib.i2v_ff_fused_gn_partial_rows(rows, c, inner, p.perm_frames, p.perm_hw, int(gn_stats_groups))
+        if prow > 0:
+            part = torch.empty((rows // prow, int(gn_stats_groups), 2), dtype=torch.float32, device=x.device)
+            p.gn_partial, p.gn_groups = _p(part), int(gn_stats_groups)
+            stats = (part, int(prow))
     _lib.check(lib.i2v_ff_fused_f16(C.byref(p), _stream()), "i2v_ff_fused_f16")
     del keep
-    return out
+    return (out, stats) if gn_stats_groups else out
 
 
 def motion_attn_tables(gamma, beta, pe, frames):
@@ -790,12 +819,12 @@
         if x2 is not None or frames_per_stat != 1 or out_perm or tuple(part.shape) != (n, (h * w) // rows, groups, 2) or \
                 not part.is_contiguous():
             raise ValueError(f"groupnorm: stats {tuple(part.shape)} / rows {rows} do not describe x {tuple(x.shape)} in {groups} groups")
-        p.gpartial_in, p.gpartial_rows = _p(part), int(rows)
+        p.gpartial_in, p.gpartial_rows, p.gpartial_groups = _p(part), int(rows), int(groups)
     _lib.check(lib.i2v_groupnorm_f16(C.byref(p), _stream()), "i2v_groupnorm_f16")
     return y
 
 
-def groupnorm_fold(x, gamma, beta, groups, eps, w, bias, *, x2=None, frames_per_stat=1):
+def groupnorm_fold(x, gamma, beta, groups, eps, w, bias, *, x2=None, frames_per_stat=1, stats=None):
     lib = _lib.load()
     _req(x, "x")
     if x.dim() != 4 or not x.is_contiguous():
@@ -830,6 +859,14 @@
     p.n_img, p.hw, p.groups, p.frames_per_stat = n, h * wd, groups, frames_per_stat
     p.eps = eps
     p.workspace = _p(ws)
+    if stats is not None:
+        part, prow = stats
+        _req(part, "stats", dtype=torch.float32)
+        prow = int(prow)
+        if x2 is not None or prow <= 0 or (h * wd) % prow != 0 or part.dim() != 3 or part.shape[2] != 2 or not part.is_contiguous() or \
+                part.shape[0] != n * ((h * wd) // prow):
+            raise ValueError(f"groupnorm_fold: stats {tuple(part.shape)} / rows {prow} do not describe x {tuple(x.shape)}")
+        p.gpartial_in, p.gpartial_rows, p.gpartial_groups = _p(part), prow, int(part.shape[1])
     _lib.check(lib.i2v_groupnorm_fold_f16(C.byref(p), _p(w2), ldw, _p(bias), n_out, _p(w_s), _p(b_s), _stream()),
                "i2v_groupnorm_fold_f16")
     return w_s, b_s
diff --git a/i2v-adapter-unofficial_amd/profiling.py b/i2v-adapter-unofficial_amd/profiling.py
--- a/i2v-adapter-unofficial_amd/profiling.py
+++ b/i2v-adapter-unofficial_amd/profiling.py
@@ -70,10 +70,13 @@
     rows, c = x.shape
     inner = args[3][1].numel() // 2
     tail = kw.get("tail")
+    stats = None
+    if isinstance(out, tuple):
+        out, stats = out
     if tail is not None:
         return ("ff_fused", 2.0 * rows * c * 2 * inner + 2.0 * rows * inner * c + 2.0 * rows * c * c,
                 _numel_bytes(x, args[3][0], args[3][2], tail[0][0], tail[1], out),
-                f"{rows}x{c} inner {inner} (LN + GEGLU FF + residual + proj_out + residual{', rows permuted' if tail[2] else ''})")
+                f"{rows}x{c} inner {inner} (LN + GEGLU FF + residual + proj_out + residual{', rows permuted' if tail[2] else ''})" + (" +gn stats" if stats is not None else ""))
     return ("ff_fused", 2.0 * rows * c * 2 * inner + 2.0 * rows * inner * c, _numel_bytes(x, args[3][0], args[3][2], out),
             f"{rows}x{c} inner {inner} (LN + GEGLU FF + residual)")
 
@@ -93,6 +96,8 @@
 
 def _work_gn_fold(args, kw, out):
     x = args[0]
+    if kw.get("stats") is not None:
+        return "groupnorm", 0.0, _numel_bytes(kw["stats"][0]), "fold " + "x".join(map(str, x.shape)) + " (stats given)"
     return "groupnorm", 0.0, _numel_bytes(x, kw.get("x2")), "fold " + "x".join(map(str, x.shape))
 
 
diff --git a/i2v-adapter-unofficial_amd/unet_motion_cross_frame_attn.py b/i2v-adapter-unofficial_amd/unet_motion_cross_frame_attn.py
--- a/i2v-adapter-unofficial_amd/unet_motion_cross_frame_attn.py
+++ b/i2v-adapter-unofficial_amd/unet_motion_cross_frame_attn.py
@@ -61,7 +61,7 @@
         for i, (resnet, attn, motion) in enumerate(zip(self.resnets, self.attentions, self.motion_modules)):
             shared = cfg_shared and i == 0
             x = resnet._fwd(x, temb_act.first_half() if shared else temb_act)
-            x = attn._fwd(x, enable, num_frames, ctx_text, ctx_ip, cfg_expand=shared)
+            x = attn._fwd(x, enable, num_frames, ctx_text, ctx_ip, cfg_expand=shared, gn_stats_groups=motion.groups)
             x = motion._fwd(x, num_frames)
             if i == n_layers - 1 and additional_residuals is not None:
                 x = K.add_broadcast_residual(x, additional_residuals, scale=residual_scale)
@@ -129,7 +129,7 @@
             if fu is not None:
                 x, skip = K.freeu(x, skip, *fu)
             x = resnet._fwd(x, temb_act, x2=skip)
-            x = attn._fwd(x, enable, num_frames, ctx_text, ctx_ip)
+            x = attn._fwd(x, enable, num_frames, ctx_text, ctx_ip, gn_stats_groups=motion.groups)
             x = motion._fwd(x, num_frames)
         if self.upsamplers is not None:
             for u in self.upsamplers:
@@ -182,7 +182,7 @@
     def _fwd(self, x, temb_act, enable, ctx_text, ctx_ip, num_frames):
         x = self.resnets[0]._fwd(x, temb_act)
         for attn, resnet, motion in zip(self.attentions, self.resnets[1:], self.motion_modules):
-            x = attn._fwd(x, enable, num_frames, ctx_text, ctx_ip)
+            x = attn._fwd(x, enable, num_frames, ctx_text, ctx_ip, gn_stats_groups=motion.groups)
             x = motion._fwd(x, num_frames)
             x = resnet._fwd(x, temb_act)
         return x
diff --git a/include/i2v_hip.h b/include/i2v_hip.h
--- a/include/i2v_hip.h
+++ b/include/i2v_hip.h
@@ -7,7 +7,7 @@
 extern "C" {
 #endif
 
-#define I2V_ABI_VERSION 27
+#define I2V_ABI_VERSION 28
 
 #define I2V_OK 0
 #define I2V_ERR_INVALID_ARG (-1)
@@ -214,10 +214,12 @@
   int32_t perm_frames, perm_hw;
   const void* res2_lo;
   void* out_lo;
+  void* gn_partial; int32_t gn_groups;
 } i2v_ff_fused_params;
 
 int32_t i2v_ff_fused_supported(int64_t rows, int32_t channels, int32_t inner);
 int32_t i2v_ff_fused_tail_supported(int64_t rows, int32_t channels, int32_t inner, int32_t perm_frames, int32_t perm_hw);
+int32_t i2v_ff_fused_gn_partial_rows(int64_t rows, int32_t channels, int32_t inner, int32_t perm_frames, int32_t perm_hw, int32_t groups);
 int i2v_ff_fused_f16(const i2v_ff_fused_params* p, i2v_stream_t stream);
 
 typedef struct i2v_gn_params {
@@ -230,7 +232,7 @@
   int32_t silu;
   int32_t out_perm; int32_t frames;
   void* workspace;
-  const void* gpartial_in; int32_t gpartial_rows;
+  const void* gpartial_in; int32_t gpartial_rows; int32_t gpartial_groups;
 } i2v_gn_params;
 
 int64_t i2v_groupnorm_workspace_bytes(int32_t n_img, int32_t hw, int32_t channels);
```
